# saugns/saugns

Hardware: AMD Instinct MI355X
Metric: mono samples/sec/GPU @ N voices (depth-3 FM) (higher is better)
Workload: dtype f32 (f64 table interpolation, u32 phase)

## Files before the change

### saugns_amd/build.py

```python
import os
import subprocess
import sys

HERE = os.path.dirname(os.path.abspath(__file__))
CSRC = os.path.join(HERE, "csrc")
LIB = os.path.join(HERE, "libsaugns_amd.so")
SOURCES = ["capi.cpp", "engine.cpp", "plan.cpp", "tables.cpp", "program_io.cpp", "sndout.cpp", "bank_builder.cpp",
           "hip_backend.hip"]
HEADERS = ["engine.h", "hip_backend.h", "capi_internal.h", "sau_dev_math.h", "sau_dev_ops.h", "launch_plan.h",
           "k_common.h", "k_wave_scan.h", "k_block_loop.h", "k_fast_types.h", "k_analyze.h", "k_decode.h", "k_fast_voice.h", "k_fast_group.h", "k_fast_group_lm.h",
           "k_chain.h", "k_finish.h", "k_levels.h", "k_decimate.h",
           "sau_dev_types.h", "../../include/sau_abi.h", "../../include/saugns_amd.h"]
FLAGS = ["--offload-arch=gfx950", "-O3", "-ffp-contract=off", "-fPIC", "-std=c++17",
         "-Wall", "-fvisibility=hidden", "-fvisibility-inlines-hidden"]


def _stale():
    if not os.path.exists(LIB):
        return True
    t = os.path.getmtime(LIB)
    deps = [os.path.join(CSRC, f) for f in SOURCES + HEADERS] + [__file__]
    return any(os.path.getmtime(d) > t for d in deps)


def build_variant(name, defines):
    build()
    hipcc = os.environ.get("HIPCC", "/opt/rocm/bin/hipcc")
    vdir = os.path.join(HERE, "variants")
    os.makedirs(vdir, exist_ok=True)
    obj = os.path.join(vdir, "hip_backend_%s.o" % name)
    subprocess.check_call([hipcc] + FLAGS + ["-D" + d for d in defines] +
                          ["-c", os.path.join(CSRC, "hip_backend.hip"), "-o", obj])
    objs = [os.path.join(CSRC, s.rsplit(".", 1)[0] + ".o") for s in SOURCES if s != "hip_backend.hip"]
    out = os.path.join(vdir, "lib_%s.so" % name)
    subprocess.check_call([hipcc, "--offload-arch=gfx950", "-shared", "-fPIC", "-o", out] + objs + [obj, "-ldl"])
    return out


def build(force=False, verbose=False):
    if not force and not _stale():
        return LIB
    import fcntl
    with open(os.path.join(HERE, ".build.lock"), "w") as lock:
        fcntl.flock(lock, fcntl.LOCK_EX)
        try:
            if not force and not _stale():
                return LIB
            return _build(verbose, force)
        finally:
            fcntl.flock(lock, fcntl.LOCK_UN)


def _build(verbose, force=False):
    hipcc = os.environ.get("HIPCC", "/opt/rocm/bin/hipcc")
    objs = []
    for src in SOURCES:
        obj = os.path.join(CSRC, src.rsplit(".", 1)[0] + ".o")
        objs.append(obj)
        deps = [src] + [h for h in HEADERS if src.endswith(".hip") or not h.startswith("k_")]
        if not force and os.path.exists(obj) and all(
                os.path.getmtime(os.path.join(CSRC, d)) <= os.path.getmtime(obj) for d in deps) and \
                os.path.getmtime(__file__) <= os.path.getmtime(obj):
            continue
        cmd = [hipcc] + FLAGS + ["-c", os.path.join(CSRC, src), "-o", obj]
        if verbose:
            print(" ".join(cmd), file=sys.stderr)
        subprocess.check_call(cmd)
    cmd = [hipcc, "--offload-arch=gfx950", "-shared", "-fPIC", "-o", LIB] + objs + ["-ldl"]
    subprocess.check_call(cmd)
    return LIB


if __name__ == "__main__":
    if len(sys.argv) > 2 and sys.argv[1] == "--variant":
        print(build_variant(sys.argv[2], sys.argv[3:]))
    else:
        print(build(force="--force" in sys.argv, verbose=True))
```

### saugns_amd/csrc/hip_backend.hip

```cpp
#include <hip/hip_runtime.h>
#include "hip_backend.h"
#include "launch_plan.h"
#include "sau_dev_ops.h"
#include <stdio.h>
#include <stdlib.h>
#include <string.h>
#include <deque>
#include <map>
#include <mutex>
#include <string>
#include <type_traits>
#include <vector>

namespace sauhip {

using namespace saudev;
using sauengine::BackendConfig;
using sauengine::tune_env;
using sauengine::SegmentDesc;
using namespace sauplan;

#include "k_common.h"
#include "k_block_loop.h"
#include "k_fast_types.h"
#include "k_analyze.h"
#include "k_decode.h"
#include "k_fast_voice.h"
#include "k_chain.h"
#include "k_finish.h"
#include "k_levels.h"
#include "k_decimate.h"
static_assert(MISC_BYTES == sizeof(Misc), "launch_plan.h plans the block loop's LDS with this size");


#define HIP_OK(call) do { hipError_t e_ = (call); if (e_ != hipSuccess) { \
	err = std::string(#call) + ": " + hipGetErrorString(e_); return false; } } while (0)

class BufPool {
public:
	static BufPool &get() { static BufPool *g = new BufPool; return *g; }
	static size_t bucket(size_t bytes) {
		size_t b = 4096;
		while (b * 2 <= bytes) b <<= 1;
		const size_t q = b / 8;
		return (bytes + q - 1) / q * q;
	}
	void *take(bool pinned, size_t bytes) {
		int dev = 0;
		(void)hipGetDevice(&dev);
		std::lock_guard<std::mutex> lk(mu_);
		auto &m = pinned ? pin_ : dev_[dev & 15];
		auto it = m.find(bytes);
		if (it == m.end()) return nullptr;
		void *q = it->second;
		m.erase(it);
		(pinned ? held_pin_ : held_dev_) -= bytes;
		return q;
	}
	bool give(bool pinned, void *q, size_t bytes) {
		int dev = 0;
		(void)hipGetDevice(&dev);
		std::lock_guard<std::mutex> lk(mu_);
		size_t &held = pinned ? held_pin_ : held_dev_;
		static const size_t cap_dev = env_mb("SAU_AMD_POOL_MB", (size_t)64 << 10);
		static const size_t cap_pin = env_mb("SAU_AMD_PINNED_POOL_MB", (size_t)1 << 10);
		if (held + bytes > (pinned ? cap_pin : cap_dev)) return false;
		(pinned ? pin_ : dev_[dev & 15]).emplace(bytes, q);
		held += bytes;
		return true;
	}
	size_t trim(bool pinned) {
		int dev = 0;
		(void)hipGetDevice(&dev);
		std::multimap<size_t, void *> out;
		{
			std::lock_guard<std::mutex> lk(mu_);
			out.swap(pinned ? pin_ : dev_[dev & 15]);
			for (auto &b : out) (pinned ? held_pin_ : held_dev_) -= b.first;
		}
		size_t n = 0;
		for (auto &b : out) { if (pinned) (void)hipHostFree(b.second); else (void)hipFree(b.second); n += b.first; }
		return n;
	}
private:
	static size_t env_mb(const char *name, size_t def_mb) {
		const char *v = getenv(name);
		return (v ? (size_t)atoll(v) : def_mb) << 20;
	}
	std::mutex mu_;
	std::multimap<size_t, void *> dev_[16], pin_;
	size_t held_dev_ = 0, held_pin_ = 0;
};

class StreamPool {
public:
	static StreamPool &get() { static StreamPool *g = new StreamPool; return *g; }
	hipStream_t take(int dev, int kind = 0) {
		std::lock_guard<std::mutex> lk(mu_);
		auto &v = free_[kind & 1][dev & 15];
		if (v.empty()) return nullptr;
		hipStream_t s = v.back();
		v.pop_back();
		return s;
	}
	void give(int dev, hipStream_t s, int kind = 0) {
		std::lock_guard<std::mutex> lk(mu_);
		auto &v = free_[kind & 1][dev & 15];
		if (v.size() < 8) v.push_back(s); else (void)hipStreamDestroy(s);
	}
private:
	std::mutex mu_;
	std::vector<hipStream_t> free_[2][16];
};

class SpreadLaunchOrder {
public:
	static SpreadLaunchOrder &get() { static SpreadLaunchOrder *g = new SpreadLaunchOrder; return *g; }
	template <typename F> bool ordered(int dev, hipStream_t stream, F launch) {
		std::lock_guard<std::mutex> lk(mu_);
		Dev &d = dev_[dev & 15];
		if (d.last && hipStreamWaitEvent(stream, d.last, 0) != hipSuccess) return false;
		if (!launch()) return false;
		hipEvent_t &e = d.ring[d.next++ & 63];
		if (!e && hipEventCreateWithFlags(&e, hipEventDisableTiming) != hipSuccess) return false;
		if (hipEventRecord(e, stream) != hipSuccess) return false;
		d.last = e;
		return true;
	}
private:
	struct Dev { hipEvent_t ring[64] = {}; hipEvent_t last = nullptr; unsigned next = 0; };
	std::mutex mu_;
	Dev dev_[16];
};

static void *pool_alloc(bool pinned, size_t &bytes, std::string &err) {
	bytes = BufPool::bucket(bytes);
	void *q = BufPool::get().take(pinned, bytes);
	if (q) return q;
	hipError_t e = pinned ? hipHostMalloc(&q, bytes, hipHostMallocDefault) : hipMalloc(&q, bytes);
	if (e != hipSuccess) {
		(void)hipGetLastError();
		if (BufPool::get().trim(pinned)) {
			e = pinned ? hipHostMalloc(&q, bytes, hipHostMallocDefault) : hipMalloc(&q, bytes);
			if (e == hipSuccess) return q;
			(void)hipGetLastError();
		}
		err = std::string(pinned ? "hipHostMalloc: " : "hipMalloc: ") + hipGetErrorString(e);
		return nullptr;
	}
	return q;
}
static void pool_free(bool pinned, void *q, size_t bytes) {
	if (!q) return;
	if (!BufPool::get().give(pinned, q, bytes)) { if (pinned) (void)hipHostFree(q); else (void)hipFree(q); }
}

static std::mutex &attr_mutex() { static std::mutex *m = new std::mutex; return *m; }
static bool raise_lds_attr(const void *fn, size_t lds, int dev, std::string &err) {
	static std::map<std::pair<const void *, int>, size_t> *slots = new std::map<std::pair<const void *, int>, size_t>;
	std::lock_guard<std::mutex> lk(attr_mutex());
	size_t &configured = (*slots)[std::make_pair(fn, dev & 15)];
	if (lds > configured) {
		hipError_t e = hipFuncSetAttribute(fn, hipFuncAttributeMaxDynamicSharedMemorySize, (int)lds);
		if (e != hipSuccess) { err = std::string("hipFuncSetAttribute: ") + hipGetErrorString(e); return false; }
		configured = lds;
	}
	return true;
}

enum : unsigned { FK_WIDE = 1, FK_TAIL = 2, FK_CUB = 4, FK_INNER = 8, FK_LANEMAJOR = 16 };
static const void *fast_kernel_fn(int build, uint32_t rows, unsigned form) {
	struct Entry { int build; uint32_t rows; unsigned form; const void *fn; };
#define FK(build, form, ...) {build, FK_ROWS(__VA_ARGS__), form, (const void *)fast_kernel<__VA_ARGS__>}
#define FK_ROWS(rows, ...) rows
	static const Entry table[] = {
		FK(0, 0, 2, 0), FK(0, 0, 4, 0), FK(0, 0, 5, 0), FK(0, 0, 6, 0), FK(0, 0, 8, 0),
		FK(1, 0, 2, 1), FK(1, 0, 4, 1),
		FK(2, 0, 2, 2), FK(2, 0, 4, 2), FK(2, 0, 5, 2), FK(2, 0, 6, 2), FK(2, 0, 8, 2),
		FK(3, 0, 4, 3), FK(3, 0, 5, 3), FK(3, 0, 6, 3),
		FK(0, FK_WIDE, 6, 0, false, true), FK(0, FK_WIDE, 8, 0, false, true), FK(0, FK_WIDE, 10, 0, false, true), FK(0, FK_WIDE, 12, 0, false, true),
		FK(2, FK_WIDE | FK_TAIL, 8, 2, false, true, true), FK(2, FK_WIDE, 8, 2, false, true), FK(2, FK_TAIL, 8, 2, false, false, true),
		FK(2, FK_CUB, (int)FAST_CUB_ROWS, 2, true),
		FK(0, FK_WIDE | FK_INNER | FK_LANEMAJOR, 12, 0, false, true, false, true, true), FK(0, FK_WIDE | FK_INNER, 12, 0, false, true, false, true),
		FK(0, FK_CUB, (int)FAST_CUB_ROWS, 0, true)};
#undef FK
#undef FK_ROWS
	for (const Entry &e : table)
		if (e.build == build && e.rows == rows && e.form == form) return e.fn;
	return nullptr;
}
static const void *repair_kernel_fn(uint32_t rows, bool wide) {
	if (wide)
		return rows == 12 ? (const void *)repair_kernel<12, true> : rows == 10 ? (const void *)repair_kernel<10, true>
		     : rows == 8 ? (const void *)repair_kernel<8, true> : rows == 6 ? (const void *)repair_kernel<6, true> : nullptr;
	return rows == 8 ? (const void *)repair_kernel<8> : rows == 6 ? (const void *)repair_kernel<6> : rows == 5 ? (const void *)repair_kernel<5>
	     : rows == 4 ? (const void *)repair_kernel<4> : rows == 2 ? (const void *)repair_kernel<2> : nullptr;
}
static const void *render_kernel_fn(uint32_t W, uint32_t T, uint32_t V, bool HB) {
	struct Entry { uint32_t W, T, V; bool HB; const void *fn; };
#define RK(W, T, V, HB) {W, T, V, HB, (const void *)render_kernel<W, T, V, HB>}
	static const Entry table[] = {
		RK(1, 4, 8, false), RK(1, 3, 8, false), RK(1, 2, 8, false), RK(1, 1, 8, false),
		RK(1, 4, 16, false), RK(1, 3, 16, false), RK(1, 2, 16, false), RK(1, 1, 16, false),
		RK(1, 1, 1, true), RK(1, 1, 1, false), RK(4, 4, 1, false), RK(8, 2, 1, false)};
#undef RK
	for (const Entry &e : table)
		if (e.W == W && e.T == T && e.V == V && e.HB == HB) return e.fn;
	return nullptr;
}

template <typename T, bool PINNED> struct PoolBuf {
	T *p = nullptr;
	size_t cap = 0, bytes = 0;
	PoolBuf() = default;
	PoolBuf(const PoolBuf &) = delete;
	PoolBuf &operator=(const PoolBuf &) = delete;
	~PoolBuf() { release(); }
	bool ensure(size_t n, std::string &err, bool keep = false) {
		if (n <= cap) return true;
		size_t nbytes = (n + n / 4 + 16) * sizeof(T);
		T *q = (T *)pool_alloc(PINNED, nbytes, err);
		if (!q) return false;
		if (keep && p && cap) {
			hipError_t e = PINNED ? (memcpy(q, p, cap * sizeof(T)), hipSuccess)
			                      : hipMemcpy(q, p, cap * sizeof(T), hipMemcpyDeviceToDevice);
			if (e != hipSuccess) { err = hipGetErrorString(e); return false; }
		}
		if (p) { (void)hipDeviceSynchronize(); pool_free(PINNED, p, bytes); }
		p = q; bytes = nbytes; cap = nbytes / sizeof(T);
		return true;
	}
	void release() { pool_free(PINNED, p, bytes); p = nullptr; cap = 0; bytes = 0; }
};
template <typename T> using DevBuf = PoolBuf<T, false>;
template <typename T> using PinBuf = PoolBuf<T, true>;

struct TableSet {
	int dev;
	std::vector<float> piluts;
	WaveConst wconst[12];
	HerpC23 *c23;
	HerpC01 *c01;
	WaveConst *wc;
};
static const TableSet *shared_tables(const float *piluts, const WaveConst *wconst, std::string &err) {
	static std::mutex mu;
	static std::vector<TableSet *> sets;
	int dev = 0;
	(void)hipGetDevice(&dev);
	std::lock_guard<std::mutex> lk(mu);
	for (const TableSet *t : sets)
		if (t->dev == dev && !memcmp(t->piluts.data(), piluts, (size_t)12 * WAVE_LEN * sizeof(float)) &&
		    !memcmp(t->wconst, wconst, sizeof t->wconst))
			return t;
	std::vector<HerpC23> h23((size_t)12 * WAVE_LEN);
	std::vector<HerpC01> h01((size_t)12 * WAVE_LEN);
	for (uint32_t wv = 0; wv < 12; ++wv)
		for (uint32_t i = 0; i < WAVE_LEN; ++i) {
			if (!herp_c1_scalable(piluts + (size_t)wv * WAVE_LEN, i)) {
				err = "wave table has slopes below 2^-100: unsupported";
				return nullptr;
			}
			herp_coeffs(piluts + (size_t)wv * WAVE_LEN, i,
					h23[(size_t)wv * WAVE_LEN + i], h01[(size_t)wv * WAVE_LEN + i]);
		}
	TableSet *t = new TableSet;
	t->dev = dev;
	t->piluts.assign(piluts, piluts + (size_t)12 * WAVE_LEN);
	memcpy(t->wconst, wconst, sizeof t->wconst);
	t->c23 = nullptr; t->c01 = nullptr; t->wc = nullptr;
	hipError_t e = hipMalloc((void **)&t->c23, h23.size() * sizeof(HerpC23));
	if (e == hipSuccess) e = hipMalloc((void **)&t->c01, h01.size() * sizeof(HerpC01));
	if (e == hipSuccess) e = hipMalloc((void **)&t->wc, 12 * sizeof(WaveConst));
	if (e == hipSuccess) e = hipMemcpy(t->c23, h23.data(), h23.size() * sizeof(HerpC23), hipMemcpyHostToDevice);
	if (e == hipSuccess) e = hipMemcpy(t->c01, h01.data(), h01.size() * sizeof(HerpC01), hipMemcpyHostToDevice);
	if (e == hipSuccess) e = hipMemcpy(t->wc, wconst, 12 * sizeof(WaveConst), hipMemcpyHostToDevice);
	if (e != hipSuccess) {
		err = std::string("wave tables: ") + hipGetErrorString(e);
		(void)hipFree(t->c23); (void)hipFree(t->c01); (void)hipFree(t->wc);
		delete t;
		return nullptr;
	}
	sets.push_back(t);
	return t;
}

int device_count() {
	int n = 0;
	if (hipGetDeviceCount(&n) != hipSuccess) return 0;
	return n;
}

bool device_pci_bus_id(int dev, char *buf, int len) {
	if (!buf || len < 16) return false;
	buf[0] = 0;
	return hipDeviceGetPCIBusId(buf, len, dev) == hipSuccess;
}

class HipBackendImpl : public HipBackend {
public:
	explicit HipBackendImpl(int device = -1) : want_dev_(device) {}
	void use_device() { (void)hipSetDevice(dev_); }

	~HipBackendImpl() override {
		use_device();
		if (stream_) (void)hipStreamSynchronize(stream_);
		if (chain_stream_) { (void)hipStreamSynchronize(chain_stream_); StreamPool::get().give(dev_, chain_stream_, 1); }
		for (hipEvent_t e : chain_ev_) (void)hipEventDestroy(e);
		for (int i = 0; i < 4; ++i) if (fetch_ev_[i]) (void)hipEventDestroy(fetch_ev_[i]);
		if (after_ev_) (void)hipEventDestroy(after_ev_);
		for (auto &e : events_) { (void)hipEventDestroy(e.a); (void)hipEventDestroy(e.b); }
		if (stream_) StreamPool::get().give(dev_, stream_);
	}

	bool init(const BackendConfig &cfg, std::string &err) override {
		cfg_ = cfg;
		int dev = 0;
		const char *env = getenv("SAU_AMD_DEVICE");
		if (want_dev_ >= 0) dev = want_dev_;
		else if (env) dev = atoi(env);
		if (dev < 0 || dev >= device_count()) { err = "no HIP device " + std::to_string(dev) + " (" + std::to_string(device_count()) + " visible)"; return false; }
		HIP_OK(hipSetDevice(dev));
		dev_ = dev;
		stream_ = StreamPool::get().take(dev);
		if (!stream_) HIP_OK(hipStreamCreateWithFlags(&stream_, hipStreamNonBlocking));
		static std::mutex prop_mu;
		static size_t dev_lds[16];
		static uint32_t dev_cus[16];
		static size_t dev_free[16];
		{
			std::lock_guard<std::mutex> lk(prop_mu);
			if (!dev_lds[dev & 15]) {
				hipDeviceProp_t prop;
				HIP_OK(hipGetDeviceProperties(&prop, dev));
				dev_lds[dev & 15] = prop.maxSharedMemoryPerMultiProcessor ? prop.maxSharedMemoryPerMultiProcessor
				                                                          : prop.sharedMemPerBlock;
				dev_cus[dev & 15] = prop.multiProcessorCount > 0 ? (uint32_t)prop.multiProcessorCount : FK_GRID;
				size_t mfree = 0, mtotal = 0;
				if (hipMemGetInfo(&mfree, &mtotal) == hipSuccess) dev_free[dev & 15] = mfree;
			}
			free_hint_ = dev_free[dev & 15];
			tun_ = tuning_from_env(tune_env);
			lim_ = device_limits(dev_lds[dev & 15], dev_cus[dev & 15], tun_);
		}
		debug_ = getenv("SAU_AMD_DEBUG") != nullptr;
		inmix_report_ = tune_env("SAU_AMD_INMIX_REPORT") != nullptr;
		inner_report_ = tune_env("SAU_AMD_INNER_REPORT") != nullptr;
		if (!ops_.ensure(cfg.op_count ? cfg.op_count : 1, err)) return false;
		HIP_OK(hipMemsetAsync(ops_.p, 0, ops_.cap * sizeof(DevOp), stream_));
		tables_ = shared_tables(cfg.piluts, cfg.wconst, err);
		if (!tables_) return false;
		memcpy(wconst_, cfg.wconst, sizeof wconst_);
		return true;
	}

	bool reserve_frames(uint32_t max_frames, bool , std::string &err) override {
		use_device();
		HIP_OK(hipStreamSynchronize(stream_));
		row_stride_ = (max_frames + 63) & ~63u;
		pcm_row_ = (size_t)row_stride_ * 2;
		if (!pcm_.ensure(pcm_row_ * cfg_.n_streams * pcm_units(), err)) return false;
		set_.vout_rows = 0;
		return true;
	}

	size_t pcm_units() const { return pcm_f32_ ? 2 : 1; }
	size_t pcm_pitch() const { return pcm_row_ * pcm_units() * sizeof(int16_t); }
	char *pcm_at(uint32_t stream) const { return (char *)pcm_.p + pcm_pitch() * stream; }
	bool set_format(sauengine::SampleFormat fmt, std::string &err) override {
		use_device();
		const bool f32 = fmt == sauengine::SF_F32;
		if (f32 == pcm_f32_) return true;
		pcm_f32_ = f32;
		if (pcm_row_ && !pcm_.ensure(pcm_row_ * cfg_.n_streams * pcm_units(), err)) { pcm_f32_ = !f32; return false; }
		return true;
	}

	void *stage(const void *src, size_t bytes, std::string &err) {
		const size_t need = (bytes + 63) & ~(size_t)63;
		if (arena_used_ + need > arena_.cap) {
			hipError_t e = hipStreamSynchronize(stream_);
			if (e != hipSuccess) { err = std::string("hipStreamSynchronize: ") + hipGetErrorString(e); return nullptr; }
			arena_used_ = 0;
			const size_t want = need > ((size_t)4 << 20) ? need : ((size_t)4 << 20);
			if (want > arena_.cap && !arena_.ensure(want, err)) return nullptr;
		}
		void *p = arena_.p + arena_used_;
		arena_used_ += need;
		memcpy(p, src, bytes);
		return p;
	}
	bool send(void *dst, const void *src, size_t bytes, std::string &err) {
		if (!bytes) return true;
		void *h = stage(src, bytes, err);
		if (!h) return false;
		HIP_OK(hipMemcpyAsync(dst, h, bytes, hipMemcpyHostToDevice, stream_));
		return true;
	}

	bool upload_plans(const Step *steps, const FastIds *fast_ids, size_t n_steps, const uint32_t *op_ids,
			size_t n_ids, std::string &err) override {
		use_device();
		if (!steps_.ensure(n_steps ? n_steps : 1, err) || !op_ids_.ensure(n_ids ? n_ids : 1, err) ||
		    !fast_ids_.ensure(n_steps ? 2 * n_steps : 1, err))
			return false;
		n_steps_total_ = (uint32_t)n_steps;
		return send(steps_.p, steps, n_steps * sizeof(Step), err) &&
			send(fast_ids_.p, fast_ids, 2 * n_steps * sizeof(FastIds), err) &&
			send(op_ids_.p, op_ids, n_ids * sizeof(uint32_t), err);
	}

	bool apply_updates(const OpUpdate *recs, size_t n, std::string &err) override {
		use_device();
		if (!n) return true;
		if (!recs_.ensure(n, err) || !send(recs_.p, recs, n * sizeof(OpUpdate), err)) return false;
		hipLaunchKernelGGL(event_kernel, dim3((unsigned)((n + 63) / 64)), dim3(64), 0, stream_,
				ops_.p, recs_.p, (uint32_t)n, tables_->wc);
		HIP_OK(hipGetLastError());
		return true;
	}

	bool poison_run(uint32_t frames, bool stereo, std::string &err) override {
		(void)frames; (void)stereo;
		use_device();
		if (pcm_.p) HIP_OK(hipMemsetD16Async((hipDeviceptr_t)pcm_.p, 0x5a5a, pcm_row_ * cfg_.n_streams * pcm_units(), stream_));
		return true;
	}

	bool zero_pcm(uint32_t first_stream, uint32_t n_streams, uint32_t first_frame, uint32_t n_frames, bool stereo,
			std::string &err) override {
		use_device();
		if (!pcm_.p || !n_streams || !n_frames) return true;
		const size_t fb = (stereo ? 2 : 1) * pcm_units() * sizeof(int16_t);
		char *at = pcm_at(first_stream) + (size_t)first_frame * fb;
		if (n_streams == 1) HIP_OK(hipMemsetAsync(at, 0, (size_t)n_frames * fb, stream_));
		else HIP_OK(hipMemset2DAsync(at, pcm_pitch(), 0, (size_t)n_frames * fb, n_streams, stream_));
		return true;
	}

	struct TimedPair { hipEvent_t a, b; int kind; bool used; };

	struct Job {
		const SegmentDesc &seg;
		PlanInputs in;
		BlockLoopPlan bl;
		FastPlan fk;
		RenderParams rp;
		FastParams fp;
		FastParams cfp;
		bool launched = true;
		bool tail_live = false;
		bool inmix_live = false;
		uint32_t early_mixed_blocks = 0;
		uint32_t block_grid = 1;
		TimedPair *tf = nullptr;
		explicit Job(const SegmentDesc &s) : seg(s) { memset(&rp, 0, sizeof rp); memset(&fp, 0, sizeof fp); }
	};

	bool render(const SegmentDesc &seg, std::string &err) override {
		use_device();
		if (!seg.n_voices) return true;
		++acc_launches_;
		Job j(seg);
		j.in.f32 = seg.format == sauengine::SF_F32;
		if (j.in.f32 != pcm_f32_) { err = "a segment of another sample format than the run announced"; return false; }
		if (j.in.f32 && seg.swap_bytes) { err = "float32 samples are not byte-swapped"; return false; }
		j.in.row_stride = row_stride_; j.in.pcm_row = pcm_row_; j.in.chain_budget = chain_rows_budget();
		j.bl = plan_block_loop(seg, tun_, lim_);
		if (!j.bl.ok) { err = "voice too large for one workgroup's LDS (block buffers + operator states)"; return false; }
		if (!ensure_rows(j, err) || !upload_descriptors(j, err)) return false;
		j.fk = plan_fast(seg, tun_, lim_, j.in);
		if (!prepare_fast(j, err) || !prepare_chains(j, err)) return false;
		fill_tables(j);
		if (!launch_analyze(j, err)) return false;
		if (j.fk.use_fast) {
			if (!launch_decode(j, err)) return false;
			if (j.fk.main_build == 2 && !launch_split(j, err)) return false;
			if (j.fp.scan ? !launch_sums_and_chains(j, err) : !launch_closed_form(j, err)) return false;
			if (!launch_cub(j, err)) return false;
			if (!j.launched) return false;
			if (!launch_repair(j, err)) return false;
			if (j.tf) (void)hipEventRecord(j.tf->b, stream_);
		}
		if (!launch_finalize(j, err)) return false;
		if (!launch_block_loop(j, err)) return false;
		return launch_mixer(j, err);
	}

	bool ensure_rows(Job &j, std::string &err) {
		const SegmentDesc &seg = j.seg;
		MixSet &S = set_;
		if (!voices_.ensure(seg.n_voices, err) || !S.vinfo.ensure(seg.n_voices, err)) return false;
		if (seg.n_voices > S.vout_rows || !S.vout.p) {
			HIP_OK(hipStreamSynchronize(stream_));
			if (!S.vout.ensure((size_t)seg.n_voices * row_stride_, err)) return false;
			S.vout_rows = seg.n_voices;
		}
		if (seg.n_pan_rows && !S.pan.ensure((size_t)seg.n_pan_rows * row_stride_, err)) return false;
		if (tun_.poison) {
			HIP_OK(hipMemsetD32Async((hipDeviceptr_t)S.vout.p, 0x3ea5a5a5, (size_t)seg.n_voices * row_stride_, stream_));
			if (seg.n_pan_rows) HIP_OK(hipMemsetD32Async((hipDeviceptr_t)S.pan.p, 0x3ea5a5a5, (size_t)seg.n_pan_rows * row_stride_, stream_));
		}
		return S.mstreams.ensure(seg.n_streams, err);
	}

	bool upload_descriptors(Job &j, std::string &err) {
		const SegmentDesc &seg = j.seg;
		MixSet &S = set_;
		ms_host_.resize(seg.n_streams);
		for (uint32_t s = 0; s < seg.n_streams; ++s) {
			MixStream &m = ms_host_[s];
			memset(&m, 0, sizeof m);
			m.first_row = seg.streams[s].first_voice;
			m.n_rows = seg.streams[s].n_voices;
			m.amp_scale = seg.streams[s].amp_scale;
			m.write_len = seg.streams[s].write_len;
			m.pcm = (int16_t *)pcm_at(s);
			if (m.write_len > j.in.max_write) j.in.max_write = m.write_len;
			if (m.n_rows > j.in.max_rows) j.in.max_rows = m.n_rows;
		}
		const bool same_voices = voices_sent_.size() == seg.n_voices && voices_dev_ == voices_.p &&
			memcmp(voices_sent_.data(), seg.voices, seg.n_voices * sizeof(VoiceDesc)) == 0;
		const bool same_ms = S.ms_sent.size() == seg.n_streams && S.ms_dev == S.mstreams.p &&
			memcmp(S.ms_sent.data(), ms_host_.data(), seg.n_streams * sizeof(MixStream)) == 0;
		if (!same_voices) {
			if (!send(voices_.p, seg.voices, seg.n_voices * sizeof(VoiceDesc), err)) return false;
			voices_sent_.assign(seg.voices, seg.voices + seg.n_voices);
			voices_dev_ = voices_.p;
		}
		if (!same_ms) {
			if (!send(S.mstreams.p, ms_host_.data(), seg.n_streams * sizeof(MixStream), err)) return false;
			S.ms_sent = ms_host_;
			S.ms_dev = S.mstreams.p;
		}
		return true;
	}

	bool prepare_fast(Job &j, std::string &err) {
		const SegmentDesc &seg = j.seg;
		const FastPlan &k = j.fk;
		FastParams &fp = j.fp;
		MixSet &S = set_;
		const size_t n_lists = (size_t)FAST_LISTS * seg.n_voices * k.fmax_steps;
		if (!finfo_.ensure(seg.n_voices, err) || !fdone_.ensure(seg.n_voices, err) ||
		    !worklist_.ensure(seg.n_voices, err) || !work_count_.ensure(4, err) ||
		    !fsteps_.ensure(n_lists * sizeof(FastStep), err) || !flines_.ensure(n_lists * sizeof(FastLine), err) ||
		    !faux_.ensure(n_lists * sizeof(FastAux), err)) return false;
		fp.voices = voices_.p; fp.steps = steps_.p; fp.fast_ids = fast_ids_.p; fp.op_ids = op_ids_.p; fp.ops = ops_.p;
		fp.vout = S.vout.p; fp.pan = S.pan.p; fp.info = finfo_.p; fp.fast_done = fdone_.p;
		fp.worklist = worklist_.p; fp.work_count = work_count_.p; fp.vinfo = S.vinfo.p;
		fp.g_c23 = tables_->c23; fp.g_c01 = tables_->c01; fp.fsteps = (FastStep *)fsteps_.p; fp.flines = (FastLine *)flines_.p; fp.faux = (FastAux *)faux_.p;
		fp.row_stride = row_stride_; fp.n_voices = seg.n_voices; fp.n_fast = k.n_fast;
		fp.seq_enable = k.seq_ok ? 1u : 0u; fp.ids_full_ofs = n_steps_total_;
		fp.scan = nullptr; fp.scan_groups = k.scan_groups; fp.mode = 0;
		if (tun_.xcd_queues && lim_.eight_xcds) {
			if (!inmix_ctl_.ensure(INMIX_WORDS, err)) return false;
			fp.inmix = inmix_ctl_.p;
		}
		if (k.scan) {
			if (!scan_.ensure((size_t)seg.n_voices * FAST_MAX_SCAN * k.scan_groups, err)) return false;
			fp.scan = scan_.p;
		}
		if (k.look) {
			if (k.look_words_real || !k.look_inside) {
				const unsigned long long *before = look_.p;
				if (!look_.ensure(k.look_words, err)) return false;
				if (look_.p != before || look_epoch_ >= (1u << 30) - 1) {
					HIP_OK(hipMemsetAsync(look_.p, 0, look_.cap * sizeof(unsigned long long), stream_));
					look_epoch_ = 0;
				}
				fp.look_epoch = ++look_epoch_;
			} else if (!look_.p && !look_.ensure(64, err)) {
				return false;
			}
			fp.look = look_.p;
		}
		if (!pass_flags_.p) {
			if (!pass_flags_.ensure(FAST_FLAGS, err)) return false;
			HIP_OK(hipMemsetAsync(pass_flags_.p, 0, pass_flags_.cap * sizeof(uint32_t), stream_));
		}
		fp.pass_flags = pass_flags_.p;
		fp.sum_levels = k.sum_levels;
		if (!repair_.ensure((size_t)seg.n_voices * FAST_REPAIR_WORDS, err)) return false;
		fp.repair = repair_.p;
		fp.repair_on = tun_.repair ? 1u : 0u;
		fp.max_ops = seg.max_ops; fp.max_steps = k.fmax_steps; fp.np = 64; fp.rows = k.rows; fp.rows_multi = k.rows_multi;
		fp.enable = k.use_fast ? 1u : 0u;
		if (k.inc_rows) {
			if (!inc_rows_.ensure((size_t)seg.n_inc_rows * 2 * k.inc_stride + 64, err)) return false;
			fp.inc_rows = inc_rows_.p; fp.inc_stride = k.inc_stride; fp.n_inc_rows = seg.n_inc_rows;
		}
		if (k.split_cf) {
			if (!vlists_.ensure((size_t)2 * seg.n_voices, err)) return false;
			fp.vlists = vlists_.p; fp.split_cf = 1; fp.rows_cf = k.rows_cf;
			fp.look_words_real = k.look_words_real && fp.look ? 1u : 0u;
		}
		fp.cub_ok = k.cub_ok ? 1u : 0u;
		memcpy(fp.wc, wconst_, sizeof wconst_);
		return true;
	}

	bool prepare_chains(Job &j, std::string &err) {
		const SegmentDesc &seg = j.seg;
		FastPlan &k = j.fk;
		FastParams &fp = j.fp;
		if (k.chains) {
			std::string rows_err;
			const size_t rows_need = (size_t)seg.n_chain_rows * 2 * k.chain_stride + 64;
			const char *rft = chain_rows_failed_once_ ? nullptr : tune_env("SAU_AMD_CHAIN_ROWS_FAIL");
			const bool rows_fail_test = rft && strcmp(rft, "real") != 0;
			if (rows_fail_test || !chain_rows_.ensure((rft && !rows_fail_test) ? (size_t)1 << 44 : rows_need, rows_err)) {
				chain_rows_failed_once_ = true;
				++chain_rows_failures_;
				if (debug_) fprintf(stderr, "saugns_amd: %zu bytes of chain rows not available (%s): block loop for this segment\n",
						rows_need * sizeof(float), rows_err.c_str());
				k.drop_chains();
			}
		}
		if (k.chains) {
			if (!chain_desc_.ensure(seg.n_chain_slots, err) ||
			    !fplines_.ensure((size_t)FAST_LISTS * seg.n_voices * k.fmax_steps * sizeof(FastLine), err)) return false;
			if (seg.chain_rows_padded) HIP_OK(hipMemsetAsync(chain_desc_.p, 0, (size_t)seg.n_chain_slots * sizeof(ChainDesc), stream_));
			fp.chain_rows = chain_rows_.p; fp.chain_stride = k.chain_stride; fp.n_chain_rows = seg.n_chain_rows; fp.n_chain_slots = seg.n_chain_slots;
			fp.chain_desc = chain_desc_.p; fp.fplines = (FastLine *)fplines_.p;
			fp.chain_inline = tun_.chain_inline ? 1u : 0u;
			fp.chain_early_ok = tun_.chain_early ? 1u : 0u;
			memcpy(fp.ctab_of_wave, k.ctabs.tab_of_wave, sizeof fp.ctab_of_wave);
			memcpy(fp.cwave_of_tab, k.ctabs.wave_of_tab, sizeof fp.cwave_of_tab);
			fp.n_ctabs = k.ctabs.n;
		}
		fp.lean_on = k.lean_on ? 1u : 0u;
		fp.rows_lean = k.rows_lean;
		return true;
	}

	void fill_tables(Job &j) {
		memcpy(j.fp.tab_of_wave, j.fk.tabs.tab_of_wave, sizeof j.fp.tab_of_wave);
		memcpy(j.fp.wave_of_tab, j.fk.tabs.wave_of_tab, sizeof j.fp.wave_of_tab);
		j.fp.n_tabs = j.fk.tabs.n;
	}

	bool launch_analyze(Job &j, std::string &err) {
		const SegmentDesc &seg = j.seg;
		(void)err;
		TimedPair *ta = timing_on_ ? new_pair(3) : nullptr;
		if (ta) (void)hipEventRecord(ta->a, stream_);
		uint32_t lo = seg.max_ops, ls = seg.max_steps;
		size_t albytes = (size_t)lo * sizeof(DevOp) + (size_t)ls * sizeof(Step) + (size_t)lo * sizeof(uint32_t);
		if (albytes > 48 * 1024 || !tun_.analyze_lds) { lo = 0; ls = 0; albytes = 0; }
		hipLaunchKernelGGL(analyze_kernel, dim3(seg.n_voices), dim3(64), albytes, stream_, j.fp, lo, ls);
		if (ta) (void)hipEventRecord(ta->b, stream_);
		return true;
	}
	bool launch_decode(Job &j, std::string &err) {
		hipLaunchKernelGGL(decode_kernel, dim3(j.seg.n_voices), dim3(64), 0, stream_, j.fp);
		if (!wait_for_predecessor(err)) return false;
		j.tf = timing_on_ ? new_pair(2) : nullptr;
		if (j.tf) (void)hipEventRecord(j.tf->a, stream_);
		return true;
	}

	bool launch_build(Job &j, std::string &err, int build, uint32_t rows, uint32_t grid, const FastParams *prm = nullptr, bool cf = false,
			bool wide = false) {
		if (build == 1 && rows > 4) rows = 4;
		if (build == 3) rows = rows < 5 ? 4 : rows > 6 ? 6 : rows;
		const void *fn = fast_kernel_fn(build, rows, (wide ? FK_WIDE : 0u) | (build == 2 && j.tail_live ? FK_TAIL : 0u));
		if (!fn) {
			err = "internal error: no fast_kernel build with " + std::to_string(rows) + " rows per pass in this form";
			return false;
		}
		const size_t lds = j.fk.launch_lds(build, rows, wide, cf);
		void *args[] = {(void *)(prm ? prm : &j.fp)};
		if (!raise_lds_attr(fn, lds, dev_, err)) return false;
		HIP_OK(hipLaunchKernel(fn, dim3(grid), dim3(1024), args, lds, stream_));
		return true;
	}
	void launch_fast(Job &j, std::string &err, uint32_t mode, uint32_t grid = 0) {
		FastParams &fp = j.fp;
		if (!grid) grid = j.fk.grid;
		fp.mode = mode;
		if (fp.lean_on && fp.chain_rows && (mode == fp.sum_levels + 1 || mode == fp.sum_levels + 2) &&
		    !launch_build(j, err, 3, fp.rows_lean, grid))
			j.launched = false;
		if (j.fk.main_build == 2) {
			fp.only_multi = 1;
			if (!launch_build(j, err, 1, j.fk.rows_multi, grid)) j.launched = false;
			fp.only_multi = 0;
		} else if (!launch_build(j, err, j.fk.main_build, j.fk.rows, grid, nullptr, false, j.fk.wide_cf)) {
			j.launched = false;
		}
	}

	bool launch_split(Job &j, std::string &err) {
		const SegmentDesc &seg = j.seg;
		const FastPlan &k = j.fk;
		FastParams &fp = j.fp, &cfp = j.cfp;
		if (k.tailmix) {
			if (!tail_ok_.ensure(seg.n_streams, err)) return false;
			fp.tail_ok = tail_ok_.p; fp.inmix_stream = set_.mstreams.p;
			fp.tail_flags = (seg.stereo ? 1u : 0u) | (seg.swap_bytes ? 2u : 0u);
			fp.tail_pcm_offset = seg.pcm_offset;
			hipLaunchKernelGGL(tailmix_kernel, dim3((seg.n_streams + 63) / 64), dim3(64), 0, stream_, fp, seg.n_streams);
			j.tail_live = true;
		}
		cfp = fp;
		cfp.n_fast = k.n_fast_cf; cfp.rows = k.rows_cf; cfp.mode = 0; cfp.only_multi = 0;
		if (getenv("SAU_AMD_DEBUG_DUO"))
			fprintf(stderr, "[sau-amd] duo %d: enabled %d look %d words_real %u FT %u rows_cf %u cub_ok %u tail %d may_scan %u of %u voices, lds %zu of %zu\n",
					(int)k.duo, (int)tun_.duo, fp.look != nullptr, fp.look_words_real, k.rows, k.rows_cf, fp.cub_ok, (int)j.tail_live, seg.n_may_scan, seg.n_voices,
					k.launch_lds(2, k.rows, false) + 1024, lim_.lds_limit);
		cfp.dyn_chunks = k.tasks_cf.dyn_chunks; cfp.dyn_static = k.tasks_cf.dyn_static;
		if (!k.duo && !launch_build(j, err, 0, k.rows_cf, k.grid_cf, &cfp, true, k.wide_cf)) j.launched = false;
		fp.mode = fp.sum_levels + 1; fp.only_multi = 0; fp.look_wpv = k.look_wpv; fp.look_groups = k.groups;
		fp.look_wpv_flags = k.look_wpv_flags;
		if (k.duo) {
			const size_t dlds = k.launch_lds(2, k.rows, false);
			if (!raise_lds_attr((const void *)duo_kernel, dlds, dev_, err)) return false;
			auto go = [&]() -> bool {
				void *da[] = {(void *)&fp, (void *)&cfp};
				return hipLaunchKernel((const void *)duo_kernel, dim3(lim_.fk_grid), dim3(1024), da, dlds, stream_) == hipSuccess;
			};
			if (!SpreadLaunchOrder::get().ordered(dev_, stream_, go)) j.launched = false;
		} else if (fp.look) {
			if (k.look_inside) {
				if (!launch_build(j, err, 2, k.rows, k.grid_look, nullptr, false, k.wide_look)) j.launched = false;
			} else if (!SpreadLaunchOrder::get().ordered(dev_, stream_, [&]() { return launch_build(j, err, 2, k.rows, k.grid_look, nullptr, false, k.wide_look); })) {
				j.launched = false;
			}
			if (fp.cub_ok) {
				const void *ck2 = fast_kernel_fn(2, FAST_CUB_ROWS, FK_CUB);
				const size_t lds2 = k.launch_lds(2, FAST_CUB_ROWS, false);
				if (!raise_lds_attr(ck2, lds2, dev_, err)) return false;
				auto go = [&]() -> bool {
					void *a2[] = {(void *)&fp};
					return hipLaunchKernel(ck2, dim3(k.grid_look), dim3(1024), a2, lds2, stream_) == hipSuccess;
				};
				if (k.look_inside ? !go() : !SpreadLaunchOrder::get().ordered(dev_, stream_, go)) j.launched = false;
			}
		}
		return true;
	}

	bool launch_sums_and_chains(Job &j, std::string &err) {
		const SegmentDesc &seg = j.seg;
		FastParams &fp = j.fp;
		if (fp.chain_rows && fp.chain_early_ok && !launch_early_chains(j, err)) return false;
		for (uint32_t pass = 1; pass <= fp.sum_levels && (!fp.look || seg.n_chain_rows); ++pass) {
			launch_fast(j, err, pass);
			hipLaunchKernelGGL(scan_kernel, dim3(seg.n_voices), dim3(64), 0, stream_, fp);
		}
		if (!fp.chain_rows) { launch_fast(j, err, fp.sum_levels + 1); return true; }
		return launch_chains(j, err);
	}

	bool launch_early_chains(Job &j, std::string &err) {
		FastParams &fp = j.fp;
		const uint32_t cgrid = j.fk.chain_grid;
		const size_t clds = chain_alone_lds((size_t)fp.n_ctabs * CHAIN_TAB_BYTES + CHAIN_IO_BYTES, cgrid);
		if (!raise_lds_attr((const void *)chain_kernel, clds, dev_, err)) return false;
		fp.chain_early = 1; fp.range_mode = 0;
		hipLaunchKernelGGL(chain_kernel, dim3(cgrid), dim3(192), clds, stream_, fp);
		const size_t rlds = chain_alone_lds(RCHAIN_LDS_BYTES, cgrid);
		if (!raise_lds_attr((const void *)rchain_kernel, rlds, dev_, err)) return false;
		hipLaunchKernelGGL(rchain_kernel, dim3(cgrid), dim3(RCHAIN_THREADS), rlds, stream_, fp);
		fp.chain_early = 0;
		return true;
	}

	bool launch_chains(Job &j, std::string &err) {
		const FastPlan &k = j.fk;
		FastParams &fp = j.fp;
		const uint32_t cgrid = k.chain_grid, n_chunks = k.chunks.n;
		const size_t clds = chain_alone_lds((size_t)fp.n_ctabs * CHAIN_TAB_BYTES + CHAIN_IO_BYTES, cgrid);
		if (!raise_lds_attr((const void *)chain_kernel, clds, dev_, err)) return false;
		TimedPair *tc = nullptr;
		if (n_chunks == 1) {
			tc = timing_on_ ? new_pair(0) : nullptr;
			fp.range_mode = 0;
			launch_fast(j, err, fp.sum_levels + 2);
			if (tc) (void)hipEventRecord(tc->a, stream_);
			hipLaunchKernelGGL(chain_kernel, dim3(cgrid), dim3(192), clds, stream_, fp);
			if (tc) (void)hipEventRecord(tc->b, stream_);
			launch_fast(j, err, fp.sum_levels + 1);
			return true;
		}
		if (!chain_stream_) {
			chain_stream_ = StreamPool::get().take(dev_, 1);
			if (!chain_stream_) {
				int lo = 0, hi = 0;
				(void)hipDeviceGetStreamPriorityRange(&lo, &hi);
				HIP_OK(hipStreamCreateWithPriority(&chain_stream_, hipStreamNonBlocking, hi));
			}
		}
		while (chain_ev_.size() < 2 * (size_t)n_chunks) {
			hipEvent_t e;
			HIP_OK(hipEventCreateWithFlags(&e, hipEventDisableTiming));
			chain_ev_.push_back(e);
		}
		tc = timing_on_ ? new_pair(0) : nullptr;
		const uint32_t *cb = k.chunks.cb;
		auto set_range = [&](FastParams &q, uint32_t mode, uint32_t c) {
			q.range_mode = mode; q.f_lo = cb[c]; q.f_hi = c + 1 == n_chunks ? 0xffffffffu : cb[c + 1];
		};
		for (uint32_t c = 0; c < n_chunks; ++c) {
			set_range(fp, 1, c);
			fp.range_last = c + 1 == n_chunks;
			launch_fast(j, err, fp.sum_levels + 2, k.pass_grid);
			HIP_OK(hipEventRecord(chain_ev_[2 * c], stream_));
			HIP_OK(hipStreamWaitEvent(chain_stream_, chain_ev_[2 * c], 0));
			FastParams cp = fp;
			set_range(cp, 1, c);
			if (tc && c == 0) (void)hipEventRecord(tc->a, chain_stream_);
			hipLaunchKernelGGL(chain_kernel, dim3(cgrid), dim3(192), clds, chain_stream_, cp);
			if (tc && c + 1 == n_chunks) (void)hipEventRecord(tc->b, chain_stream_);
			HIP_OK(hipEventRecord(chain_ev_[2 * c + 1], chain_stream_));
		}
		uint32_t mixed_blocks = 0;
		if (k.early_mix) hipLaunchKernelGGL(premix_kernel, dim3((j.seg.n_voices + 63) / 64), dim3(64), 0, stream_, fp);
		for (uint32_t c = 0; c < n_chunks; ++c) {
			HIP_OK(hipStreamWaitEvent(stream_, chain_ev_[2 * c + 1], 0));
			set_range(fp, 2, c);
			fp.range_last = c + 1 == n_chunks;
			launch_fast(j, err, fp.sum_levels + 1, c + 1 == n_chunks ? k.grid : k.pass_grid);
			if (k.early_mix && c + 1 < n_chunks && cb[c + 1] > 512) {
				const uint32_t hi = (cb[c + 1] - 512) / 256;
				if (hi > mixed_blocks) {
					MixParams mp = mix_params(j.seg, set_);
					mp.blk_lo = mixed_blocks; mp.blk_hi = hi;
					TimedPair *tm = timing_on_ ? new_pair(1) : nullptr;
					if (tm) (void)hipEventRecord(tm->a, stream_);
					hipLaunchKernelGGL((j.in.f32 ? mix_kernel_f32 : mix_kernel), dim3(hi - mixed_blocks, j.seg.n_streams), dim3(256), 0, stream_, mp);
					if (tm) (void)hipEventRecord(tm->b, stream_);
					mixed_blocks = hi;
				}
			}
		}
		j.early_mixed_blocks = mixed_blocks;
		fp.range_mode = 0; fp.f_lo = 0; fp.f_hi = 0; fp.range_last = 0;
		return true;
	}

	bool launch_closed_form(Job &j, std::string &err) {
		const SegmentDesc &seg = j.seg;
		const FastPlan &k = j.fk;
		FastParams &fp = j.fp;
		fp.dyn_chunks = k.tasks.dyn_chunks; fp.dyn_static = k.tasks.dyn_static; fp.dyn_small = k.tasks.dyn_small;
		if (k.queues) {
			fp.inmix_flags = k.inmix_flags;
			fp.inmix_div_s = k.div.s; fp.inmix_div_m = k.div.m;
			if (k.inmix) {
				fp.inmix_stream = set_.mstreams.p;
				fp.inmix_pcm_offset = seg.pcm_offset;
				hipLaunchKernelGGL(premix_kernel, dim3((seg.n_voices + 63) / 64), dim3(64), 0, stream_, fp);
				j.inmix_live = true;
			}
		}
		if (k.inner != INNER_NONE) {
			const bool lm = k.inner == INNER_LANE_MAJOR;
			const void *ik = fast_kernel_fn(0, 12, FK_WIDE | FK_INNER | (lm ? FK_LANEMAJOR : 0u));
			const size_t lds = k.inner_lds();
			FastParams ep = fp;
			ep.mode = 0; ep.edge_only = 1; ep.dyn_static = 1; ep.dyn_chunks = 2; ep.dyn_small = 0; ep.inmix_flags = 0;
			if (!launch_build(j, err, 0, k.rows, k.grid_edge, &ep, false, true)) j.launched = false;
			fp.mode = 0;
			void *iargs[] = {(void *)&fp};
			if (!raise_lds_attr(ik, lds, dev_, err)) return false;
			HIP_OK(hipLaunchKernel(ik, dim3(k.grid), dim3(1024), iargs, lds, stream_));
			if (inner_report_) fprintf(stderr, "[sau-amd] inner: %s, %u voices\n", lm ? "lane-major" : "row-major", seg.n_voices);
		} else {
			if (inner_report_) fprintf(stderr, "[sau-amd] inner: none (rows %u, wide %d, chunks %u), %u voices\n", k.rows, k.wide_cf ? 1 : 0, fp.dyn_chunks, seg.n_voices);
			launch_fast(j, err, 0);
		}
		fp.dyn_chunks = 0; fp.inmix_flags = 0; fp.dyn_small = 0;
		return true;
	}

	bool launch_cub(Job &j, std::string &err) {
		if (!j.fp.cub_ok) return true;
		const FastPlan &k = j.fk;
		FastParams q = k.main_build == 2 ? j.cfp : j.fp;
		q.n_fast = k.n_fast_cf; q.rows = FAST_CUB_ROWS; q.mode = 0; q.only_multi = 0;
		q.dyn_chunks = k.tasks_cub.dyn_chunks; q.dyn_static = k.tasks_cub.dyn_static;
		const size_t qlds = k.launch_lds(0, FAST_CUB_ROWS, false, true);
		const void *ck = fast_kernel_fn(0, FAST_CUB_ROWS, FK_CUB);
		if (!raise_lds_attr(ck, qlds, dev_, err)) return false;
		void *qargs[] = {(void *)&q};
		HIP_OK(hipLaunchKernel(ck, dim3(k.grid_cub), dim3(1024), qargs, qlds, stream_));
		return true;
	}

	bool launch_repair(Job &j, std::string &err) {
		const FastPlan &k = j.fk;
		const size_t rlds = k.launch_lds(0, k.rows_repair, k.wide_cf, k.main_build == 2);
		FastParams rpar = k.main_build == 2 ? j.cfp : j.fp;
		rpar.mode = 0;
		const void *rk = repair_kernel_fn(k.rows_repair, k.wide_cf);
		if (!rk) {
			err = "internal error: no repair_kernel build with " + std::to_string(k.rows_repair) + " rows per pass in this form";
			return false;
		}
		if (!raise_lds_attr(rk, rlds, dev_, err)) return false;
		j.fp.mode = 0;
		void *rargs[] = {(void *)&rpar};
		HIP_OK(hipLaunchKernel(rk, dim3(k.grid_repair), dim3(1024), rargs, rlds, stream_));
		return true;
	}

	bool launch_finalize(Job &j, std::string &err) {
		const SegmentDesc &seg = j.seg;
		TimedPair *tz = timing_on_ ? new_pair(3) : nullptr;
		if (tz) (void)hipEventRecord(tz->a, stream_);
		hipLaunchKernelGGL(finalize_kernel, dim3((unsigned)(((size_t)seg.n_voices * j.fp.max_ops * 8 + 63) / 64)), dim3(64), 0,
				stream_, j.fp);
		if (tz) (void)hipEventRecord(tz->b, stream_);
		HIP_OK(hipGetLastError());
		if (debug_ && j.fk.use_fast) {
			(void)hipStreamSynchronize(stream_);
			FastInfo fi0;
			(void)hipMemcpy(&fi0, finfo_.p, sizeof fi0, hipMemcpyDeviceToHost);
			fprintf(stderr, "[sau-amd] fast: voice 0 total %u H %u bail %u steps %u seq %u; n_fast %u rows %u\n",
					fi0.total, fi0.H, fi0.bail, fi0.n_fsteps, fi0.seq, j.fk.n_fast, j.fk.rows);
			std::vector<FastStep> fs(fi0.n_fsteps < 64 ? fi0.n_fsteps : 64);
			if (!fs.empty()) (void)hipMemcpy(fs.data(), fsteps_.p, fs.size() * sizeof(FastStep), hipMemcpyDeviceToHost);
			for (size_t i = 0; i < fs.size(); ++i)
				fprintf(stderr, "[sau-amd]   step %zu kind %u flags %#x which %u dep %u out %d pm %d fpm %d amp %d aux %d type %#x inc %u ac %g fc %g ramp %u\n",
						i, fs[i].kind & 0xff, (fs[i].kind >> 8) & 0xff, (fs[i].kind >> 16) & 0xff, fs[i].kind >> 24,
						(int)fs[i].out_off, (int)fs[i].pm_off, (int)fs[i].fpm_off, (int)fs[i].amp_off, (int)fs[i].aux_off,
						fs[i].type, fs[i].inc, fs[i].ac, fs[i].fc, fs[i].ramp);
		}
		return true;
	}

	bool launch_block_loop(Job &j, std::string &err) {
		const SegmentDesc &seg = j.seg;
		const BlockLoopPlan &b = j.bl;
		RenderParams &rp = j.rp;
		rp.team_bytes = (uint32_t)b.team_bytes;
		memcpy(rp.tab_of_wave, b.tabs.tab_of_wave, sizeof rp.tab_of_wave);
		memcpy(rp.wave_of_tab, b.tabs.wave_of_tab, sizeof rp.wave_of_tab);
		rp.voices = voices_.p; rp.steps = steps_.p; rp.op_ids = op_ids_.p; rp.ops = ops_.p;
		rp.vout = set_.vout.p; rp.pan = set_.pan.p; rp.vinfo = set_.vinfo.p;
		rp.g_c23 = tables_->c23; rp.g_c01 = tables_->c01;
		rp.row_stride = row_stride_; rp.seg_len = seg.len;
		rp.n_slots = seg.n_slots; rp.max_ops = seg.max_ops; rp.n_tabs = b.tabs.n;
		rp.max_steps = seg.max_steps; rp.n_main = seg.n_main;
		memcpy(rp.wc, wconst_, sizeof wconst_);
		rp.fast_done = fdone_.p; rp.worklist = worklist_.p; rp.work_count = work_count_.p;
		j.block_grid = b.grid(seg, j.fk.use_fast);
		if (b.HB) {
			const size_t stride = ((size_t)seg.n_slots * 64 * sizeof(float) + (size_t)seg.max_ops * sizeof(DevOp) +
				(size_t)seg.max_steps * sizeof(Step) + 255) / 256 * 256 / sizeof(float);
			if (stride > 0xffffffffu) { err = "voice too large (block buffers + operator records beyond 16 GiB)"; return false; }
			if (!big_slots_.ensure((size_t)j.block_grid * stride, err)) return false;
			rp.big_slots = big_slots_.p; rp.big_stride = (uint32_t)stride;
		}
		if (!wait_for_predecessor(err)) return false;
		TimedPair *tp = timing_on_ ? new_pair(0) : nullptr;
		if (tp) (void)hipEventRecord(tp->a, stream_);
		const void *fn = render_kernel_fn(b.W, b.T, b.V, b.HB);
		if (!fn) { err = "internal error: no render_kernel build of this geometry"; return false; }
		if (!raise_lds_attr(fn, b.lds, dev_, err)) return false;
		void *args[] = {(void *)&rp};
		HIP_OK(hipLaunchKernel(fn, dim3(j.block_grid), dim3(64 * b.W * b.V), args, b.lds, stream_));
		HIP_OK(hipGetLastError());
		if (tp) (void)hipEventRecord(tp->b, stream_);
		if (debug_) debug_dump("after render", seg, j.block_grid);
		return true;
	}

	bool launch_mixer(Job &j, std::string &err) {
		const SegmentDesc &seg = j.seg;
		const uint32_t max_write = j.in.max_write;
		const Mixer which = plan_mixer(seg, tun_, j.in, pcm_pitch(), j.inmix_live, j.early_mixed_blocks);
		if (which == MIX_NONE) return true;
		MixParams mp = mix_params(seg, set_);
		mp.early_blocks = j.early_mixed_blocks;
		mp.inmix = j.inmix_live ? inmix_ctl_.p : nullptr;
		mp.tail_ok = j.tail_live ? tail_ok_.p : nullptr;
		TimedPair *tm = timing_on_ ? new_pair(1) : nullptr;
		if (tm) (void)hipEventRecord(tm->a, stream_);
		switch (which) {
		case MIX_FEW_F32: hipLaunchKernelGGL(mix_few_kernel_f32, dim3((max_write + 1023) / 1024, seg.n_streams), dim3(256), 0, stream_, mp); break;
		case MIX_F32: hipLaunchKernelGGL(mix_kernel_f32, dim3((max_write + 255) / 256, seg.n_streams), dim3(256), 0, stream_, mp); break;
		case MIX_FEW: hipLaunchKernelGGL(mix_few_kernel, dim3((max_write + 1023) / 1024, seg.n_streams), dim3(256), 0, stream_, mp); break;
		case MIX_64: hipLaunchKernelGGL(mix_kernel64, dim3((max_write + 63) / 64, seg.n_streams), dim3(64), 0, stream_, mp); break;
		default: hipLaunchKernelGGL(mix_kernel, dim3((max_write + 255) / 256, seg.n_streams), dim3(256), 0, stream_, mp); break;
		}
		HIP_OK(hipGetLastError());
		if (tm) (void)hipEventRecord(tm->b, stream_);
		if (mp.inmix && inmix_report_) report_inmix(mp, seg.n_voices, max_write);
		return true;
	}

	void report_inmix(const MixParams &mp, uint32_t n_voices, uint32_t max_write) {
		std::vector<uint32_t> h(INMIX_WORDS);
		uint32_t g[2] = {0, 0};
		(void)hipStreamSynchronize(stream_);
		(void)hipMemcpy(h.data(), mp.inmix, INMIX_WORDS * sizeof(uint32_t), hipMemcpyDeviceToHost);
		(void)hipMemcpy(g, work_count_.p, sizeof g, hipMemcpyDeviceToHost);
		const uint32_t nch = h[INMIX_NCH] < INMIX_MAX_CHUNKS ? h[INMIX_NCH] : INMIX_MAX_CHUNKS, tpc = h[INMIX_TPC];
		uint32_t tiles = 0, whole = 0, all = 0;
		for (uint32_t k = 0; k < nch; ++k) {
			uint32_t lo_f = k * h[INMIX_CF], hi_f = lo_f + h[INMIX_CF];
			if (k >= h[INMIX_NCH1]) { lo_f = h[INMIX_BASE] + (k - h[INMIX_NCH1]) * h[INMIX_CFS]; hi_f = lo_f + h[INMIX_CFS]; }
			else if (hi_f > h[INMIX_BASE]) hi_f = h[INMIX_BASE];
			if (hi_f > max_write) hi_f = max_write;
			const uint32_t tk = hi_f > lo_f ? (hi_f - lo_f + INMIX_TILE - 1) / INMIX_TILE : 0u;
			uint32_t c = 0;
			for (uint32_t j = 0; j < tk && j < tpc && j < INMIX_MAX_TPC; ++j) c += (h[INMIX_CHUNK + INMIX_LINE * k + INMIX_BITS + (j >> 5)] >> (j & 31u)) & 1u;
			tiles += c; whole += c == tk ? 1u : 0u; all += tk;
		}
		fprintf(stderr, "[sau-amd] inmix: voices %u frames %u chunks %u x %u frames, tiles %u of %u, chunks mixed whole %u, guard %u %u\n",
				n_voices, max_write, nch, h[INMIX_CF], tiles, all, whole, g[0], g[1]);
	}

	template <typename SetT> MixParams mix_params(const SegmentDesc &seg, const SetT &S) {
		MixParams mp;
		mp.streams = S.mstreams.p; mp.vout = S.vout.p; mp.pan = S.pan.p; mp.vinfo = S.vinfo.p;
		mp.row_stride = row_stride_; mp.pcm_offset = seg.pcm_offset;
		mp.stereo = seg.stereo ? 1 : 0;
		mp.swap_bytes = seg.swap_bytes ? 1 : 0;
		mp.blk_lo = 0; mp.blk_hi = 0; mp.early_blocks = 0; mp.guard = work_count_.p; mp.inmix = nullptr; mp.tail_ok = nullptr;
		return mp;
	}

	bool fetch_pcm(uint32_t stream, int16_t *dst, uint32_t frames, bool stereo, std::string &err) override {
		if (pcm_f32_) { err = "the last run's samples are float32"; return false; }
		return fetch_units(stream, dst, (size_t)frames * (stereo ? 2 : 1), err);
	}
	bool fetch_pcm_f32(uint32_t stream, float *dst, uint32_t frames, bool stereo, std::string &err) override {
		if (!pcm_f32_) { err = "the last run's samples are int16"; return false; }
		return fetch_units(stream, (int16_t *)dst, (size_t)frames * (stereo ? 2 : 1) * 2, err);
	}
	bool fetch_units(uint32_t stream, int16_t *dst, const size_t n, std::string &err) {
		use_device();
		const bool pinned = host_blocks_.count(dst) != 0;
		if (!pinned && !h_pcm_.ensure(n, err)) return false;
		HIP_OK(hipMemcpyAsync(pinned ? dst : h_pcm_.p, pcm_at(stream), n * sizeof(int16_t),
				hipMemcpyDeviceToHost, stream_));
		HIP_OK(hipStreamSynchronize(stream_));
		if (!pinned) memcpy(dst, h_pcm_.p, n * sizeof(int16_t));
		return true;
	}

	bool fetch_pcm_async(uint32_t stream, int16_t *dst, uint32_t frames, bool stereo, int slot,
			std::string &err) override {
		if (pcm_f32_) { err = "the last run's samples are float32"; return false; }
		return fetch_bytes_async(stream, dst, (size_t)frames * (stereo ? 2 : 1) * sizeof(int16_t), slot, err);
	}
	bool fetch_pcm_f32_async(uint32_t stream, float *dst, uint32_t frames, bool stereo, int slot,
			std::string &err) override {
		if (!pcm_f32_) { err = "the last run's samples are int16"; return false; }
		return fetch_bytes_async(stream, dst, (size_t)frames * (stereo ? 2 : 1) * sizeof(float), slot, err);
	}
	bool fetch_bytes_async(uint32_t stream, void *dst, size_t bytes, int slot, std::string &err) {
		slot &= 3;
		use_device();
		if (!fetch_ev_[slot]) HIP_OK(hipEventCreateWithFlags(&fetch_ev_[slot], hipEventDisableTiming));
		hipStream_t cs = stream_;
		HIP_OK(hipMemcpyAsync(dst, pcm_at(stream), bytes, hipMemcpyDeviceToHost, cs));
		HIP_OK(hipEventRecord(fetch_ev_[slot], cs));
		return true;
	}
	bool wait_fetch(int slot, std::string &err) override {
		slot &= 3;
		if (fetch_ev_[slot]) HIP_OK(hipEventSynchronize(fetch_ev_[slot]));
		return true;
	}
	void *alloc_host(size_t bytes) override {
		use_device();
		std::string err;
		void *p = pool_alloc(true, bytes, err);
		if (p) host_blocks_[p] = bytes;
		return p;
	}
	void free_host(void *p) override {
		use_device();
		auto it = host_blocks_.find(p);
		if (it == host_blocks_.end()) return;
		(void)hipStreamSynchronize(stream_);
		pool_free(true, p, it->second);
		host_blocks_.erase(it);
	}

	bool begin_metering(std::string &err) override {
		use_device();
		if (lev_acc_.p) return true;
		if (!lev_acc_.ensure(cfg_.n_streams, err)) return false;
		HIP_OK(hipMemsetAsync(lev_acc_.p, 0, (size_t)cfg_.n_streams * sizeof(LevelsAcc), stream_));
		return true;
	}
	bool launch_levels(LevelsParams lp, const LevelsPlan &plan, std::string &err) {
		if (!plan.blocks) lp.parts = nullptr;
		else {
			if (!lev_parts_.ensure(plan.parts, err)) return false;
			lp.parts = lev_parts_.p;
			lp.blocks = plan.blocks;
			if (lp.f32) hipLaunchKernelGGL(levels_kernel<float>, dim3(plan.blocks, plan.rows), dim3(LEVELS_THREADS), 0, stream_, lp);
			else hipLaunchKernelGGL(levels_kernel<int16_t>, dim3(plan.blocks, plan.rows), dim3(LEVELS_THREADS), 0, stream_, lp);
			HIP_OK(hipGetLastError());
		}
		hipLaunchKernelGGL(levels_finish_kernel, dim3(plan.finish_grid), dim3(64), 0, stream_, lp);
		HIP_OK(hipGetLastError());
		return true;
	}
	bool measure_streams(const uint32_t *frames, bool stereo, sauengine::SampleFormat format, std::string &err) override {
		use_device();
		const bool f32 = format == sauengine::SF_F32;
		if (!lev_acc_.p) { err = "level metering has not begun"; return false; }
		if (f32 != pcm_f32_ || !pcm_.p) { err = "no rows of that sample format to measure"; return false; }
		uint32_t longest = 0;
		for (uint32_t s = 0; s < cfg_.n_streams; ++s) {
			if (frames[s] > row_stride_) { err = "frames beyond the streams' rows"; return false; }
			if (frames[s] > longest) longest = frames[s];
		}
		if (!longest) return true;
		const LevelsPlan plan = plan_levels(longest, stereo ? 2 : 1, cfg_.n_streams);
		if (!plan.ok) { err = "too many streams for one level measurement"; return false; }
		if (!lev_frames_.ensure(cfg_.n_streams, err) || !send(lev_frames_.p, frames, (size_t)cfg_.n_streams * sizeof(uint32_t), err)) return false;
		LevelsParams lp;
		memset((void *)&lp, 0, sizeof lp);
		lp.rows = pcm_.p; lp.pitch = pcm_pitch();
		lp.row_frames = lev_frames_.p;
		lp.channels = stereo ? 2 : 1;
		lp.acc = lev_acc_.p; lp.n_rows = cfg_.n_streams; lp.f32 = f32 ? 1 : 0; lp.accumulate = 1;
		return launch_levels(lp, plan, err);
	}
	static void levels_out(const LevelsAcc &a, sauengine::Levels &o) {
		o.frames = a.frames;
		for (int c = 0; c < 2; ++c) {
			const float ip = (float)a.ipeak[c] / 32767.0f;
			o.peak[c] = a.fpeak[c] > ip ? a.fpeak[c] : ip;
			o.sum_sq[c] = a.fsum[c] + (double)a.isum[c] / (32767.0 * 32767.0);
			o.over[c] = a.over[c]; o.full_scale[c] = a.full[c]; o.nonfinite[c] = a.nonf[c];
		}
	}
	bool read_records(const LevelsAcc *dev, size_t n, sauengine::Levels *out, std::string &err) {
		std::vector<LevelsAcc> h(n);
		HIP_OK(hipMemcpyAsync(h.data(), dev, n * sizeof(LevelsAcc), hipMemcpyDeviceToHost, stream_));
		HIP_OK(hipStreamSynchronize(stream_));
		for (size_t i = 0; i < n; ++i) levels_out(h[i], out[i]);
		return true;
	}
	bool read_levels(sauengine::Levels *out, bool reset, std::string &err) override {
		use_device();
		if (!lev_acc_.p) { memset((void *)out, 0, sizeof(sauengine::Levels) * cfg_.n_streams); return true; }
		if (!read_records(lev_acc_.p, cfg_.n_streams, out, err)) return false;
		if (reset) HIP_OK(hipMemsetAsync(lev_acc_.p, 0, (size_t)cfg_.n_streams * sizeof(LevelsAcc), stream_));
		return true;
	}
	bool measure_rows(const void *rows, size_t pitch, size_t n_rows, sauengine::SampleFormat format, size_t frames, bool stereo,
			sauengine::Levels *out, std::string &err) override {
		use_device();
		const bool f32 = format == sauengine::SF_F32;
		const size_t ch = stereo ? 2 : 1, size = f32 ? sizeof(float) : sizeof(int16_t);
		if (!n_rows) return true;
		if (!rows || ((uintptr_t)rows & 15u) || (pitch & 15u) || !out) { err = "bad argument: rows and pitch_bytes must be multiples of 16"; return false; }
		if (frames > SIZE_MAX / 8 || (n_rows > 1 && frames * ch * size > pitch)) { err = "bad argument: rows longer than their pitch"; return false; }
		if (frames) {
			hipPointerAttribute_t at;
			memset((void *)&at, 0, sizeof at);
			if (hipPointerGetAttributes(&at, rows) != hipSuccess) { (void)hipGetLastError(); err = "bad argument: rows is not device memory"; return false; }
			if (at.type != hipMemoryTypeDevice || at.device != dev_) { err = "bad argument: rows must be memory of the batch's device"; return false; }
			hipDeviceptr_t base = nullptr;
			size_t span = 0;
			if (hipMemGetAddressRange(&base, &span, (hipDeviceptr_t)rows) != hipSuccess) { (void)hipGetLastError(); err = "bad argument: rows is not device memory"; return false; }
			size_t need = 0;
			const bool wraps = __builtin_mul_overflow(pitch, n_rows - 1, &need) || __builtin_add_overflow(need, frames * ch * size, &need);
			const size_t ofs = (size_t)((const char *)rows - (const char *)base);
			if (wraps || ofs > span || need > span - ofs) { err = "bad argument: the rows reach beyond their allocation"; return false; }
		}
		const LevelsPlan plan = plan_levels(frames, (uint32_t)ch, n_rows);
		if (!plan.ok) { err = "bad argument: too many rows (65535 at most) or frames for one level measurement"; return false; }
		if (!lev_out_.ensure(n_rows, err)) return false;
		LevelsParams lp;
		memset((void *)&lp, 0, sizeof lp);
		lp.rows = rows; lp.pitch = pitch; lp.row_frames = nullptr; lp.frames = frames;
		lp.channels = (uint32_t)ch;
		lp.acc = lev_out_.p; lp.n_rows = (uint32_t)n_rows; lp.f32 = f32 ? 1 : 0; lp.accumulate = 0;
		return launch_levels(lp, plan, err) && read_records(lev_out_.p, n_rows, out, err);
	}
	bool requantize(uint32_t stream, uint32_t frames, bool stereo, float gain, sauengine::SampleFormat out, bool swap_bytes,
			std::string &err) override {
		use_device();
		if (!pcm_f32_ || !pcm_.p) { err = "the last run's samples are not float32"; return false; }
		if (stream >= cfg_.n_streams || frames > row_stride_) { err = "frames beyond the stream's row"; return false; }
		const bool f32 = out == sauengine::SF_F32;
		if (f32 && swap_bytes) { err = "float32 samples are not byte-swapped"; return false; }
		const size_t n = (size_t)frames * (stereo ? 2 : 1);
		if (!n) return true;
		if (!requant_.ensure(n * (f32 ? sizeof(float) : sizeof(int16_t)), err)) return false;
		RequantParams rq;
		rq.src = (const float *)pcm_at(stream); rq.dst = requant_.p; rq.n = n; rq.gain = gain; rq.swap_bytes = swap_bytes ? 1 : 0;
		const dim3 grid((unsigned)((n + 1023) / 1024));
		if (f32) hipLaunchKernelGGL(requant_kernel<float>, grid, dim3(256), 0, stream_, rq);
		else hipLaunchKernelGGL(requant_kernel<int16_t>, grid, dim3(256), 0, stream_, rq);
		HIP_OK(hipGetLastError());
		return true;
	}
	bool fetch_requant_async(void *dst, size_t bytes, int slot, std::string &err) override {
		slot &= 3;
		use_device();
		if (bytes > requant_.bytes) { err = "more bytes than were requantised"; return false; }
		if (!fetch_ev_[slot]) HIP_OK(hipEventCreateWithFlags(&fetch_ev_[slot], hipEventDisableTiming));
		HIP_OK(hipMemcpyAsync(dst, requant_.p, bytes, hipMemcpyDeviceToHost, stream_));
		HIP_OK(hipEventRecord(fetch_ev_[slot], stream_));
		return true;
	}

	bool begin_decimation(int factor, bool stereo, std::string &err) override {
		use_device();
		const DecimPlan plan = plan_decimate(0, factor, stereo ? 2 : 1, cfg_.n_streams, sizeof(float));
		if (!plan.ok) { err = "bad argument"; return false; }
		const size_t hist = (size_t)cfg_.n_streams * plan.hist_floats;
		if (!decim_hist_.ensure(hist, err) || !decim_taps_.ensure(plan.taps, err) || !decim_frames_.ensure(cfg_.n_streams, err)) return false;
		HIP_OK(hipMemsetAsync(decim_hist_.p, 0, hist * sizeof(float), stream_));
		std::vector<double> h(plan.taps);
		if (sauengine::decimator_taps(factor, h.data(), h.size()) != plan.taps) { err = "bad argument"; return false; }
		if (!send(decim_taps_.p, h.data(), h.size() * sizeof(double), err)) return false;
		decim_factor_ = factor; decim_stereo_ = stereo;
		return true;
	}
	template <int K, typename OutT> void launch_decimate(const DecimPlan &plan, const DecimParams &dp, bool stereo) {
		const dim3 grid(plan.tiles, plan.streams), block(DECIM_THREADS);
		if (stereo) hipLaunchKernelGGL((decimate_kernel<K, OutT, 2>), grid, block, 0, stream_, dp, (const double *)decim_taps_.p);
		else hipLaunchKernelGGL((decimate_kernel<K, OutT, 1>), grid, block, 0, stream_, dp, (const double *)decim_taps_.p);
	}
	bool decimate(const uint32_t *frames_hi, uint32_t buf_len, int factor, bool stereo, sauengine::SampleFormat out_fmt, bool swap_bytes,
			std::string &err) override {
		use_device();
		if (!decim_hist_.p || factor != decim_factor_ || stereo != decim_stereo_) { err = "decimation has not begun"; return false; }
		const bool f32 = out_fmt == sauengine::SF_F32;
		if (f32 && swap_bytes) { err = "float32 samples are not byte-swapped"; return false; }
		const uint32_t ch = stereo ? 2 : 1;
		const DecimPlan plan = plan_decimate(buf_len, factor, ch, cfg_.n_streams, f32 ? sizeof(float) : sizeof(int16_t));
		if (!plan.ok) { err = "bad argument"; return false; }
		const unsigned long long n_hi = (unsigned long long)buf_len * (unsigned)factor;
		bool any = false;
		for (uint32_t s = 0; s < cfg_.n_streams; ++s) {
			if (frames_hi[s] > n_hi || frames_hi[s] > row_stride_) { err = "frames beyond the streams' rows"; return false; }
			any = any || frames_hi[s] != 0;
		}
		if (any && (!pcm_f32_ || !pcm_.p)) { err = "the last run's samples are not float32"; return false; }
		decim_out_f32_ = f32; decim_out_pitch_ = plan.out_pitch; decim_out_bytes_ = (size_t)buf_len * ch * (f32 ? sizeof(float) : sizeof(int16_t));
		if (!plan.tiles) return true;
		if (!decim_out_.ensure(plan.out_pitch * cfg_.n_streams, err)) return false;
		if (!send(decim_frames_.p, frames_hi, (size_t)cfg_.n_streams * sizeof(uint32_t), err)) return false;
		DecimParams dp;
		memset((void *)&dp, 0, sizeof dp);
		dp.rows = (const float *)pcm_.p; dp.row_pitch = pcm_f32_ ? pcm_pitch() : 0;
		dp.frames = decim_frames_.p; dp.hist = decim_hist_.p;
		dp.out = decim_out_.p; dp.out_pitch = plan.out_pitch;
		dp.buf_len = buf_len; dp.swap_bytes = swap_bytes ? 1 : 0;
		switch (factor * 2 + (f32 ? 1 : 0)) {
		case 5: launch_decimate<2, float>(plan, dp, stereo); break;
		case 4: launch_decimate<2, int16_t>(plan, dp, stereo); break;
		case 9: launch_decimate<4, float>(plan, dp, stereo); break;
		case 8: launch_decimate<4, int16_t>(plan, dp, stereo); break;
		case 17: launch_decimate<8, float>(plan, dp, stereo); break;
		default: launch_decimate<8, int16_t>(plan, dp, stereo); break;
		}
		HIP_OK(hipGetLastError());
		hipLaunchKernelGGL(decimate_carry_kernel, dim3(plan.streams), dim3(DECIM_CARRY_THREADS), 0, stream_, dp, plan.hist_floats, ch, n_hi);
		HIP_OK(hipGetLastError());
		return true;
	}
	bool fetch_decimated_async(uint32_t stream, void *dst, size_t bytes, int slot, std::string &err) override {
		slot &= 3;
		use_device();
		if (stream >= cfg_.n_streams || bytes > decim_out_bytes_ || (bytes && !decim_out_.p)) { err = "more bytes than were decimated"; return false; }
		if (!fetch_ev_[slot]) HIP_OK(hipEventCreateWithFlags(&fetch_ev_[slot], hipEventDisableTiming));
		if (bytes) {
			const char *src = (const char *)decim_out_.p + decim_out_pitch_ * stream;
			if (host_blocks_.count(dst)) HIP_OK(hipMemcpyAsync(dst, src, bytes, hipMemcpyDeviceToHost, stream_));
			else {
				if (!h_pcm_.ensure((bytes + 1) / 2, err)) return false;
				HIP_OK(hipMemcpyAsync(h_pcm_.p, src, bytes, hipMemcpyDeviceToHost, stream_));
				HIP_OK(hipStreamSynchronize(stream_));
				memcpy(dst, h_pcm_.p, bytes);
			}
		}
		HIP_OK(hipEventRecord(fetch_ev_[slot], stream_));
		return true;
	}
	const float *device_decimated_f32(uint32_t stream) override {
		return decim_out_.p && decim_out_f32_ && decim_out_bytes_ && stream < cfg_.n_streams ? (const float *)((const char *)decim_out_.p + decim_out_pitch_ * stream) : nullptr;
	}
	size_t device_decimated_pitch() override { return decim_out_.p && decim_out_bytes_ ? decim_out_pitch_ : 0; }

	const int16_t *device_pcm(uint32_t stream) override { return pcm_.p && !pcm_f32_ ? (const int16_t *)pcm_at(stream) : nullptr; }
	const float *device_pcm_f32(uint32_t stream) override { return pcm_.p && pcm_f32_ ? (const float *)pcm_at(stream) : nullptr; }
	size_t device_pcm_pitch() override { return pcm_.p ? pcm_pitch() : 0; }

	bool sync(std::string &err) override {
		use_device();
		HIP_OK(hipStreamSynchronize(stream_));
		arena_used_ = 0;
		return true;
	}
	bool save_state(int slot, std::string &err) override {
		slot &= 3;
		use_device();
		if (!ops_snap_[slot].ensure(ops_.cap, err)) return false;
		HIP_OK(hipMemcpyAsync(ops_snap_[slot].p, ops_.p, ops_.cap * sizeof(DevOp), hipMemcpyDeviceToDevice, stream_));
		return true;
	}
	bool load_state(int slot, std::string &err) override {
		slot &= 3;
		use_device();
		if (!ops_snap_[slot].p || ops_snap_[slot].cap < ops_.cap) { err = "no operator state was saved under this slot"; return false; }
		HIP_OK(hipMemcpyAsync(ops_.p, ops_snap_[slot].p, ops_.cap * sizeof(DevOp), hipMemcpyDeviceToDevice, stream_));
		return true;
	}

	void timing(double *render_ms, double *mix_ms, uint64_t *launches, bool reset) override {
		if (!timing_on_) { timing_on_ = true; }
		(void)hipStreamSynchronize(stream_);
		drain_pairs();
		if (render_ms) *render_ms = acc_ms_[0] + acc_ms_[2];
		if (mix_ms) *mix_ms = acc_ms_[1];
		if (launches) *launches = acc_launches_;
		if (reset) { acc_ms_[0] = acc_ms_[1] = acc_ms_[2] = acc_ms_[3] = 0; acc_launches_ = 0; }
	}

	size_t chain_rows_budget() override { return sauengine::chain_rows_budget(free_hint_, chain_rows_failures_); }
	void *stream_handle() override { return (void *)stream_; }
	bool order_after(HipBackend *before, std::string &err) override {
		HipBackendImpl *o = static_cast<HipBackendImpl *>(before);
		if (o == this) return true;
		if (o->dev_ != dev_) { err = "sauAmd_Batch_order_after: the two batches are on different devices"; return false; }
		use_device();
		if (!after_ev_) HIP_OK(hipEventCreateWithFlags(&after_ev_, hipEventDisableTiming));
		HIP_OK(hipEventRecord(after_ev_, o->stream_));
		after_pending_ = true;
		return true;
	}
	bool wait_for_predecessor(std::string &err) {
		if (!after_pending_) return true;
		after_pending_ = false;
		HIP_OK(hipStreamWaitEvent(stream_, after_ev_, 0));
		return true;
	}
	void set_timing(int level) override { timing_on_ = level > 0; timing_level_ = level; }

	void timing_ex(double *out4, uint64_t *segments, bool reset) override {
		if (!timing_on_) timing_on_ = true;
		(void)hipStreamSynchronize(stream_);
		drain_pairs();
		out4[0] = acc_ms_[2]; out4[1] = acc_ms_[0]; out4[2] = acc_ms_[1]; out4[3] = acc_ms_[3];
		if (segments) *segments = acc_launches_;
		if (reset) { acc_ms_[0] = acc_ms_[1] = acc_ms_[2] = acc_ms_[3] = 0; acc_launches_ = 0; }
	}

	void debug_dump(const char *what, const SegmentDesc &seg, uint32_t block_grid) {
		(void)hipStreamSynchronize(stream_);
		uint32_t n = cfg_.op_count < 8 ? cfg_.op_count : 8;
		std::vector<DevOp> h(n);
		(void)hipMemcpy(h.data(), ops_.p, n * sizeof(DevOp), hipMemcpyDeviceToHost);
		fprintf(stderr, "[sau-amd] %s: seg len %u off %u voices %u slots %u\n", what, seg.len,
				seg.pcm_offset, seg.n_voices, seg.n_slots);
		for (uint32_t v = 0; v < seg.n_voices && v < 4; ++v)
			fprintf(stderr, "  voice %u: run_len %u plan %u+%u ops %u+%u\n", v, seg.voices[v].run_len,
					seg.voices[v].plan_ofs, seg.voices[v].plan_len, seg.voices[v].ops_ofs, seg.voices[v].nops);
		{
			uint32_t wc = 0;
			(void)hipMemcpy(&wc, work_count_.p, 4, hipMemcpyDeviceToHost);
			{
				std::vector<FastInfo> all(seg.n_voices);
				(void)hipMemcpy(all.data(), finfo_.p, all.size() * sizeof(FastInfo), hipMemcpyDeviceToHost);
				uint32_t shown = 0;
				for (size_t v = 0; v < all.size() && shown < 16; ++v)
					if (all[v].bail || all[v].total < seg.voices[v].run_len) {
						uint32_t dbg = 0;
						(void)hipMemcpy(&dbg, repair_.p + v * FAST_REPAIR_WORDS + 1, 4, hipMemcpyDeviceToHost);
						fprintf(stderr, "  voice %zu: fast total %u of %u, bail %u, H %u, seq %u; last unresolved hold: lane p_min+%u row %u step %u group %u (mod 4096)\n", v, all[v].total,
								seg.voices[v].run_len, all[v].bail, all[v].H, all[v].seq, dbg >> 24, (dbg >> 20) & 15, (dbg >> 12) & 255, dbg & 0xfff);
						++shown;
					}
			}
			std::vector<VoiceOut> vi(seg.n_voices < 4 ? seg.n_voices : 4);
			std::vector<uint32_t> fd(vi.size());
			std::vector<FastInfo> fi(vi.size());
			(void)hipMemcpy(vi.data(), set_.vinfo.p, vi.size() * sizeof(VoiceOut), hipMemcpyDeviceToHost);
			(void)hipMemcpy(fd.data(), fdone_.p, fd.size() * 4, hipMemcpyDeviceToHost);
			(void)hipMemcpy(fi.data(), finfo_.p, fi.size() * sizeof(FastInfo), hipMemcpyDeviceToHost);
			float v8[8] = {0};
			(void)hipMemcpy(v8, set_.vout.p, sizeof v8, hipMemcpyDeviceToHost);
			fprintf(stderr, "  work_count %u block_grid %u; row0: %g %g %g %g %g %g\n", wc, block_grid, v8[0], v8[1],
					v8[2], v8[3], v8[4], v8[5]);
			for (size_t v = 0; v < vi.size(); ++v)
				fprintf(stderr, "  vinfo %zu: pan %g has_pan %u valid %u prow %u | fast total %u H %u bail %u done %u\n", v,
						vi[v].pan_const, vi[v].has_pan, vi[v].valid_len, vi[v].pan_row, fi[v].total, fi[v].H,
						fi[v].bail, fd[v]);
		}
		for (uint32_t i = 0; i < n; ++i) {
			const DevOp &o = h[i];
			fprintf(stderr, "  op %u: time %u flags %#x type %u wave %u phase %u prev_s %g fb %g\n", i, o.time,
					o.flags, o.type, o.wave, o.phase, o.prev_s, o.fb_s);
			for (int l = 0; l < 6; ++l)
				if (o.line[l].flags || o.line[l].v0 != 0.f)
					fprintf(stderr, "     line %d: v0 %g vt %g pos %u end %u type %u flags %#x\n", l,
							o.line[l].v0, o.line[l].vt, o.line[l].pos, o.line[l].end, o.line[l].type,
							o.line[l].flags);
		}
	}

private:
	TimedPair *new_pair(int kind) {
		if (timing_level_ == 1 && kind != 2) return nullptr;
		if (n_used_ == events_.size()) {
			if (events_.size() >= 4096) { (void)hipStreamSynchronize(stream_); drain_pairs(); }
			else {
				TimedPair p; p.kind = 0; p.used = false;
				if (hipEventCreate(&p.a) != hipSuccess || hipEventCreate(&p.b) != hipSuccess) return nullptr;
				events_.push_back(p);
			}
		}
		TimedPair *p = &events_[n_used_++];
		p->kind = kind; p->used = true;
		return p;
	}
	void drain_pairs() {
		for (size_t i = 0; i < n_used_; ++i) {
			float ms = 0;
			if (hipEventElapsedTime(&ms, events_[i].a, events_[i].b) == hipSuccess) {
				acc_ms_[events_[i].kind & 3] += ms;
			}
		}
		n_used_ = 0;
	}

	BackendConfig cfg_;
	hipStream_t stream_ = nullptr;
	Tuning tun_;
	DeviceLimits lim_;
	bool debug_ = false;
	bool inner_report_ = false;
	bool inmix_report_ = false;
	uint32_t row_stride_ = 0;
	size_t pcm_row_ = 0;
	bool pcm_f32_ = false;
	WaveConst wconst_[12];
	DevBuf<DevOp> ops_;
	DevBuf<DevOp> ops_snap_[4];
	DevBuf<Step> steps_;
	DevBuf<FastIds> fast_ids_;
	uint32_t n_steps_total_ = 0;
	DevBuf<uint32_t> op_ids_;
	DevBuf<VoiceDesc> voices_;
	struct MixSet {
		DevBuf<float> vout, pan;
		DevBuf<VoiceOut> vinfo;
		DevBuf<MixStream> mstreams;
		uint32_t vout_rows = 0;
		std::vector<MixStream> ms_sent;
		const void *ms_dev = nullptr;
	};
	MixSet set_;
	DevBuf<int16_t> pcm_;
	DevBuf<OpUpdate> recs_;
	const TableSet *tables_ = nullptr;
	PinBuf<int16_t> h_pcm_;
	PinBuf<unsigned char> arena_;
	size_t arena_used_ = 0;
	std::vector<VoiceDesc> voices_sent_;
	std::vector<MixStream> ms_host_;
	const void *voices_dev_ = nullptr;
	std::deque<TimedPair> events_;
	size_t n_used_ = 0;
	bool timing_on_ = false;
	double acc_ms_[4] = {0, 0, 0, 0};
	uint64_t acc_launches_ = 0;
	int timing_level_ = 2;
	DevBuf<FastInfo> finfo_;
	DevBuf<uint32_t> fdone_, worklist_, work_count_;
	DevBuf<float> big_slots_;
	DevBuf<unsigned char> fsteps_, flines_, faux_;
	DevBuf<unsigned long long> scan_;
	DevBuf<uint32_t> pass_flags_, repair_;
	hipEvent_t fetch_ev_[4] = {nullptr, nullptr, nullptr, nullptr};
	int dev_ = 0;
	int want_dev_ = -1;
	std::map<void *, size_t> host_blocks_;
	DevBuf<unsigned long long> look_;
	uint32_t look_epoch_ = 0;
	DevBuf<uint32_t> inc_rows_;
	hipStream_t chain_stream_ = nullptr;
	std::vector<hipEvent_t> chain_ev_;
	DevBuf<float> chain_rows_;
	bool chain_rows_failed_once_ = false;
	unsigned chain_rows_failures_ = 0;
	size_t free_hint_ = 0;
	DevBuf<ChainDesc> chain_desc_;
	DevBuf<unsigned char> fplines_;
	hipEvent_t after_ev_ = nullptr;
	bool after_pending_ = false;
	DevBuf<uint32_t> inmix_ctl_;
	DevBuf<uint32_t> tail_ok_;
	DevBuf<LevelsAcc> lev_acc_, lev_out_;
	DevBuf<LevelsPart> lev_parts_;
	DevBuf<uint32_t> lev_frames_;
	DevBuf<unsigned char> requant_;
	DevBuf<float> decim_hist_;
	DevBuf<double> decim_taps_;
	DevBuf<uint32_t> decim_frames_;
	DevBuf<unsigned char> decim_out_;
	int decim_factor_ = 0;
	bool decim_stereo_ = false, decim_out_f32_ = false;
	size_t decim_out_pitch_ = 0, decim_out_bytes_ = 0;
	DevBuf<uint32_t> vlists_;
	size_t chain_alone_lds(size_t need, uint32_t grid) const {
		if (!tun_.chain_alone || grid > lim_.cus || need * 2 > lim_.lds_limit) return need;
		const size_t half = lim_.lds_limit / 2 + 1024;
		return need > half ? need : half;
	}
};

HipBackend *create_hip_backend(std::string &err, int device) {
	if (device_count() <= 0) {
		err = "no HIP device available (this backend has no CPU fallback)";
		return nullptr;
	}
	return new HipBackendImpl(device);
}

}
```

### saugns_amd/csrc/k_analyze.h

```cpp

__device__ __forceinline__ bool step_is_chain(const Step &st, const DevOp &o) {
	return !o.rt_frozen && step_may_chain(st) && (o.type == OT_WAVE || o.type == OT_RASEG) &&
		(st.sm != NO_SLOT || o.line[L_PMA].v0 != 0.f || (o.line[L_PMA].flags & LP_GOAL));
}
__device__ __forceinline__ bool step_is_chain_acc(const Step &st, const DevOp &o) {
	return step_is_chain(st, o) && !o.rt_fconst_valid && st.pm == NO_SLOT && st.fpm == NO_SLOT;
}

__device__ __forceinline__ bool step_is_chain_inline(bool enabled, const Step *plan, uint32_t si, const uint32_t *ids, const DevOp *ops,
		uint32_t *line_step) {
	if (!enabled) { *line_step = ~0u; return false; }
	const Step st = plan[si];
	const DevOp &o = ops[ids[st.op]];
	*line_step = ~0u;
	if (!step_is_chain(st, o) || st.pm != NO_SLOT || st.fpm != NO_SLOT || st.sm != NO_SLOT) return false;
	if (o.rt_fconst_valid) return true;
	uint32_t fmul = st.fmul, prov = st.prov;
	if (st.freq != NO_SLOT) {
		uint32_t q = si;
		bool found = false;
		while (q-- > 0) {
			const Step sq = plan[q];
			if (sq.kind == ST_LINE && sq.which == L_FREQ && sq.op == st.op && sq.out == st.freq) { found = true; break; }
			if ((sq.kind == ST_OSC || sq.kind == ST_LERP || sq.kind == ST_LINE || sq.kind == ST_SMLINE) && sq.out == st.freq) return false;
		}
		if (!found) return false;
		*line_step = q;
		fmul = plan[q].fmul; prov = plan[q].prov;
	}
	if (fmul != NO_SLOT) {
		const LineState &fl = o.line[L_FREQ];
		const bool ratio = (fl.flags & LP_STATE_RATIO) || ((fl.flags & LP_GOAL) && (fl.flags & LP_GOAL_RATIO));
		if (ratio && !(prov != NO_SLOT && ops[ids[prov]].rt_fconst_valid)) return false;
	}
	return true;
}

__device__ __forceinline__ uint32_t block_owner(const Step *plan, uint32_t si, uint32_t slot) {
	for (uint32_t q = si; q-- > 0;) {
		const Step sq = plan[q];
		if (sq.kind == ST_LINE && sq.which == L_FREQ && sq.out == slot) return sq.op;
	}
	return 0xff;
}

__device__ __forceinline__ bool op_has_fpm(const Step *plan, uint32_t n, uint32_t op) {
	for (uint32_t q = 0; q < n; ++q) {
		const Step sq = plan[q];
		if (sq.kind == ST_OSC && sq.op == op) return sq.fpm != NO_SLOT;
	}
	return false;
}

__global__ void __launch_bounds__(64) analyze_kernel(FastParams P, uint32_t lds_ops, uint32_t lds_steps) {
	extern __shared__ __align__(16) unsigned char a_lds[];
	const uint32_t v = blockIdx.x;
	const int lane = threadIdx.x;
	if (v == 0 && lane == 0 && P.inmix)
		for (uint32_t x = 0; x < 8; ++x) P.inmix[INMIX_QUEUE + INMIX_LINE * x] = 0;
	if (v == 0 && lane == 0) { P.work_count[0] = 0; P.work_count[1] = 0; }
	if (v >= P.n_voices) return;
	const VoiceDesc vd = P.voices[v];
	const uint32_t *gids = P.op_ids + vd.ops_ofs;
	const bool use_lds = lds_ops != 0 && vd.nops <= lds_ops && vd.plan_len <= lds_steps;
	DevOp *lops = (DevOp *)a_lds;
	Step *lplan = (Step *)(a_lds + (size_t)lds_ops * sizeof(DevOp));
	uint32_t *lids = (uint32_t *)(a_lds + (size_t)lds_ops * sizeof(DevOp) + (size_t)lds_steps * sizeof(Step));
	__shared__ uint8_t a_extra[256], a_dep[256], a_level[256];
	for (uint32_t i = (uint32_t)lane; i < 64; i += 64) { ((uint32_t *)a_extra)[i] = 0; ((uint32_t *)a_dep)[i] = 0; ((uint32_t *)a_level)[i] = 0; }
	if (use_lds) {
		static_assert(sizeof(DevOp) % 16 == 0 && sizeof(Step) == 16, "copied 16 bytes at a time");
		constexpr uint32_t Q = sizeof(DevOp) / 16;
		for (uint32_t i = (uint32_t)lane; i < vd.nops * Q; i += 64)
			((uint4 *)lops)[i] = ((const uint4 *)&P.ops[gids[i / Q]])[i % Q];
		for (uint32_t i = (uint32_t)lane; i < vd.plan_len; i += 64) ((uint4 *)lplan)[i] = ((const uint4 *)(P.steps + vd.plan_ofs))[i];
		for (uint32_t i = (uint32_t)lane; i < vd.nops; i += 64) lids[i] = i;
	}
	__syncthreads();
	if (lane == 0) {
	const uint32_t *ids = use_lds ? lids : gids;
	DevOp *const OPS = use_lds ? lops : P.ops;
	bool bad = (vd.flags & VD_NO_FAST) != 0 || !P.enable;
	bool seq = false, has_red = false, has_rcub = false, has_rchain = false;
	uint32_t min_time = 0xFFFFFFFFu;
	const Step *plan = use_lds ? lplan : P.steps + vd.plan_ofs;
	for (uint32_t i = 0; i < vd.nops; ++i) OPS[ids[i]].rt_frozen = 0;
	if (P.chain_desc)
		for (uint32_t k = 0; k < vd.n_chain; ++k)
			((uint32_t *)P.chain_desc)[(size_t)(vd.chain_slot + k) * CHAIN_DESC_WORDS] = 0;
	const bool chain_ok = P.chain_rows != nullptr && P.scan != nullptr;
	bool has_chain = false;
	{
		uint32_t dep = 0, frozen_at = 0;
		for (uint32_t si = 0; si < vd.plan_len; ++si) {
			const Step st = plan[si];
			DevOp &o = OPS[ids[st.op]];
			if (st.flags & SF_BEGIN) {
				++dep;
				if (!frozen_at && !(o.flags & OPF_TIME_INF) && o.time == 0) frozen_at = dep;
			}
			if (frozen_at) o.rt_frozen = 1;
			if (st.flags & SF_END) {
				if (dep == frozen_at) frozen_at = 0;
				--dep;
			}
		}
	}
	if (OPS[ids[vd.carr_local]].rt_frozen) bad = true;
	for (uint32_t i = 0; i < vd.nops; ++i) {
		DevOp &o = OPS[ids[i]];
		if (o.rt_frozen) continue;
		if ((vd.flags & VD_TAILS) && o.type == OT_RASEG && o.wave == LN_cub) has_rcub = true;
		for (uint32_t ln = 0; ln < L_COUNT; ++ln) {
			if (!(o.line[ln].flags & LP_GOAL)) continue;
			if ((vd.flags & VD_TAILS) && o.line[ln].type == LN_cub) bad = true;
			if (ln == L_FREQ || ln == L_FREQ2) seq = true;
			else if (ln == L_PAN) {
				if (!(vd.plan_len && plan[vd.plan_len - 1].kind == ST_VOICE)) bad = true;
			} else if (ln == L_PMA) { if (!(chain_ok && (o.type == OT_WAVE || (o.type == OT_RASEG && P.chain_early_ok)))) bad = true; }
			else if (ln != L_AMP && ln != L_AMP2) bad = true;
		}
		if (o.type == OT_NOISE && o.wave == NZ_re) { seq = true; has_red = true; }
		if (o.line[L_PMA].v0 != 0.f && !(chain_ok && (o.type == OT_WAVE || (o.type == OT_RASEG && P.chain_early_ok)))) bad = true;
		if (o.type == OT_WAVE) o.ras_level = 0;
		o.rt_fconst_valid = 0;
		o.rt_fblk_valid = 0;
		o.st_phase = 0;
		o.st_prev_phase = 0;
		if (!(o.flags & OPF_TIME_INF) && o.time < min_time) min_time = o.time;
	}
	uint32_t depth = 0, maxd = 0;
	auto extra_of = [&](uint32_t sl) -> uint32_t { return sl == NO_SLOT ? 0u : (uint32_t)a_extra[sl & 255u]; };
	auto set_extra = [&](uint32_t sl, uint32_t x, bool keep_max) {
		if (sl == NO_SLOT) return;
		if (keep_max) { const uint32_t old = extra_of(sl); if (old > x) x = old; }
		a_extra[sl & 255u] = (uint8_t)(x & 7u);
	};
	uint32_t x_carrier = 0;
	for (uint32_t si = 0; si < vd.plan_len && !bad; ++si) {
		const Step st = plan[si];
		DevOp &o = OPS[ids[st.op]];
		if (o.rt_frozen) {
			if (st.flags & SF_BEGIN) ++depth;
			if (st.flags & SF_END) --depth;
			continue;
		}
		if (st.flags & SF_BEGIN) { ++depth; if (depth > maxd) maxd = depth; }
		const bool is_osc = o.type == OT_WAVE || o.type == OT_RASEG;
		const bool freq_here = (st.kind == ST_LINE && st.which == L_FREQ) ||
			(st.kind == ST_OSC && st.freq == NO_SLOT && is_osc);
		if (st.kind == ST_ZERO) bad = true;
		if (st.kind == ST_SMLINE && !(chain_ok && o.type == OT_WAVE)) bad = true;
		if (st.kind == ST_OSC && st.sm != NO_SLOT && !(chain_ok && o.type == OT_WAVE)) bad = true;
		if (step_may_chain(st) && o.type == OT_WAVE &&
		    (st.sm != NO_SLOT || o.line[L_PMA].v0 != 0.f || (o.line[L_PMA].flags & LP_GOAL)))
			has_chain = true;
		if (step_may_chain(st) && o.type == OT_RASEG && !o.rt_frozen &&
		    (st.sm != NO_SLOT || o.line[L_PMA].v0 != 0.f || (o.line[L_PMA].flags & LP_GOAL))) {
			has_chain = true;
			has_rchain = true;
		}
		bool pconst = false; float pf = 0.f;
		if (st.fmul != NO_SLOT && st.fmul >= FSLOT_BASE) {
			const uint32_t ow = block_owner(plan, si, st.fmul);
			if (ow != 0xff) {
				const DevOp &po = OPS[ids[ow]];
				pconst = po.rt_fblk_valid != 0; pf = po.rt_fconst;
			} else if (st.prov != NO_SLOT) {
				const DevOp &po = OPS[ids[st.prov]];
				pconst = po.rt_fconst_valid != 0; pf = po.rt_fconst;
			}
		}
		uint32_t x_step = 0;
		if (st.kind == ST_LERP) x_step = extra_of(st.freq) > extra_of(st.pm) ? extra_of(st.freq) : extra_of(st.pm);
		if ((st.kind == ST_OSC || st.kind == ST_LERP) && st.out != NO_SLOT && st.out >= FSLOT_BASE) {
			const uint32_t ow = block_owner(plan, si, st.out);
			if (ow != 0xff) {
				DevOp &oo = OPS[ids[ow]];
				oo.rt_fblk_valid = 0;
				const uint32_t wd = st.kind == ST_OSC ? depth : depth + 1;
				if (oo.st_phase == 0 || wd < oo.st_phase) oo.st_phase = wd;
			}
		}
		if (st.kind == ST_LINE || freq_here) {
			const LineState &ls = o.line[st.kind == ST_LINE ? st.which : L_FREQ];
			const bool g_ratio = (ls.flags & LP_GOAL_RATIO) != 0, s_ratio = (ls.flags & LP_STATE_RATIO) != 0;
			if (st.fmul != NO_SLOT) {
				if ((ls.flags & LP_GOAL) && g_ratio != s_ratio) {
					const bool parent_const = st.prov != NO_SLOT && OPS[ids[st.prov]].rt_fconst_valid != 0;
					if (!parent_const) bad = true;
				}
				if ((s_ratio || ((ls.flags & LP_GOAL) && g_ratio)) && !pconst) {
					seq = true;
					if (st.fmul >= FSLOT_BASE) {
						const uint32_t ow = block_owner(plan, si, st.fmul);
						const uint32_t wd = ow != 0xff ? OPS[ids[ow]].st_phase : 0u;
						if (wd) {
							const uint32_t need = depth + (op_has_fpm(plan, vd.plan_len, st.op) ? 1u : 0u);
							x_step = (need > wd ? need - wd : 0u) + extra_of(st.fmul);
							if (st.kind == ST_LINE && (st.which == L_FREQ || st.which == L_FREQ2) && (o.st_phase == 0 || wd < o.st_phase))
								o.st_phase = wd;
						}
					}
				}
			}
		}
		if (freq_here && !bad) {
			const LineState &fl = o.line[L_FREQ];
			bool isconst = !(fl.flags & LP_GOAL) && !(st.kind == ST_LINE && (st.flags & SF_FORCE));
			float fc = fl.v0;
			if (st.fmul != NO_SLOT && (fl.flags & LP_STATE_RATIO)) {
				if (pconst) fc = fl.v0 * pf;
				else isconst = false;
			}
			o.rt_fconst = fc;
			o.rt_fconst_valid = isconst ? 1u : 0u;
			o.rt_fblk_valid = (isconst || (st.kind == ST_LINE && (st.flags & SF_FORCE) && !(fl.flags & LP_GOAL) &&
					!((fl.flags & LP_STATE_RATIO) && st.fmul != NO_SLOT && !pconst))) ? 1u : 0u;
			if (!isconst) seq = true;
		}
		if (st.kind == ST_OSC && is_osc && st.freq != NO_SLOT && !o.rt_fconst_valid) seq = true;
		if (st.kind == ST_LINE) {
			if (x_step > 7) bad = true;
			set_extra(st.out, extra_of(st.fmul), false);
			if ((st.which == L_FREQ || st.which == L_FREQ2) && x_step > o.st_prev_phase) o.st_prev_phase = x_step;
		} else if (st.kind == ST_LERP) {
			if (x_step > 7) bad = true;
			set_extra(st.out, x_step, true);
		} else if (st.kind == ST_OSC) {
			uint32_t x = x_step > o.st_prev_phase ? x_step : o.st_prev_phase;
			const uint32_t in[5] = {extra_of(st.freq), extra_of(st.pm), extra_of(st.fpm), extra_of(st.amp), extra_of(st.sm)};
#pragma unroll
			for (int k = 0; k < 5; ++k) if (in[k] > x) x = in[k];
			if (x > 7) bad = true;
			o.st_prev_phase = x;
			if (st.op == vd.carr_local) x_carrier = x;
			if (!(st.which & OX_VOICE)) set_extra(st.out, x, (st.flags & SF_LAYER) != 0 || st.out >= FSLOT_BASE);
		} else if (st.kind == ST_VOICE) {
			const uint32_t x = extra_of(st.out) > extra_of(st.pm) ? extra_of(st.out) : extra_of(st.pm);
			if (x > x_carrier) x_carrier = x;
		}
		if (st.flags & SF_END) --depth;
	}
	bool early = false;
	if (has_chain && !bad) {
		constexpr uint32_t c0 = 1u, c1 = 2u;
		auto dep = [&](uint32_t c, uint32_t sl) -> bool { return sl != NO_SLOT && (a_dep[sl & 255u] & c) != 0; };
		auto set_dep = [&](uint32_t c, uint32_t sl, bool v, bool keep) {
			if (sl == NO_SLOT) return;
			const uint8_t old = a_dep[sl & 255u];
			a_dep[sl & 255u] = v ? (uint8_t)(old | c) : (keep ? old : (uint8_t)(old & ~c));
		};
		for (uint32_t si = 0; si < vd.plan_len && !bad; ++si) {
			const Step st = plan[si];
			const DevOp &o = OPS[ids[st.op]];
			if (o.rt_frozen) continue;
			if (st.kind == ST_LINE) { set_dep(c0, st.out, dep(c0, st.fmul), false); set_dep(c1, st.out, dep(c1, st.fmul), false); }
			else if (st.kind == ST_SMLINE) { set_dep(c0, st.out, false, false); set_dep(c1, st.out, false, false); }
			else if (st.kind == ST_LERP) {
				set_dep(c0, st.out, dep(c0, st.freq) || dep(c0, st.pm), true);
				set_dep(c1, st.out, dep(c1, st.freq) || dep(c1, st.pm), true);
			} else if (st.kind == ST_OSC) {
				const bool in_dep = dep(c0, st.pm) || dep(c0, st.fpm) || dep(c0, st.freq) || dep(c0, st.fmul) || dep(c0, st.sm);
				const bool in_late = dep(c1, st.pm) || dep(c1, st.fpm) || dep(c1, st.freq) || dep(c1, st.fmul) || dep(c1, st.sm);
				const bool chain = step_may_chain(st) && (o.type == OT_WAVE || o.type == OT_RASEG) &&
					(st.sm != NO_SLOT || o.line[L_PMA].v0 != 0.f || (o.line[L_PMA].flags & LP_GOAL));
				uint32_t ls_ = ~0u;
				const bool inl = chain && step_is_chain_inline(P.chain_early_ok != 0, plan, si, ids, OPS, &ls_);
				const bool fvar = (o.type == OT_WAVE || o.type == OT_RASEG) && !o.rt_fconst_valid && !(chain && inl);
				if (chain && o.type == OT_RASEG) {
					if (inl) early = true; else bad = true;
				}
				if (chain && in_late) bad = true;
				else if (chain && in_dep) early = true;
				if (fvar && (dep(c1, st.freq) || dep(c1, st.fmul))) bad = true;
				else if (fvar && (dep(c0, st.freq) || dep(c0, st.fmul))) early = true;
				if (!(st.which & OX_VOICE)) {
					set_dep(c0, st.out, chain || in_dep || dep(c0, st.amp), (st.flags & SF_LAYER) != 0);
					set_dep(c1, st.out, (chain && !inl) || in_late || dep(c1, st.amp), (st.flags & SF_LAYER) != 0);
				}
			}
		}
	}
	uint32_t seq_kind = seq ? 1u : 0u, n_scan_out = 0, levels_out = 0, lvl_bits_out = 0;
	if (seq && !bad) {
		auto level_of = [&](uint32_t sl) -> uint32_t { return sl == NO_SLOT ? 0u : (uint32_t)a_level[sl & 255u]; };
		auto set_level = [&](uint32_t sl, uint32_t lv, bool keep_max) {
			if (sl == NO_SLOT) return;
			if (keep_max) { const uint32_t old = level_of(sl); if (old > lv) lv = old; }
			a_level[sl & 255u] = (uint8_t)(lv & 3u);
		};
		auto max2 = [](uint32_t a, uint32_t b) { return a > b ? a : b; };
		bool multi = true;
		uint32_t n_scan = 0;
		for (uint32_t si = 0; si < vd.plan_len; ++si) {
			const Step st = plan[si];
			DevOp &o = OPS[ids[st.op]];
			if (o.rt_frozen) continue;
			if (st.kind == ST_LINE) {
				set_level(st.out, level_of(st.fmul), false);
			} else if (st.kind == ST_LERP) {
				set_level(st.out, max2(level_of(st.freq), level_of(st.pm)), true);
			} else if (st.kind == ST_OSC) {
				const bool fvar = ((o.type == OT_WAVE || o.type == OT_RASEG) && !o.rt_fconst_valid &&
					!(chain_ok && step_is_chain_acc(st, o))) || (o.type == OT_NOISE && o.wave == NZ_re);
				uint32_t lv = max2(max2(level_of(st.pm), level_of(st.fpm)), max2(level_of(st.amp),
						max2(level_of(st.freq), level_of(st.fmul))));
				if (fvar) {
					const uint32_t mine = 1 + max2(level_of(st.freq), level_of(st.fmul));
					if (mine > P.sum_levels || n_scan >= FAST_MAX_SCAN) multi = false;
					else {
						lvl_bits_out |= mine << (2 * n_scan);
						if (mine > levels_out) levels_out = mine;
						o.rt_fblk_valid = mine;
					}
					++n_scan;
					lv = max2(lv, mine > 3 ? 3u : mine);
				}
				if (!(st.which & OX_VOICE)) set_level(st.out, lv, (st.flags & SF_LAYER) != 0);
			}
		}
		if (P.look && !has_chain && n_scan <= FAST_MAX_SCAN && n_scan <= vd.n_look) {
			seq_kind = 3;
		} else if (multi && P.scan) {
			seq_kind = 2;
			for (uint32_t p = 0; p < levels_out && p < P.sum_levels; ++p) atomicOr(&P.pass_flags[p], 1u);
		}
		n_scan_out = n_scan;
	}
	if (has_red && seq_kind != 3) bad = true;
	(void)has_rchain;
	if (has_rcub && (!P.cub_ok || (seq_kind != 0 && seq_kind != 3) || has_chain)) bad = true;
	if (has_chain && !bad) {
		if (seq_kind == 1) bad = true;
		else {
			seq_kind = 2;
			atomicOr(&P.pass_flags[FAST_MAX_LEVELS + 1], 1u);
		}
	}
	FastInfo fi;
	if (seq || has_chain) ++x_carrier;
	fi.n_chain = has_chain && !bad ? 1u : 0u;
	fi.H = maxd + x_carrier; fi.xlead = x_carrier; fi.bail = 0; fi.n_fsteps = 0; fi.n_pass[0] = fi.n_pass[1] = fi.n_pass[2] = fi.n_pass[3] = 0; fi.seq = seq_kind; fi.cub = has_rcub ? 1u : 0u; fi.early = (early && has_chain && !bad) ? 1u : 0u; fi.n_scan = n_scan_out; fi.levels = levels_out; fi.lvl_bits = lvl_bits_out; fi.tail = 0; fi.tail_stream = 0;
	fi.total = 0;
	if ((seq || has_chain) && !P.seq_enable) bad = true;
	if (!bad && vd.nops <= P.max_ops && vd.plan_len <= P.max_steps && maxd >= 1 && maxd + x_carrier <= P.np / 2)
		fi.total = min(min_time, vd.run_len);
	P.info[v] = fi;
	if (fi.total && seq_kind == 2 && n_scan_out == 0 && P.lean_on) atomicOr(&P.pass_flags[FAST_LEAN_FLAG], 1u);
	else if (fi.total && (seq_kind == 1 || seq_kind == 2)) atomicOr(&P.pass_flags[FAST_MAX_LEVELS + 2], 1u);
	P.fast_done[v] = 0;
	P.repair[(size_t)v * FAST_REPAIR_WORDS] = 0;
	if (fi.total && fi.cub) atomicOr(&P.pass_flags[FAST_CUB_FLAG], 1u);
	if (fi.total && fi.early) atomicOr(&P.pass_flags[FAST_EARLY_FLAG], 1u);
	if (P.split_cf && fi.total) {
		if (seq_kind == 0) P.vlists[atomicAdd(&P.pass_flags[FAST_CF_COUNT], 1u)] = v;
		else if (seq_kind == 3) P.vlists[P.n_voices + atomicAdd(&P.pass_flags[FAST_LK_COUNT], 1u)] = v;
	}
	}
	if (use_lds) {
		__syncthreads();
		constexpr uint32_t Q = sizeof(DevOp) / 16;
		for (uint32_t i = (uint32_t)lane; i < vd.nops * Q; i += 64)
			((uint4 *)&P.ops[gids[i / Q]])[i % Q] = ((const uint4 *)lops)[i];
	}
}
```

### saugns_amd/csrc/k_decode.h

```cpp
struct FastStep {
	uint32_t kind;
	uint32_t out_off, pm_off, fpm_off, amp_off, aux_off;
	uint32_t type;
	uint32_t inc, phase0, prev_phase;
	float fc, ac, diff_scale, diff_offset;
	int32_t tab;
	uint32_t gop;
	double prev_Is;
	float pan;
	uint32_t ramp;
};
static_assert(sizeof(FastStep) == 80, "FastStep is 20 dwords");

struct FastLine {
	Sweep sw;
	uint32_t goal_len;
	float hold;
	uint32_t pad;
};
static_assert(sizeof(FastLine) == 48, "FastLine is 12 dwords");

enum : uint32_t {
	CM_BASE = 0,
	CM_INC = 1,
	CM_INLINE = 2,
};
enum : uint32_t { CL_FCONST = 1, CL_MUL_GOAL = 2, CL_MUL_HOLD = 4, CL_EARLY = 8 ,
	CL_RASEG = 16  };
struct ChainDesc {
	uint32_t n;
	uint32_t gop;
	uint32_t wave_mode;
	uint32_t row;
	float coeff;
	uint32_t inc_const;
	uint32_t lflags;
	float mulc;
	FastLine fl;
	FastLine pl;
};
static_assert(sizeof(ChainDesc) == 4 * CHAIN_DESC_WORDS && offsetof(ChainDesc, n) == 0, "ChainDesc is 32 dwords, n first");
__device__ __forceinline__ uint32_t chain_wave_id(const ChainDesc &c) { return c.wave_mode & 0xffu; }
__device__ __forceinline__ uint32_t chain_mode(const ChainDesc &c) { return c.wave_mode >> 8; }

enum : uint32_t {
	FA_FVAR_SLOT = 1u << 0,
	FA_FVAR_LINE = 1u << 1,
	FA_MUL_GOAL = 1u << 2,
	FA_MUL_HOLD = 1u << 3,
};
struct FastAux {
	uint32_t freq_off, fmul_off;
	float coeff;
	uint32_t flags;
	float mulc;
	uint32_t pad[3];
	FastLine fl;
};
static_assert(sizeof(FastAux) == 80, "FastAux is 20 dwords");


typedef const uint32_t __attribute__((address_space(4))) *const_u32_ptr;
#ifndef FK_COMMON
#define FK_COMMON 1
#endif
#ifndef FK_CONSTD
#define FK_CONSTD 1
#endif
#ifndef FK_PREFETCH
#define FK_PREFETCH 0
#endif
__device__ __forceinline__ FastLine load_line_uniform(const FastLine *p) {
	const_u32_ptr q = (const_u32_ptr)(uintptr_t)p;
	union { FastLine s; uint32_t u[12]; } c;
#pragma unroll
	for (int i = 0; i < 12; ++i) c.u[i] = q[i];
	return c.s;
}
__device__ __forceinline__ FastAux load_aux_uniform(const FastAux *p) {
	const_u32_ptr q = (const_u32_ptr)(uintptr_t)p;
	union { FastAux s; uint32_t u[20]; } c;
#pragma unroll
	for (int i = 0; i < 20; ++i) c.u[i] = q[i];
	return c.s;
}
__device__ __forceinline__ float fast_line_value(const FastLine &fl, int t) {
	const uint32_t i = (uint32_t)t;
	return i < fl.goal_len ? sweep_value_inl<true>(fl.sw, i) : fl.hold;
}

__global__ void __launch_bounds__(64) scan_kernel(FastParams P) {
	const uint32_t v = blockIdx.x;
	const int l = threadIdx.x;
	if (P.pass_flags[P.mode - 1] == 0) return;
	const FastInfo fi = P.info[v];
	if (fi.seq != 2 || fi.total == 0) return;
	const uint32_t C = 64u - fi.H;
	const uint32_t nrows = (fi.total + C - 1) / C;
	const uint32_t ngroups = (nrows + P.rows_multi - 1) / P.rows_multi;
	for (uint32_t x = 0; x < fi.n_scan && x < FAST_MAX_SCAN; ++x) {
		if (((fi.lvl_bits >> (2 * x)) & 3u) != P.mode) continue;
		unsigned long long *a = P.scan + ((size_t)v * FAST_MAX_SCAN + x) * P.scan_groups;
		unsigned long long carry = 0;
		for (uint32_t base = 0; base < ngroups; base += 64) {
			const bool in = base + (uint32_t)l < ngroups;
			const unsigned long long val = in ? a[base + l] : 0ull;
			const unsigned long long incl = wave_incl_scan64_dpp(val);
			if (in) a[base + l] = carry + (incl - val);
			carry += readlane64(incl, 63);
		}
	}
}

__global__ void __launch_bounds__(64) decode_kernel(FastParams P) {
	const uint32_t v = blockIdx.x;
	const int l = threadIdx.x;
	if (P.info[v].total == 0) return;
	const bool lean = P.lean_on && P.info[v].seq == 2 && P.info[v].n_scan == 0;
	const uint32_t NP = 64 * (P.info[v].cub ? FAST_CUB_ROWS : lean ? P.rows_lean : (P.info[v].seq == 1 || P.info[v].seq == 2) ? P.rows_multi :
		(P.split_cf && P.info[v].seq == 0) ? P.rows_cf : P.rows);
	const VoiceDesc vd = P.voices[v];
	const uint32_t *ids = P.op_ids + vd.ops_ofs;
	bool keep = false;
	FastStep f;
	FastLine fl, pl;
	FastAux fa;
	memset(&f, 0, sizeof f); memset(&fl, 0, sizeof fl); memset(&fa, 0, sizeof fa); memset(&pl, 0, sizeof pl);
	bool is_chain = false, chain_line = false, chain_inline = false;
	uint32_t dep = 0;
	const uint32_t seq = P.info[v].seq;
	if ((uint32_t)l < vd.plan_len) {
		const Step *plan = P.steps + vd.plan_ofs;
		for (uint32_t q = 0; q <= (uint32_t)l; ++q) {
			const Step sq = plan[q];
			if (sq.flags & SF_BEGIN) ++dep;
			if (q < (uint32_t)l && (sq.flags & SF_END)) --dep;
		}
		const Step st = plan[l];
		const DevOp &o = P.ops[ids[st.op]];
		keep = !(st.kind == ST_LINE && st.which == L_FREQ && o.rt_fconst_valid);
		is_chain = step_is_chain(st, o);
		const uint32_t st_which = st.kind == ST_SMLINE ? (uint32_t)L_PMA : (uint32_t)st.which;
		bool zero_fill = false;
		if (o.rt_frozen) {
			bool root_end = false;
			if (st.kind == ST_OSC && (st.flags & SF_END)) {
				uint32_t d2 = 0, frozen_at = 0;
				for (uint32_t q = 0; q <= (uint32_t)l; ++q) {
					const Step sq = plan[q];
					const DevOp &oq = P.ops[ids[sq.op]];
					if (sq.flags & SF_BEGIN) {
						++d2;
						if (!frozen_at && !(oq.flags & OPF_TIME_INF) && oq.time == 0) frozen_at = d2;
					}
					if (q == (uint32_t)l) root_end = (d2 == frozen_at);
					if (sq.flags & SF_END) { if (d2 == frozen_at) frozen_at = 0; --d2; }
				}
			}
			zero_fill = root_end && !(st.flags & SF_LAYER) && !(st.which & OX_VOICE);
			keep = zero_fill;
		}
		const uint32_t eff_dep = dep + P.info[v].xlead - min(P.ops[ids[st.op]].st_prev_phase, P.info[v].xlead);
		f.kind = (uint32_t)(st.kind == ST_SMLINE ? (uint8_t)ST_LINE : st.kind) | ((uint32_t)st.flags << 8) | (st_which << 16) | (eff_dep << 24);
		const FastIds cs = P.fast_ids[(seq ? P.ids_full_ofs : 0u) + vd.plan_ofs + l];
		f.out_off = cs.out != NO_SLOT ? (uint32_t)cs.out * NP : ~0u;
		f.pm_off = cs.pm != NO_SLOT ? (uint32_t)cs.pm * NP : ~0u;
		f.fpm_off = cs.fpm != NO_SLOT ? (uint32_t)cs.fpm * NP : ~0u;
		f.amp_off = cs.amp != NO_SLOT ? (uint32_t)cs.amp * NP : ~0u;
		f.aux_off = cs.aux != NO_SLOT ? (uint32_t)cs.aux * NP : ~0u;
		if (st.kind == ST_OSC) f.aux_off = cs.sm != NO_SLOT ? (uint32_t)cs.sm * NP : ~0u;
		const uint32_t wv = o.type == OT_WAVE ? (o.wave < 12 ? o.wave : 0) : o.wave;
		f.type = o.type | (wv << 8) | ((o.flags & OPF_OSC_RESET) ? 1u << 16 : 0u);
		f.fc = o.rt_fconst;
		f.inc = rint32w(o.coeff * o.rt_fconst);
		f.phase0 = o.type == OT_NOISE ? o.noise_n : o.phase;
		f.prev_phase = o.type == OT_NOISE ? o.noise_prev : o.prev_phase;
		f.ac = (st.kind == ST_LINE || st.kind == ST_SMLINE) ? o.line[st_which].v0 : o.line[L_AMP].v0;
		f.diff_scale = o.type == OT_WAVE ? P.wc[wv].diff_scale : 0.f;
		f.diff_offset = o.type == OT_WAVE ? P.wc[wv].diff_offset : 0.f;
		f.tab = o.type == OT_WAVE ? P.tab_of_wave[wv] : -1;
		f.gop = ids[st.op];
		f.prev_Is = o.prev_Is;
		if (o.type == OT_RASEG) {
			const bool rate2x = (o.flags & OPF_RATE2X) != 0;
			const unsigned long long inc64 = (unsigned long long)rint64((rate2x ? o.coeff * 2 : o.coeff) * o.rt_fconst);
			f.inc = (uint32_t)inc64;
			f.prev_phase = (uint32_t)(inc64 >> 32);
			f.prev_Is = __longlong_as_double((long long)o.cycle_phase);
			f.tab = (int32_t)((o.ras_func & 0xff) | ((o.ras_flags & 0xffff) << 8) | ((o.wave & 0x7f) << 24));
			f.diff_scale = bits_f(o.ras_level);
			f.diff_offset = bits_f(o.ras_alpha);
			f.type |= rate2x ? 1u << 17 : 0u;
			if (P.info[v].cub && (vd.flags & VD_TAILS) && o.wave == LN_cub && !o.rt_frozen) {
				uint32_t rem = (vd.flags & VD_MORE) ? TAIL_FAR : min(vd.run_len, TAIL_FAR);
				uint32_t closed = 0;
				for (uint32_t q = (uint32_t)l + 1; q-- > 0;) {
					const Step sq = plan[q];
					if (q != (uint32_t)l && (sq.flags & SF_END)) ++closed;
					if (sq.flags & SF_BEGIN) {
						if (closed) --closed;
						else {
							const DevOp &oa = P.ops[ids[sq.op]];
							if (!(oa.flags & OPF_TIME_INF) && oa.time < rem) rem = oa.time;
						}
					}
				}
				f.type |= FT_CUBTAIL;
				f.phase0 = rem;
			}
		}
		f.pan = o.line[L_PAN].v0;
		f.ramp = 0;
		if (o.type == OT_AMP) f.fc = 1.f;
		if (is_chain && !zero_fill) {
			uint32_t k = 0;
			for (uint32_t q = 0; q < (uint32_t)l; ++q) if (step_may_chain(plan[q])) ++k;
			const uint32_t row = vd.chain_base + k;
			f.type |= FT_CHAIN;
			f.pan = bits_f(row);
			ChainDesc cd;
			memset(&cd, 0, sizeof cd);
			cd.n = P.info[v].total; cd.gop = ids[st.op]; cd.row = row;
			uint32_t cmode = step_is_chain_acc(st, o) ? CM_INC : CM_BASE;
			if (st.sm == NO_SLOT) {
				LineState pls = o.line[L_PMA];
				const LineBlock lb = line_begin(pls, P.info[v].total, false, 0.f, lattice_none(), 0);
				pl.sw = lb.sw; pl.goal_len = lb.goal_len; pl.hold = lb.hold; pl.pad = 0;
				chain_line = true;
			}
			uint32_t lstep = ~0u;
			if (step_is_chain_inline(P.chain_inline != 0 || P.info[v].early != 0, plan, (uint32_t)l, ids, P.ops, &lstep)) {
				chain_inline = true;
				cmode = CM_INLINE;
				if (P.info[v].early) { cd.lflags |= CL_EARLY; f.type |= FT_CHAIN_EARLY; }
				if (o.type == OT_RASEG) cd.lflags |= CL_RASEG;
				cd.coeff = o.coeff;
				cd.pl = pl;
				cd.mulc = 1.f;
				if (o.rt_fconst_valid) {
					cd.lflags |= CL_FCONST;
					cd.inc_const = rint32w(o.coeff * o.rt_fconst);
				} else {
					const Step ls = lstep != ~0u ? plan[lstep] : st;
					const bool have_mul = ls.fmul != NO_SLOT;
					float pf = 1.f;
					if (have_mul && ls.prov != NO_SLOT) pf = P.ops[ids[ls.prov]].rt_fconst;
					LineState fls = o.line[L_FREQ];
					const LineBlock lb = line_begin(fls, P.info[v].total, have_mul, pf, lattice_none(), 0);
					cd.fl.sw = lb.sw; cd.fl.goal_len = lb.goal_len; cd.fl.hold = lb.hold; cd.fl.pad = 0;
					if (lb.mul_goal) cd.lflags |= CL_MUL_GOAL;
					if (lb.mul_hold) cd.lflags |= CL_MUL_HOLD;
					cd.mulc = pf;
				}
			}
			cd.wave_mode = (wv & 0xffu) | (cmode << 8);
			P.chain_desc[vd.chain_slot + k] = cd;
		}
		if (st.kind == ST_OSC && o.type == OT_WAVE && !zero_fill && !is_chain && st.pm == NO_SLOT && st.fpm == NO_SLOT &&
		    o.rt_fconst_valid && f.inc == 0 && ((o.flags & OPF_OSC_RESET) || o.prev_phase == o.phase)) {
			float held = o.prev_s;
			double Is0 = o.prev_Is;
			uint32_t pprev = o.prev_phase;
			if (o.flags & OPF_OSC_RESET) {
				const HerpC23 *g23 = P.g_c23 + (size_t)wv * WAVE_LEN;
				const HerpC01 *g01 = P.g_c01 + (size_t)wv * WAVE_LEN;
				const uint32_t pa = o.phase, pb = o.phase - SLEN;
				Is0 = herp_poly(g23[pa >> SLEN_BITS], g01[pa >> SLEN_BITS], pa);
				held = wosc_reset_s(Is0, herp_poly_rise(g23[pb >> SLEN_BITS], g01[pb >> SLEN_BITS], pb), g01[pb >> SLEN_BITS].c0,
						P.wc[wv].diff_scale, P.wc[wv].diff_offset);
				pprev = pa;
			}
			DevOp &ow = P.ops[ids[st.op]];
			ow.st_phase = o.phase; ow.st_prev_phase = pprev; ow.st_prev_Is = Is0; ow.st_prev_s = held;
			f.type = OT_AMP;
			f.fc = held;
		}
		if (zero_fill) {
			f.kind = (uint32_t)ST_LINE | ((uint32_t)L_AMP << 16) | (dep << 24);
			f.ac = 0.f;
			f.ramp = ((4u << FAST_MAX_LEVELS) - 4u) | FR_CHAIN_IN;
		} else {
			const bool line_step = st.kind == ST_LINE || st.kind == ST_SMLINE;
			const bool amp_inline = st.kind == ST_OSC && st.amp == NO_SLOT;
			const bool have_mul = st.fmul != NO_SLOT;
			bool pconst = false; float pf = 1.f;
			if (have_mul && st.prov != NO_SLOT) {
				const DevOp &po = P.ops[ids[st.prov]];
				pconst = po.rt_fconst_valid != 0; pf = po.rt_fconst;
			}
			fa.freq_off = ~0u; fa.fmul_off = ~0u; fa.coeff = o.coeff; fa.flags = 0; fa.mulc = 1.f;
			fa.pad[0] = fa.pad[1] = fa.pad[2] = 0;
			fa.fl.goal_len = 0; fa.fl.hold = 0.f; fa.fl.pad = 0;
			fa.fl.sw = sweep_setup(LN_sah, 0.f, 0.f, 0, 1);
			LineState ls = o.line[line_step ? st_which : L_AMP];
			if (line_step || amp_inline) {
				if (ls.flags & LP_GOAL) {
					const LineBlock lb = line_begin(ls, P.info[v].total, line_step && have_mul, pconst ? pf : 1.f, lattice_none(), 0);
					fl.sw = lb.sw; fl.goal_len = lb.goal_len; fl.hold = lb.hold; fl.pad = 0;
					f.ramp = 1;
					if (lb.mul_goal) fa.flags |= FA_MUL_GOAL;
					if (lb.mul_hold) fa.flags |= FA_MUL_HOLD;
				} else if (line_step && have_mul && (ls.flags & LP_STATE_RATIO)) {
					fa.flags |= FA_MUL_HOLD;
				}
				if (fa.flags & (FA_MUL_GOAL | FA_MUL_HOLD)) {
					if (pconst) fa.mulc = pf; else fa.fmul_off = cs.fmul != NO_SLOT ? (uint32_t)cs.fmul * NP : ~0u;
					f.ramp |= 2;
				}
			}
			const bool is_osc = o.type == OT_WAVE || o.type == OT_RASEG;
			if (seq == 2) {
				unsigned long long want[FAST_MAX_LEVELS];
				bool mine[FAST_MAX_LEVELS];
				for (uint32_t p = 0; p < FAST_MAX_LEVELS; ++p) { want[p] = 0; mine[p] = false; }
				unsigned long long want_c = 0;
				bool mine_c = false;
				bool ran_full = false;
				unsigned long long want_f = 0;
				bool mine_f = false;
				uint32_t xi = 0;
				for (uint32_t q = vd.plan_len; q-- > 0;) {
					const Step sq = plan[q];
					const DevOp &oq = P.ops[ids[sq.op]];
					if (oq.rt_frozen) continue;
					if (sq.kind == ST_LINE && sq.which == L_FREQ && oq.rt_fconst_valid) continue;
					const FastIds cq = P.fast_ids[P.ids_full_ofs + vd.plan_ofs + q];
					auto bit = [](uint8_t id) -> unsigned long long { return id != NO_SLOT ? 1ull << id : 0ull; };
					const bool q_fvar = sq.kind == ST_OSC && (oq.type == OT_WAVE || oq.type == OT_RASEG) && !oq.rt_fconst_valid &&
						!step_is_chain_acc(sq, oq);
					const uint32_t q_level = q_fvar ? oq.rt_fblk_valid : 0u;
					if (q_fvar && q < (uint32_t)l) ++xi;
					const bool writes = sq.kind == ST_LINE || sq.kind == ST_LERP || sq.kind == ST_SMLINE ||
						(sq.kind == ST_OSC && !(sq.which & OX_VOICE));
					const bool rmw = sq.kind == ST_LERP || (sq.kind == ST_OSC && (sq.flags & SF_LAYER));
					const bool v_early = P.info[v].early != 0;
					const bool q_chain = step_is_chain(sq, oq);
					uint32_t q_ls = ~0u;
					const bool q_inline = q_chain && step_is_chain_inline(P.chain_inline != 0 || v_early, plan, q, ids, P.ops, &q_ls);
					const bool q_early = q_inline && v_early;
					{
						bool needed = false;
						if (q_inline) {
							if (v_early && writes && (want_c & bit(cq.out))) {
								needed = true;
								if (!rmw) want_c &= ~bit(cq.out);
								want_c |= bit(cq.amp);
							}
						} else if (q_chain) {
							needed = true;
							want_c |= bit(cq.freq) | bit(cq.fmul) | bit(cq.pm) | bit(cq.fpm) | bit(cq.sm);
						} else if (writes && (want_c & bit(cq.out))) {
							needed = true;
							if (!rmw) want_c &= ~bit(cq.out);
							want_c |= bit(cq.pm) | bit(cq.fpm) | bit(cq.amp) | bit(cq.aux) | bit(cq.freq) | bit(cq.fmul) | bit(cq.sm);
						}
						if (q == (uint32_t)l) mine_c = needed;
						bool needed_f = sq.kind == ST_VOICE || (sq.kind == ST_OSC && (sq.which & OX_VOICE));
						if (!needed_f && writes && (want_f & bit(cq.out))) {
							needed_f = true;
							if (!rmw) want_f &= ~bit(cq.out);
						}
						const bool q_saved = q_fvar && seq == 2 && P.inc_rows && vd.n_inc && sq.fpm == NO_SLOT && !q_chain;
						if (needed_f) {
							if (sq.kind == ST_VOICE) want_f |= bit(cq.out) | bit(cq.pm);
							else if (q_chain) want_f |= bit(cq.amp);
							else if (q_saved) want_f |= bit(cq.pm) | bit(cq.amp) | bit(cq.aux) | bit(cq.sm);
							else want_f |= bit(cq.pm) | bit(cq.fpm) | bit(cq.amp) | bit(cq.aux) | bit(cq.freq) | bit(cq.fmul) | bit(cq.sm);
						}
						if (q == (uint32_t)l) mine_f = needed_f;
					}
					for (uint32_t p = 0; p < FAST_MAX_LEVELS; ++p) {
						bool needed = false;
						if (q_early) {
							if (writes && (want[p] & bit(cq.out))) {
								needed = true;
								if (!rmw) want[p] &= ~bit(cq.out);
								want[p] |= bit(cq.amp);
							}
						} else if (q_fvar && q_level == p + 1) {
							needed = true;
							want[p] |= bit(cq.freq) | bit(cq.fmul);
						} else if (!(q_fvar && q_level > p + 1)) {
							if (writes && (want[p] & bit(cq.out))) {
								needed = true;
								if (!rmw) want[p] &= ~bit(cq.out);
								want[p] |= bit(cq.pm) | bit(cq.fpm) | bit(cq.amp) | bit(cq.aux) | bit(cq.freq) | bit(cq.fmul);
							}
						}
						if (q == (uint32_t)l) {
							mine[p] = needed;
							if (needed && !(q_fvar && q_level == p + 1) && p < P.sum_levels) ran_full = true;
						}
					}
				}
				for (uint32_t p = 0; p < FAST_MAX_LEVELS; ++p) if (mine[p]) f.ramp |= 4u << p;
				if (mine_c) f.ramp |= FR_CHAIN_IN;
				if (!mine_f && (mine_c || ran_full || st.kind == ST_LINE || st.kind == ST_SMLINE || st.kind == ST_LERP))
					f.ramp |= FR_FINAL_SKIP;
				fa.pad[1] = (o.type == OT_WAVE || o.type == OT_RASEG) && !o.rt_fconst_valid && !step_is_chain_acc(st, o) ? o.rt_fblk_valid : 0u;
				fa.pad[0] = xi;
			}
			const bool is_red = o.type == OT_NOISE && o.wave == NZ_re;
			if (seq == 3 && st.kind == ST_OSC && ((is_osc && !o.rt_fconst_valid) || is_red)) {
				uint32_t xi = 0;
				for (uint32_t q = 0; q < (uint32_t)l; ++q) {
					const Step sq = plan[q];
					const DevOp &oq = P.ops[ids[sq.op]];
					if (oq.rt_frozen) continue;
					if (sq.kind == ST_OSC && (((oq.type == OT_WAVE || oq.type == OT_RASEG) && !oq.rt_fconst_valid) ||
					                          (oq.type == OT_NOISE && oq.wave == NZ_re))) ++xi;
				}
				fa.pad[0] = xi; fa.pad[1] = 0;
				if (is_red) f.ramp |= 2;
			}
			if (st.kind == ST_OSC && is_osc && !o.rt_fconst_valid) {
				if (st.freq != NO_SLOT) {
					fa.flags |= FA_FVAR_SLOT;
					fa.freq_off = cs.freq != NO_SLOT ? (uint32_t)cs.freq * NP : ~0u;
				} else {
					LineState fls = o.line[L_FREQ];
					const LineBlock lb = line_begin(fls, P.info[v].total, have_mul, pconst ? pf : 1.f, lattice_none(), 0);
					fa.fl.sw = lb.sw; fa.fl.goal_len = lb.goal_len; fa.fl.hold = lb.hold;
					fa.flags |= FA_FVAR_LINE;
					if (lb.mul_goal) fa.flags |= FA_MUL_GOAL;
					if (lb.mul_hold) fa.flags |= FA_MUL_HOLD;
					if (fa.flags & (FA_MUL_GOAL | FA_MUL_HOLD)) {
						if (pconst) fa.mulc = pf; else fa.fmul_off = cs.fmul != NO_SLOT ? (uint32_t)cs.fmul * NP : ~0u;
					}
				}
				f.ramp |= 2;
				if (step_is_chain_acc(st, o)) fa.pad[2] = 1;
				else if (seq == 2 && P.inc_rows && vd.n_inc && st.fpm == NO_SLOT && !is_chain) {
					uint32_t k = 0;
					for (uint32_t q = 0; q < (uint32_t)l; ++q) {
						const Step sq = plan[q];
						const uint32_t tq = P.ops[ids[sq.op]].type;
						if (sq.kind == ST_OSC && (tq == OT_WAVE || tq == OT_RASEG)) ++k;
					}
					if (k < vd.n_inc) fa.pad[2] = 2u | ((vd.inc_base + k) << 8);
				}
			}
		}
	}
	{
		bool lost = false;
		if ((uint32_t)l < vd.plan_len && seq) {
			const Step st = P.steps[vd.plan_ofs + l];
			const FastIds cs = P.fast_ids[P.ids_full_ofs + vd.plan_ofs + l];
			const DevOp &o = P.ops[ids[st.op]];
			if (keep && st.kind == ST_LINE && st.which == L_FREQ && cs.out == NO_SLOT) lost = true;
			if (keep && st.kind == ST_LINE && (st.which == L_FREQ2 || st.which == L_AMP2) && cs.out == NO_SLOT)
				keep = false;
			if (keep && st.kind == ST_LERP && st.freq != NO_SLOT && cs.aux == NO_SLOT) {
				bool found = false;
				for (uint32_t q = (uint32_t)l; q-- > 0;) {
					const Step sq = P.steps[vd.plan_ofs + q];
					if (sq.out != st.freq) continue;
					if (sq.kind == ST_LINE && (sq.which == L_FREQ2 || sq.which == L_AMP2)) {
						const DevOp &oq = P.ops[ids[sq.op]];
						const LineState &ls = oq.line[sq.which];
						float c = ls.v0;
						bool pc = true;
						if (sq.fmul != NO_SLOT && (ls.flags & LP_STATE_RATIO)) {
							pc = sq.prov != NO_SLOT && P.ops[ids[sq.prov]].rt_fconst_valid != 0;
							if (pc) c *= P.ops[ids[sq.prov]].rt_fconst;
							else {
								for (uint32_t r = q; r-- > 0;) {
									const Step sr = P.steps[vd.plan_ofs + r];
									if (sr.out != sq.fmul) continue;
									if (sr.kind == ST_LINE && sr.which == L_FREQ) {
										const DevOp &po = P.ops[ids[sr.op]];
										const LineState &pls = po.line[L_FREQ];
										pc = !(pls.flags & LP_GOAL) && (sr.fmul == NO_SLOT || !(pls.flags & LP_STATE_RATIO) ||
										                                (sr.prov != NO_SLOT && P.ops[ids[sr.prov]].rt_fconst_valid != 0));
										if (pc) c *= po.rt_fconst;
									}
									break;
								}
							}
						}
						found = pc && !(ls.flags & LP_GOAL);
						f.fc = c;
					}
					break;
				}
				if (!found) lost = true;
			}
			if (keep && st.kind == ST_OSC && (o.type == OT_WAVE || o.type == OT_RASEG) && !o.rt_fconst_valid && st.freq != NO_SLOT && cs.freq == NO_SLOT) lost = true;
			if (keep && (f.ramp & 2) && fa.fmul_off == ~0u && (fa.flags & (FA_MUL_GOAL | FA_MUL_HOLD)) && fa.mulc == 1.f && st.fmul != NO_SLOT && cs.fmul == NO_SLOT) {
				bool pc = false;
				if (st.prov != NO_SLOT) pc = P.ops[ids[st.prov]].rt_fconst_valid != 0;
				if (!pc) lost = true;
			}
		}
		if (__any(lost)) {
			if (l == 0) { P.info[v].total = 0; P.info[v].bail = 1; }
			keep = false;
		}
	}
#pragma unroll
	for (uint32_t li = 0; li < FAST_LISTS; ++li) {
		bool in;
		if (li == 0) in = keep && !(f.ramp & FR_FINAL_SKIP);
		else if (li == 4) in = keep && seq == 2 && (f.ramp & FR_CHAIN_IN);
		else in = keep && seq == 2 && (f.ramp & (2u << li));
		const unsigned long long m = __ballot(in);
		if (in) {
			const uint32_t pos = (uint32_t)__popcll(m & ((1ull << l) - 1ull));
			const size_t at = ((size_t)li * P.n_voices + v) * P.max_steps + pos;
			P.fsteps[at] = f;
			if (f.ramp & 1) P.flines[at] = fl;
			if (f.ramp & 2) P.faux[at] = fa;
			if (chain_line && P.fplines) P.fplines[at] = pl;
		}
		if (l == 0) { if (li == 0) P.info[v].n_fsteps = (uint32_t)__popcll(m); else P.info[v].n_pass[li - 1] = (uint32_t)__popcll(m); }
	}
	const unsigned long long mc = __ballot(is_chain && keep && !chain_inline);
	if (l == 0) P.info[v].n_chain = (uint32_t)__popcll(mc);
}
```

### saugns_amd/csrc/launch_plan.h

```cpp
#ifndef SAU_LAUNCH_PLAN_H
#define SAU_LAUNCH_PLAN_H

#include "engine.h"
#include "sau_dev_math.h"
#include <string.h>

namespace sauplan {

using namespace saudev;
using sauengine::SegmentDesc;

#ifndef FK_GRID
#define FK_GRID 256
#endif
constexpr uint32_t FAST_TAB_BYTES = (uint32_t)(WAVE_LEN * (sizeof(HerpC23) + sizeof(HerpC01))), FAST_TAB_BYTES_WIDE = 65536u;
constexpr uint32_t FAST_MAX_SCAN = 8;
constexpr uint32_t LOOK_LDS_BYTES = FAST_MAX_SCAN * 2 * 64 * sizeof(unsigned long long);
constexpr uint32_t FAST_MAX_LEVELS = 3;
constexpr uint32_t FAST_CUB_ROWS = 4;
constexpr uint32_t FAST_LISTS = 5;
constexpr uint32_t INMIX_NSMALL = 8;
#ifndef SAU_CHAIN_BATCH_FRAMES
#define SAU_CHAIN_BATCH_FRAMES 32
#endif
constexpr uint32_t CHAIN_BATCH = SAU_CHAIN_BATCH_FRAMES;
constexpr uint32_t CHAIN_IO_WORDS = CHAIN_BATCH * 64;
constexpr uint32_t CHAIN_TAB_BYTES = 65536, CHAIN_TAB_C01 = 32768;
constexpr size_t CHAIN_IO_BYTES = (size_t)(2 * 2 + 2) * CHAIN_IO_WORDS * 4;
constexpr size_t MISC_BYTES = 1488;
constexpr size_t BLOCK_TAB_BYTES = (size_t)WAVE_LEN * (sizeof(HerpC23) + sizeof(HerpC01));

struct Tuning {
	int geo = 1;
	uint32_t multi_min = 256;
	uint32_t multi_teams = 16;
	uint32_t fk_grid = 0;
	bool lds_limit_set = false;
	size_t lds_limit = 0;
	bool fast = true;
	bool seq = true;
	bool two_pass = true;
	bool lookback = true;
	bool inc_rows = true;
	uint32_t fast_rows = 8;
	uint32_t look_rows = 8;
	uint32_t look_min_voices = 1;
	bool look_no_lds = false, look_withhold = false, look_spread = false;
	bool wide_tabs = true;
	bool wide_look = true;
	uint32_t more_rows = 12;
	bool repair = true;
	bool analyze_lds = true;
	bool chain = true;
	bool chain_inline = true;
	bool chain_early = true;
	uint32_t chain_chunks = 0;
	uint32_t chain_chunk_frames = 16384;
	bool short_last_chunk = true;
	bool chain_alone = false;
	bool lean = true;
	uint32_t lean_rows = 6;
	bool dyn = true;
	uint32_t dyn_groups = 12;
	uint32_t dyn_floor = 24;
	uint32_t dyn_min_tasks = 2;
	bool xcd_queues = true;
	bool inmix = true;
	uint32_t inmix_min_voices = 64;
	uint32_t inmix_min_steps = 2;
	bool inmix_taper = false;
	uint32_t inmix_at = 13;
	bool inmix_dry = false;
	bool inner = true;
	bool lanemajor = true;
	bool duo = true;
	uint32_t duo_lw = 0, duo_prio = 0;
	bool tailmix = false;
	bool mix_few = true;
	bool early_mix = true;
	bool mix64 = true;
	bool poison = false;
};

inline Tuning tuning_from_env(const char *(*env)(const char *)) {
	Tuning t;
	auto off = [&](const char *name) { return env(name) == nullptr; };
	auto num = [&](const char *name, uint32_t &v) { if (const char *s = env(name)) v = (uint32_t)atoi(s); };
	auto at_least_1 = [&](const char *name, uint32_t &v) { if (const char *s = env(name)) { const int n = atoi(s); v = n >= 1 ? (uint32_t)n : 1u; } };
	const char *wt = env("SAU_AMD_GEOMETRY");
	t.geo = (wt && !strcmp(wt, "8x2")) ? 0 : 1;
	if (const char *mm = env("SAU_AMD_MULTI_MIN")) t.multi_min = (uint32_t)atol(mm);
	if (const char *mt = env("SAU_AMD_MULTI_TEAMS")) t.multi_teams = atoi(mt) == 8 ? 8u : 16u;
	if (const char *fg = env("SAU_AMD_FK_GRID")) { const int n = atoi(fg); if (n >= 1 && n <= (int)FK_GRID) t.fk_grid = (uint32_t)n; }
	if (const char *ll = env("SAU_AMD_LDS_LIMIT")) { t.lds_limit_set = true; t.lds_limit = (size_t)atol(ll); }
	t.fast = off("SAU_AMD_NO_FAST");
	t.seq = off("SAU_AMD_NO_SEQ");
	t.two_pass = off("SAU_AMD_NO_TWO_PASS");
	t.lookback = off("SAU_AMD_NO_LOOKBACK");
	t.inc_rows = off("SAU_AMD_NO_INC_ROWS");
	if (const char *fr = env("SAU_AMD_FAST_ROWS")) {
		const int r = atoi(fr);
		t.fast_rows = r >= 8 ? 8 : r >= 6 ? 6 : r >= 5 ? 5 : r >= 4 ? 4 : 2;
	}
	num("SAU_AMD_LOOK_ROWS", t.look_rows);
	num("SAU_AMD_LOOK_MIN_VOICES", t.look_min_voices);
	t.look_no_lds = !off("SAU_AMD_LOOK_NO_LDS");
	t.look_withhold = !off("SAU_AMD_LOOK_WITHHOLD");
	t.look_spread = !off("SAU_AMD_LOOK_SPREAD");
	t.wide_tabs = off("SAU_AMD_NO_WIDE_TABS");
	t.wide_look = off("SAU_AMD_NO_WIDE_LOOK");
	num("SAU_AMD_MORE_ROWS", t.more_rows);
	t.repair = off("SAU_AMD_NO_REPAIR");
	t.analyze_lds = off("SAU_AMD_ANALYZE_NO_LDS");
	t.chain = off("SAU_AMD_NO_CHAIN");
	t.chain_inline = off("SAU_AMD_NO_CHAIN_INLINE");
	t.chain_early = off("SAU_AMD_NO_EARLY_CHAINS");
	if (const char *cc = env("SAU_AMD_CHAIN_CHUNKS")) {
		const int n = atoi(cc);
		t.chain_chunks = n >= 32 ? 32 : n >= 1 ? (uint32_t)n : 1;
	}
	if (const char *cf = env("SAU_AMD_CHAIN_CHUNK_FRAMES")) { const int n = atoi(cf); if (n >= 4096) t.chain_chunk_frames = (uint32_t)n; }
	t.short_last_chunk = off("SAU_AMD_NO_SHORT_LAST_CHUNK");
	if (const char *ca = env("SAU_AMD_CHAIN_ALONE")) t.chain_alone = atoi(ca) != 0;
	t.lean = off("SAU_AMD_NO_LEAN");
	num("SAU_AMD_LEAN_ROWS", t.lean_rows);
	t.dyn = off("SAU_AMD_NO_DYN");
	at_least_1("SAU_AMD_DYN_GROUPS", t.dyn_groups);
	at_least_1("SAU_AMD_DYN_FLOOR", t.dyn_floor);
	at_least_1("SAU_AMD_DYN_MIN_TASKS", t.dyn_min_tasks);
	t.xcd_queues = off("SAU_AMD_NO_XCD_QUEUES");
	t.inmix = off("SAU_AMD_NO_INMIX");
	num("SAU_AMD_INMIX_MIN_VOICES", t.inmix_min_voices);
	num("SAU_AMD_INMIX_MIN_STEPS", t.inmix_min_steps);
	t.inmix_taper = !off("SAU_AMD_INMIX_TAPER");
	if (const char *ia = env("SAU_AMD_INMIX_AT")) t.inmix_at = (uint32_t)atoi(ia) & 15u;
	t.inmix_dry = !off("SAU_AMD_INMIX_DRY");
	t.inner = off("SAU_AMD_NO_INNER");
	t.lanemajor = off("SAU_AMD_NO_LANEMAJOR");
	t.duo = off("SAU_AMD_NO_DUO");
	if (const char *lw = env("SAU_AMD_DUO_LW")) t.duo_lw = (uint32_t)atoi(lw) & 15u;
	if (const char *pr = env("SAU_AMD_DUO_PRIO")) t.duo_prio = (uint32_t)atoi(pr) & 7u;
	t.tailmix = !off("SAU_AMD_TAILMIX");
	t.mix_few = off("SAU_AMD_NO_MIX_FEW");
	t.early_mix = off("SAU_AMD_NO_EARLY_MIX");
	t.mix64 = off("SAU_AMD_NO_MIX64");
	t.poison = !off("SAU_AMD_POISON");
	return t;
}

struct DeviceLimits {
	size_t lds_limit = 160 * 1024;
	uint32_t fk_grid = FK_GRID;
	uint32_t cus = 256;
	bool eight_xcds = true;
};
inline DeviceLimits device_limits(size_t lds_per_cu, uint32_t cus, const Tuning &t) {
	DeviceLimits d;
	d.cus = cus;
	d.eight_xcds = cus == 256;
	d.fk_grid = t.fk_grid ? t.fk_grid : cus < FK_GRID ? cus : FK_GRID;
	d.lds_limit = t.lds_limit_set ? t.lds_limit : lds_per_cu > 160 * 1024 ? (size_t)160 * 1024 : lds_per_cu;
	return d;
}

struct PlanInputs {
	uint32_t row_stride = 0;
	size_t pcm_row = 0;
	size_t chain_budget = 0;
	bool f32 = false;
	uint32_t max_write = 0;
	uint32_t max_rows = 0;
};

struct TableMap {
	uint32_t n = 0;
	int8_t tab_of_wave[12];
	uint8_t wave_of_tab[12];
};
inline TableMap map_tables(uint64_t wave_mask, size_t max_tabs) {
	TableMap m;
	memset(m.wave_of_tab, 0, sizeof m.wave_of_tab);
	for (int wv = 0; wv < 12; ++wv) {
		m.tab_of_wave[wv] = -1;
		if (((wave_mask >> wv) & 1) && m.n < max_tabs) {
			m.tab_of_wave[wv] = (int8_t)m.n;
			m.wave_of_tab[m.n] = (uint8_t)wv;
			++m.n;
		}
	}
	return m;
}
inline size_t tabs_that_fit(size_t limit, size_t fixed, size_t tab_bytes) { return fixed > limit ? 0 : (limit - fixed) / tab_bytes; }
inline uint32_t n_waves_used(uint64_t wave_mask) { return (uint32_t)__builtin_popcountll(wave_mask & 0xffffffffull); }

inline size_t buf_area(uint32_t n_bufs, uint32_t rows, uint32_t fmax_steps) {
	return (size_t)n_bufs * 64 * rows * sizeof(float) + (size_t)fmax_steps * sizeof(unsigned long long);
}
inline bool fits_lds(const DeviceLimits &d, size_t n_tabs, size_t tab_bytes, size_t area, size_t extra = 0) {
	return n_tabs * tab_bytes + 16 * area + extra + 1024 <= d.lds_limit;
}
inline uint32_t row_groups(uint32_t len, uint32_t rows) { return (len + (60 * rows) - 1) / (60 * rows); }
inline uint32_t wave_grid(unsigned long long waves, uint32_t max_grid) {
	const unsigned long long g = (waves + 15) / 16;
	return g > max_grid ? max_grid : g < 1 ? 1u : (uint32_t)g;
}
inline uint32_t group_grid(uint32_t n_voices, uint32_t groups, uint32_t max_grid) {
	return wave_grid((unsigned long long)n_voices * (groups < 64 ? groups : 64), max_grid);
}
inline uint32_t fewer_rows(uint32_t t) { return t > 6 ? 6u : t > 5 ? 5u : t > 4 ? 4u : 2u; }
inline uint32_t rows_at_most(uint32_t r) { return r >= 8 ? 8u : r >= 6 ? 6u : r >= 5 ? 5u : r >= 4 ? 4u : 2u; }

struct BlockLoopPlan {
	bool ok = true;
	uint32_t W = 4, T = 4, V = 1;
	bool HB = false;
	size_t team_bytes = 0, lds = 0;
	TableMap tabs;
	uint32_t grid(const SegmentDesc &seg, bool use_fast) const {
		const bool all = seg.maybe_block || !use_fast;
		if (V > 1) {
			const uint32_t full = (seg.n_voices + V - 1) / V;
			return all ? (full < 512 ? full : 512) : 2;
		}
		return all ? (seg.n_voices < 1024 ? seg.n_voices : 1024) : 16;
	}
};
inline BlockLoopPlan plan_block_loop(const SegmentDesc &seg, const Tuning &tun, const DeviceLimits &dev) {
	BlockLoopPlan p;
	p.W = tun.geo ? 4 : 8; p.T = tun.geo ? 4 : 2;
	auto team_size = [&](uint32_t w, uint32_t t) {
		size_t b = p.HB ? MISC_BYTES + 64
			: (size_t)w * 64 * t * sizeof(float) * seg.n_slots + (size_t)seg.max_ops * sizeof(DevOp) +
			MISC_BYTES + (size_t)seg.max_steps * sizeof(Step) + 64;
		return (b + 15) & ~(size_t)15;
	};
	if (tun.multi_min && seg.n_voices >= tun.multi_min && (seg.serial || tun.multi_min == 1)) {
		const size_t need_tab = seg.wave_mask ? BLOCK_TAB_BYTES : 0;
		const uint32_t mt = tun.multi_teams;
		for (uint32_t t : {4u, 3u, 2u, 1u})
			if (mt * team_size(1, t) + need_tab <= dev.lds_limit) { p.W = 1; p.T = t; p.V = mt; break; }
	}
	if (p.V == 1 && team_size(p.W, p.T) > dev.lds_limit) { p.W = 1; p.T = 1; }
	if (p.V == 1 && p.W == 1 && team_size(1, 1) > dev.lds_limit) p.HB = true;
	p.team_bytes = team_size(p.W, p.T);
	const size_t fixed = p.team_bytes * p.V;
	if (fixed > dev.lds_limit) { p.ok = false; return p; }
	size_t budget = dev.lds_limit / 2 > fixed ? dev.lds_limit / 2 - fixed : 0;
	if (p.V > 1) budget = dev.lds_limit - fixed;
	if (budget < BLOCK_TAB_BYTES && dev.lds_limit - fixed >= BLOCK_TAB_BYTES) budget = BLOCK_TAB_BYTES;
	p.tabs = map_tables(seg.wave_mask, budget / BLOCK_TAB_BYTES);
	p.lds = p.tabs.n * BLOCK_TAB_BYTES + fixed;
	return p;
}

struct ChainChunks {
	uint32_t n = 1;
	uint32_t cb[34];
	bool short_last = false;
};
inline ChainChunks chain_chunk_bounds(uint32_t len, const Tuning &tun) {
	ChainChunks k;
	uint32_t n = tun.chain_chunks ? tun.chain_chunks : (len + tun.chain_chunk_frames - 1) / tun.chain_chunk_frames;
	if (n > 32) n = 32;
	while (n > 1 && len / n < 4096) --n;
	if (n < 1) n = 1;
	k.short_last = !tun.chain_chunks && tun.short_last_chunk && n >= 4 && n < 32 && len > 8 * 4096u;
	const uint32_t tail = k.short_last ? 4096u : 0u;
	const uint32_t body = tail ? (len - tail) & ~255u : len;
	const uint32_t clen0 = ((body + n - 1) / n + 255) & ~255u;
	for (uint32_t c = 0; c <= n; ++c) k.cb[c] = (unsigned long long)c * clen0 < body ? c * clen0 : body;
	if (tail) { ++n; k.cb[n] = len; }
	uint32_t m = 0;
	for (uint32_t c = 0; c < n; ++c)
		if (k.cb[c + 1] > k.cb[c]) { k.cb[m] = k.cb[c]; ++m; k.cb[m] = k.cb[c + 1]; }
	if (m) n = m;
	k.n = n;
	return k;
}

struct Tasks { uint32_t dyn_chunks = 0, dyn_static = 0, dyn_small = 0; };
inline uint32_t task_groups(const SegmentDesc &seg, const Tuning &tun) {
	const uint32_t S = seg.max_steps ? seg.max_steps : 1;
	uint32_t G = tun.dyn_groups;
	if (G * S < tun.dyn_floor) G = (tun.dyn_floor + S - 1) / S;
	return G;
}
inline Tasks plan_tasks(const SegmentDesc &seg, const Tuning &tun, uint32_t n_groups, uint32_t grid) {
	Tasks q;
	const uint32_t waves = grid * 16;
	const uint32_t G = task_groups(seg, tun);
	const uint32_t k_dyn = (n_groups + G - 1) / G;
	if (tun.dyn && (unsigned long long)seg.n_voices * k_dyn >= (unsigned long long)tun.dyn_min_tasks * waves) {
		q.dyn_chunks = k_dyn ? k_dyn : 1;
		q.dyn_static = 0;
	} else {
		uint32_t k = waves / seg.n_voices;
		if (k > n_groups) k = n_groups;
		q.dyn_chunks = k ? k : 1;
		q.dyn_static = 1;
	}
	return q;
}
inline Tasks static_tasks(const SegmentDesc &seg, uint32_t n_groups, uint32_t grid) {
	Tasks q;
	uint32_t k = grid * 16 / seg.n_voices;
	if (k > n_groups) k = n_groups;
	q.dyn_chunks = k ? k : 1; q.dyn_static = 1;
	return q;
}
struct MagicDiv { uint32_t m = 0, s = 0; };
inline MagicDiv magic_div(uint32_t d) {
	MagicDiv q;
	while ((1ull << q.s) < d) ++q.s;
	q.m = (uint32_t)(((1ull << (32 + q.s)) / d) + 1ull - (1ull << 32));
	return q;
}
inline uint32_t magic_quotient(uint32_t q, MagicDiv d) {
	if (d.s == 0) return q;
	const uint32_t t = (uint32_t)(((unsigned long long)q * d.m) >> 32);
	return (t + ((q - t) >> 1)) >> (d.s - 1);
}

enum Inner : uint32_t { INNER_NONE = 0, INNER_ROW_MAJOR = 1, INNER_LANE_MAJOR = 2 };
enum Mixer : uint32_t { MIX_NONE = 0, MIX_FEW_F32, MIX_F32, MIX_FEW, MIX_64, MIX_256 };

struct FastPlan {
	bool use_fast = false;
	bool seq_ok = false;
	bool look_split = false;
	int main_build = 0;
	uint32_t fmax_steps = 0, n_fast = 0, n_fast_cf = 0;
	uint32_t rows = 2;
	uint32_t rows_multi = 2;
	uint32_t rows_cf = 2;
	uint32_t rows_lean = 4;
	bool lean_on = false;
	TableMap tabs;
	uint32_t n_want = 0;
	bool wide_cf = false;
	bool wide_look = false;
	bool cub_ok = false;
	uint32_t sum_levels = 2;
	uint32_t scan_groups = 0;
	bool scan = false;
	bool look = false;
	size_t look_words = 0;
	bool look_words_real = false;
	uint32_t look_wpv = 1;
	bool look_inside = true;
	uint32_t look_wpv_flags = 0;
	bool inc_rows = false;
	uint32_t inc_stride = 0;
	bool chains = false;
	uint32_t chain_stride = 0, chain_grid = 0;
	TableMap ctabs;
	ChainChunks chunks;
	uint32_t pass_grid = 0;
	bool early_mix = false;
	bool split_cf = false, duo = false, tailmix = false;
	bool queues = false;
	bool inmix = false;
	uint32_t inmix_flags = 0;
	MagicDiv div;
	Inner inner = INNER_NONE;
	Tasks tasks, tasks_cf, tasks_cub;
	uint32_t groups = 0, groups_cf = 0;
	uint32_t grid = 1, grid_cf = 1, grid_look = 1, grid_edge = 1, grid_cub = 1, grid_repair = 1;
	uint32_t rows_repair = 2;

	void drop_chains() { chains = false; lean_on = false; }
	size_t launch_lds(int build, uint32_t r, bool wide, bool cf = false) const {
		return tabs.n * (size_t)(wide ? FAST_TAB_BYTES_WIDE : FAST_TAB_BYTES) + 16 * buf_area(cf ? n_fast_cf : n_fast, r, fmax_steps) +
			(build == 2 ? LOOK_LDS_BYTES : 0);
	}
	size_t inner_lds() const {
		return inner == INNER_LANE_MAJOR ? tabs.n * (size_t)FAST_TAB_BYTES_WIDE : launch_lds(0, rows, true);
	}
};

inline void plan_rows(FastPlan &p, const SegmentDesc &seg, const Tuning &tun, const DeviceLimits &dev) {
	p.fmax_steps = seg.max_steps < 64 ? seg.max_steps : 64;
	uint32_t FT = tun.fast_rows;
	p.look_split = tun.seq && seg.may_scan && tun.two_pass && tun.lookback && tun.look_rows != 0 && seg.n_voices >= tun.look_min_voices;
	if (tun.seq && seg.may_scan && FT > 4 && !p.look_split) FT = 4;
	if (p.look_split && FT > tun.look_rows) FT = rows_at_most(tun.look_rows);
	p.seq_ok = tun.seq && seg.may_scan;
	p.n_fast = p.seq_ok && seg.n_fast_full > seg.n_fast ? seg.n_fast_full : seg.n_fast;
	p.n_fast_cf = seg.n_fast;
	p.n_want = n_waves_used(seg.wave_mask);
	auto area_of = [&](uint32_t t) { return buf_area(p.n_fast, t, p.fmax_steps); };
	const size_t look_lds = p.look_split ? LOOK_LDS_BYTES : 0;
	while (FT > 2 && !fits_lds(dev, seg.wave_mask ? 1 : 0, FAST_TAB_BYTES, area_of(FT), look_lds)) FT = fewer_rows(FT);
	{
		uint32_t t = FT;
		while (t > 4 && !fits_lds(dev, p.n_want, FAST_TAB_BYTES, area_of(t), look_lds)) t = fewer_rows(t);
		if (fits_lds(dev, p.n_want, FAST_TAB_BYTES, area_of(t), look_lds)) FT = t;
	}
	p.use_fast = tun.fast && fits_lds(dev, 0, 0, area_of(FT), look_lds);
	p.rows = FT;
	p.rows_multi = FT > 4 && p.seq_ok ? 4 : FT;
	p.tabs = map_tables(seg.wave_mask, p.use_fast ? tabs_that_fit(dev.lds_limit, 16 * area_of(FT) + look_lds + 1024, FAST_TAB_BYTES) : 0);
	const uint32_t ft = p.tabs.n;
	const bool all_wide_ok = tun.wide_tabs && tun.more_rows && ft > 0 && ft == p.n_want && seg.max_steps >= 2;
	if (p.use_fast && !p.seq_ok && all_wide_ok && FT == 8)
		for (uint32_t t : {12u, 10u})
			if (t <= tun.more_rows && fits_lds(dev, ft, FAST_TAB_BYTES_WIDE, area_of(t))) { p.rows = p.rows_multi = t; break; }
	p.split_cf = p.use_fast && p.seq_ok && p.look_split;
	auto area_cf = [&](uint32_t t) { return buf_area(p.n_fast_cf, t, p.fmax_steps); };
	p.rows_cf = 2;
	if (p.split_cf) {
		for (uint32_t t : {8u, 6u, 5u, 4u})
			if (t <= tun.fast_rows && fits_lds(dev, ft, FAST_TAB_BYTES, area_cf(t))) { p.rows_cf = t; break; }
		if (p.rows_cf == 8 && all_wide_ok)
			for (uint32_t t : {12u, 10u})
				if (t <= tun.more_rows && fits_lds(dev, ft, FAST_TAB_BYTES_WIDE, area_cf(t))) { p.rows_cf = t; break; }
	}
	p.cub_ok = p.use_fast && seg.maybe_cub && fits_lds(dev, ft, FAST_TAB_BYTES, area_cf(FAST_CUB_ROWS)) &&
		(!p.look_split || fits_lds(dev, ft, FAST_TAB_BYTES, area_of(FAST_CUB_ROWS), LOOK_LDS_BYTES));
	p.rows_lean = 4;
	for (uint32_t t : {6u, 5u})
		if (t <= tun.fast_rows && t <= tun.lean_rows && fits_lds(dev, ft, FAST_TAB_BYTES, area_of(t))) { p.rows_lean = t; break; }
	p.main_build = !p.seq_ok ? 0 : p.look_split ? 2 : 1;
	auto wide_fits = [&](uint32_t rows, size_t area) {
		return tun.wide_tabs && (rows == 8 || rows == 6 || rows == 10 || rows == 12) && ft > 0 && ft == p.n_want && seg.max_steps >= 2 &&
			fits_lds(dev, ft, FAST_TAB_BYTES_WIDE, area);
	};
	p.wide_cf = p.main_build == 2 ? wide_fits(p.rows_cf, area_cf(p.rows_cf)) : p.main_build == 0 && wide_fits(p.rows, area_of(p.rows));
	p.wide_look = tun.wide_tabs && tun.wide_look && p.rows == 8 && ft > 0 && ft == p.n_want &&
		fits_lds(dev, ft, FAST_TAB_BYTES_WIDE, area_of(p.rows), LOOK_LDS_BYTES);
	p.sum_levels = seg.sum_levels >= FAST_MAX_LEVELS ? FAST_MAX_LEVELS : 2u;
}

inline void plan_sums(FastPlan &p, const SegmentDesc &seg, const Tuning &tun, const DeviceLimits &dev) {
	if (p.seq_ok && tun.two_pass) {
		p.scan_groups = seg.len / (32 * p.rows_multi) + 2;
		p.scan = !p.look_split || seg.n_chain_rows;
		p.look = p.look_split && seg.n_look_rows;
	}
	if (p.look) {
		const uint32_t groups = row_groups(seg.len, p.rows);
		unsigned long long wpv = ((unsigned long long)dev.fk_grid * 16) / seg.n_voices;
		if (wpv > 64) wpv = 64;
		if (wpv > groups) wpv = groups;
		if (wpv < 1) wpv = 1;
		auto is_inside = [&](unsigned long long w) { return w <= 16 && (16 % w) == 0 && !tun.look_no_lds; };
		p.look_words = (size_t)seg.n_look_rows * 2 * p.scan_groups;
		p.look_words_real = p.look_words * sizeof(unsigned long long) <= ((size_t)1 << 30);
		if (!p.look_words_real && !is_inside(wpv) && !tun.look_no_lds)
			wpv = wpv > 16 ? 16 : wpv > 8 ? 8 : wpv > 4 ? 4 : 2;
		p.look_wpv = (uint32_t)wpv;
		p.look_inside = !p.look_words_real && is_inside(wpv);
	}
	p.inc_stride = (seg.len + 63) & ~63u;
	p.inc_rows = tun.inc_rows && p.use_fast && p.scan && seg.n_inc_rows && seg.len <= sauengine::CHAIN_SEG &&
		(size_t)seg.n_inc_rows * 2 * p.inc_stride * sizeof(uint32_t) <= ((size_t)1 << 30);
}

inline void plan_chains(FastPlan &p, const SegmentDesc &seg, const Tuning &tun, const DeviceLimits &dev, const PlanInputs &in) {
	p.chains = tun.chain && p.use_fast && p.scan && seg.serial && seg.n_chain_rows &&
		seg.len <= sauengine::chain_seg_frames(seg.n_chain_rows, in.chain_budget);
	p.chain_stride = (seg.len + 63) & ~63u;
	p.ctabs = map_tables(seg.wave_mask, tabs_that_fit(dev.lds_limit, CHAIN_IO_BYTES + 1024, CHAIN_TAB_BYTES));
	p.lean_on = p.chains && tun.lean &&
		fits_lds(dev, p.tabs.n, FAST_TAB_BYTES, buf_area(p.n_fast, p.rows_lean, p.fmax_steps));
	p.chain_grid = (seg.n_chain_slots + 63) / 64;
	if (p.chains) p.chunks = chain_chunk_bounds(seg.len, tun);
	p.pass_grid = p.chunks.n > 1 && p.grid + p.chain_grid > dev.fk_grid ? (dev.fk_grid > p.chain_grid + 32 ? dev.fk_grid - p.chain_grid : 32) : p.grid;
	p.early_mix = tun.early_mix && in.max_write && !p.cub_ok && !(tun.mix_few && in.max_rows <= 8 && seg.n_streams >= 8);
}

inline void plan_split(FastPlan &p, const SegmentDesc &seg, const Tuning &tun, const DeviceLimits &dev, const PlanInputs &in) {
	const uint32_t ft = p.tabs.n;
	p.tailmix = p.look && p.rows == 8 && tun.tailmix && !in.f32 && in.max_write && !p.cub_ok && seg.len < (1u << 30) &&
		tun.mix_few && in.max_rows <= 8 && seg.n_streams >= 8 && (seg.pcm_offset & 3u) == 0 && (in.pcm_row & 3u) == 0;
	p.groups_cf = row_groups(seg.len, p.rows_cf);
	p.grid_cf = group_grid(seg.n_voices, p.groups_cf, dev.fk_grid);
	p.duo = tun.duo && p.look && p.look_words_real && p.rows == 8 && p.rows_cf == 8 && !p.cub_ok && !p.tailmix &&
		!p.wide_look && !p.wide_cf && fits_lds(dev, ft, FAST_TAB_BYTES, buf_area(p.n_fast, p.rows, p.fmax_steps), LOOK_LDS_BYTES);
	p.tasks_cf = plan_tasks(seg, tun, p.groups_cf, p.duo ? (dev.fk_grid + 1) / 2 : p.grid_cf);
	p.look_wpv_flags = (tun.look_no_lds ? 1u : 0u) | (tun.look_withhold ? 2u : 0u) | (tun.look_spread ? 4u : 0u);
	if (p.duo) p.look_wpv_flags |= (tun.duo_lw << 8) | (tun.duo_prio << 12);
	p.grid_look = wave_grid((unsigned long long)seg.n_voices * (p.look_words_real ? (p.groups < 64 ? p.groups : 64) : p.look_wpv), dev.fk_grid);
}

inline void plan_closed_form(FastPlan &p, const SegmentDesc &seg, const Tuning &tun, const DeviceLimits &dev, const PlanInputs &in) {
	if (p.main_build == 0) p.tasks = plan_tasks(seg, tun, p.groups, p.grid);
	p.queues = tun.xcd_queues && dev.eight_xcds && p.main_build == 0 && !p.tasks.dyn_static && p.tasks.dyn_chunks >= 16 && !p.cub_ok;
	if (p.queues) {
		p.inmix_flags = 64u;
		if (tun.inmix_taper) {
			const uint32_t G = task_groups(seg, tun);
			const uint32_t small = G / 4 ? G / 4 : 1;
			if (p.groups >= 32 * G + INMIX_NSMALL * small) {
				p.tasks.dyn_small = small;
				p.tasks.dyn_chunks = (p.groups - INMIX_NSMALL * small + G - 1) / G + INMIX_NSMALL;
			}
		}
		p.div = magic_div(seg.n_voices);
		p.inmix = tun.inmix && !in.f32 && seg.n_streams == 1 && in.max_write && seg.n_voices >= tun.inmix_min_voices &&
			seg.max_steps >= tun.inmix_min_steps && in.row_stride < (1u << 24);
		if (p.inmix)
			p.inmix_flags = 64u | 32u | (seg.stereo ? 1u : 0u) | (seg.swap_bytes ? 2u : 0u) | (tun.inmix_dry ? 4u : 0u) | ((tun.inmix_at & 15u) << 8);
	}
	if (tun.inner && p.main_build == 0 && p.wide_cf && p.rows == 12 && p.tasks.dyn_chunks >= 3)
		p.inner = tun.lanemajor && p.n_fast == 1 ? INNER_LANE_MAJOR : INNER_ROW_MAJOR;
	p.grid_edge = wave_grid(2ull * seg.n_voices, dev.fk_grid);
}

inline FastPlan plan_fast(const SegmentDesc &seg, const Tuning &tun, const DeviceLimits &dev, const PlanInputs &in) {
	FastPlan p;
	plan_rows(p, seg, tun, dev);
	plan_sums(p, seg, tun, dev);
	p.groups = row_groups(seg.len, p.rows);
	p.grid = group_grid(seg.n_voices, p.groups, dev.fk_grid);
	plan_chains(p, seg, tun, dev, in);
	if (p.use_fast && p.main_build == 2) plan_split(p, seg, tun, dev, in);
	if (p.use_fast && !p.scan) plan_closed_form(p, seg, tun, dev, in);
	const uint32_t g4 = row_groups(seg.len, FAST_CUB_ROWS);
	p.grid_cub = group_grid(seg.n_voices, g4, dev.fk_grid);
	p.tasks_cub = static_tasks(seg, g4, p.grid_cub);
	p.rows_repair = p.main_build == 2 ? p.rows_cf : p.rows;
	p.grid_repair = wave_grid(seg.n_voices, 64);
	return p;
}

inline Mixer plan_mixer(const SegmentDesc &seg, const Tuning &tun, const PlanInputs &in, size_t pcm_pitch, bool inmix_live,
		uint32_t early_blocks) {
	if (!in.max_write) return MIX_NONE;
	const bool few = tun.mix_few && in.max_rows <= 8 && seg.n_streams >= 8;
	const bool few_f32_aligned = (pcm_pitch & 15u) == 0 && (seg.pcm_offset & (seg.stereo ? 1u : 3u)) == 0;
	if (in.f32) return few && few_f32_aligned ? MIX_FEW_F32 : MIX_F32;
	if (few && (seg.pcm_offset & 3u) == 0 && (in.pcm_row & 3u) == 0) return MIX_FEW;
	if (inmix_live && !early_blocks && tun.mix64) return MIX_64;
	return MIX_256;
}

constexpr uint32_t LEVELS_THREADS = 256;
constexpr uint32_t LEVELS_SWEEP_F32 = LEVELS_THREADS * 4, LEVELS_SWEEP_S16 = LEVELS_THREADS * 8;
constexpr uint32_t LEVELS_WG_SAMPLES = 16384;
static_assert(LEVELS_WG_SAMPLES % LEVELS_SWEEP_S16 == 0 && LEVELS_WG_SAMPLES % LEVELS_SWEEP_F32 == 0, "a block is whole sweeps (and begins on an even sample, on 16 bytes)");
constexpr uint32_t LEVELS_MAX_ROWS = 65535;
struct LevelsPlan {
	bool ok = false;
	uint32_t blocks = 0;
	uint32_t rows = 0;
	uint32_t finish_grid = 0;
	size_t parts = 0;
};
inline LevelsPlan plan_levels(uint64_t max_frames, uint32_t channels, size_t n_rows) {
	LevelsPlan p;
	const uint64_t samples = max_frames * channels;
	const uint64_t blocks = (samples + LEVELS_WG_SAMPLES - 1) / LEVELS_WG_SAMPLES;
	if (n_rows > LEVELS_MAX_ROWS || blocks > 0x7fffffffull || max_frames > (~(uint64_t)0 >> 2)) return p;
	p.ok = true;
	p.blocks = (uint32_t)blocks;
	p.rows = (uint32_t)n_rows;
	p.finish_grid = (uint32_t)((n_rows + 63) / 64);
	p.parts = (size_t)n_rows * (size_t)blocks;
	return p;
}

constexpr uint32_t DECIM_THREADS = 64, DECIM_PER_LANE = 4;
constexpr uint32_t DECIM_TILE = 256;
static_assert(DECIM_TILE == DECIM_THREADS * DECIM_PER_LANE, "a lane's frames are DECIM_THREADS apart");
constexpr uint32_t DECIM_HALF = (uint32_t)sauengine::DECIM_HALF;
constexpr uint32_t DECIM_SPAN_Q = DECIM_TILE + 2 * DECIM_HALF;
constexpr uint32_t DECIM_CARRY_THREADS = 256;
constexpr uint32_t DECIM_MAX_STREAMS = 65535;
struct DecimPlan {
	bool ok = false;
	uint32_t tiles = 0;
	uint32_t streams = 0;
	uint32_t taps = 0;
	uint32_t hist_floats = 0;
	uint32_t lds_bytes = 0;
	size_t out_pitch = 0;
};
inline DecimPlan plan_decimate(uint64_t buf_len, int factor, uint32_t channels, size_t n_streams, size_t sample_bytes) {
	DecimPlan p;
	if ((factor != 2 && factor != 4 && factor != 8) || (channels != 1 && channels != 2) || n_streams > DECIM_MAX_STREAMS) return p;
	const uint64_t tiles = (buf_len + DECIM_TILE - 1) / DECIM_TILE;
	if (tiles > 0x7fffffffull || buf_len * (uint64_t)factor > 0xffffffffull) return p;
	p.ok = true;
	p.tiles = (uint32_t)tiles;
	p.streams = (uint32_t)n_streams;
	p.taps = 2 * DECIM_HALF * (uint32_t)factor + 1;
	p.hist_floats = (p.taps - 1) * channels;
	p.lds_bytes = DECIM_SPAN_Q * (uint32_t)factor * channels * (uint32_t)sizeof(float);
	p.out_pitch = ((size_t)buf_len * channels * sample_bytes + 255) & ~(size_t)255;
	return p;
}
static_assert(2 * DECIM_HALF * 8 * 2 <= DECIM_CARRY_THREADS * 4, "decimate_carry_kernel: a stream's longest history, four floats per thread");

}
#endif
```

Before: 246.4 million.

## Fuse analyze and decode kernels into a single per-voice prologue kernel

The separate analyze and decode kernels are merged into one prologue kernel. Lane 0 analyzes the voice into shared memory, then all 64 lanes decode the steps, reading ops and the plan from the LDS copies instead of global memory, and the ops are written back once at the end. This removes one kernel launch and a round trip of per-voice info and op state through global memory. The render sequence is also reorganized as a planned stage list. Decode now runs inside the prologue even when the fast path is off; it returns early when the voice total is zero.

Result: no change. 246.8 million (median of 6 runs) (+0.2%).

```diff
diff --git a/saugns_amd/build.py b/saugns_amd/build.py
--- a/saugns_amd/build.py
+++ b/saugns_amd/build.py
@@ -8,7 +8,7 @@
 SOURCES = ["capi.cpp", "engine.cpp", "plan.cpp", "tables.cpp", "program_io.cpp", "sndout.cpp", "bank_builder.cpp",
            "hip_backend.hip"]
 HEADERS = ["engine.h", "hip_backend.h", "capi_internal.h", "sau_dev_math.h", "sau_dev_ops.h", "launch_plan.h",
-           "k_common.h", "k_wave_scan.h", "k_block_loop.h", "k_fast_types.h", "k_analyze.h", "k_decode.h", "k_fast_voice.h", "k_fast_group.h", "k_fast_group_lm.h",
+           "k_common.h", "k_wave_scan.h", "k_block_loop.h", "k_fast_types.h", "k_analyze.h", "k_decode.h", "k_prologue.h", "k_fast_voice.h", "k_fast_group.h", "k_fast_group_lm.h",
            "k_chain.h", "k_finish.h", "k_levels.h", "k_decimate.h",
            "sau_dev_types.h", "../../include/sau_abi.h", "../../include/saugns_amd.h"]
 FLAGS = ["--offload-arch=gfx950", "-O3", "-ffp-contract=off", "-fPIC", "-std=c++17",
diff --git a/saugns_amd/csrc/hip_backend.hip b/saugns_amd/csrc/hip_backend.hip
--- a/saugns_amd/csrc/hip_backend.hip
+++ b/saugns_amd/csrc/hip_backend.hip
@@ -25,6 +25,7 @@
 #include "k_fast_types.h"
 #include "k_analyze.h"
 #include "k_decode.h"
+#include "k_prologue.h"
 #include "k_fast_voice.h"
 #include "k_chain.h"
 #include "k_finish.h"
@@ -472,19 +473,26 @@
 		j.fk = plan_fast(seg, tun_, lim_, j.in);
 		if (!prepare_fast(j, err) || !prepare_chains(j, err)) return false;
 		fill_tables(j);
-		if (!launch_analyze(j, err)) return false;
-		if (j.fk.use_fast) {
-			if (!launch_decode(j, err)) return false;
-			if (j.fk.main_build == 2 && !launch_split(j, err)) return false;
-			if (j.fp.scan ? !launch_sums_and_chains(j, err) : !launch_closed_form(j, err)) return false;
-			if (!launch_cub(j, err)) return false;
-			if (!j.launched) return false;
-			if (!launch_repair(j, err)) return false;
-			if (j.tf) (void)hipEventRecord(j.tf->b, stream_);
-		}
-		if (!launch_finalize(j, err)) return false;
-		if (!launch_block_loop(j, err)) return false;
-		return launch_mixer(j, err);
+		Stage stages[MAX_STAGES];
+		const uint32_t n_stages = plan_stages(j.fk, stages);
+		for (uint32_t i = 0; i < n_stages; ++i) {
+			switch (stages[i]) {
+			case STAGE_PROLOGUE: if (!launch_prologue(j, err)) return false; break;
+			case STAGE_SPLIT: if (!launch_split(j, err)) return false; break;
+			case STAGE_SUMS_CHAINS: if (!launch_sums_and_chains(j, err)) return false; break;
+			case STAGE_CLOSED_FORM: if (!launch_closed_form(j, err)) return false; break;
+			case STAGE_CUB: if (!launch_cub(j, err)) return false; break;
+			case STAGE_REPAIR:
+				if (!j.launched) return false;
+				if (!launch_repair(j, err)) return false;
+				if (j.tf) (void)hipEventRecord(j.tf->b, stream_);
+				break;
+			case STAGE_FINALIZE: if (!launch_finalize(j, err)) return false; break;
+			case STAGE_BLOCK_LOOP: if (!launch_block_loop(j, err)) return false; break;
+			case STAGE_MIXER: if (!launch_mixer(j, err)) return false; break;
+			}
+		}
+		return true;
 	}
 
 	bool ensure_rows(Job &j, std::string &err) {
@@ -640,20 +648,16 @@
 		j.fp.n_tabs = j.fk.tabs.n;
 	}
 
-	bool launch_analyze(Job &j, std::string &err) {
+	bool launch_prologue(Job &j, std::string &err) {
 		const SegmentDesc &seg = j.seg;
-		(void)err;
 		TimedPair *ta = timing_on_ ? new_pair(3) : nullptr;
 		if (ta) (void)hipEventRecord(ta->a, stream_);
 		uint32_t lo = seg.max_ops, ls = seg.max_steps;
 		size_t albytes = (size_t)lo * sizeof(DevOp) + (size_t)ls * sizeof(Step) + (size_t)lo * sizeof(uint32_t);
 		if (albytes > 48 * 1024 || !tun_.analyze_lds) { lo = 0; ls = 0; albytes = 0; }
-		hipLaunchKernelGGL(analyze_kernel, dim3(seg.n_voices), dim3(64), albytes, stream_, j.fp, lo, ls);
+		hipLaunchKernelGGL(prologue_kernel, dim3(seg.n_voices), dim3(64), albytes, stream_, j.fp, lo, ls);
 		if (ta) (void)hipEventRecord(ta->b, stream_);
-		return true;
-	}
-	bool launch_decode(Job &j, std::string &err) {
-		hipLaunchKernelGGL(decode_kernel, dim3(j.seg.n_voices), dim3(64), 0, stream_, j.fp);
+		if (!j.fk.use_fast) return true;
 		if (!wait_for_predecessor(err)) return false;
 		j.tf = timing_on_ ? new_pair(2) : nullptr;
 		if (j.tf) (void)hipEventRecord(j.tf->a, stream_);
diff --git a/saugns_amd/csrc/k_analyze.h b/saugns_amd/csrc/k_analyze.h
--- a/saugns_amd/csrc/k_analyze.h
+++ b/saugns_amd/csrc/k_analyze.h
@@ -52,38 +52,11 @@
 	return false;
 }
 
-__global__ void __launch_bounds__(64) analyze_kernel(FastParams P, uint32_t lds_ops, uint32_t lds_steps) {
-	extern __shared__ __align__(16) unsigned char a_lds[];
-	const uint32_t v = blockIdx.x;
-	const int lane = threadIdx.x;
-	if (v == 0 && lane == 0 && P.inmix)
-		for (uint32_t x = 0; x < 8; ++x) P.inmix[INMIX_QUEUE + INMIX_LINE * x] = 0;
-	if (v == 0 && lane == 0) { P.work_count[0] = 0; P.work_count[1] = 0; }
-	if (v >= P.n_voices) return;
-	const VoiceDesc vd = P.voices[v];
-	const uint32_t *gids = P.op_ids + vd.ops_ofs;
-	const bool use_lds = lds_ops != 0 && vd.nops <= lds_ops && vd.plan_len <= lds_steps;
-	DevOp *lops = (DevOp *)a_lds;
-	Step *lplan = (Step *)(a_lds + (size_t)lds_ops * sizeof(DevOp));
-	uint32_t *lids = (uint32_t *)(a_lds + (size_t)lds_ops * sizeof(DevOp) + (size_t)lds_steps * sizeof(Step));
-	__shared__ uint8_t a_extra[256], a_dep[256], a_level[256];
-	for (uint32_t i = (uint32_t)lane; i < 64; i += 64) { ((uint32_t *)a_extra)[i] = 0; ((uint32_t *)a_dep)[i] = 0; ((uint32_t *)a_level)[i] = 0; }
-	if (use_lds) {
-		static_assert(sizeof(DevOp) % 16 == 0 && sizeof(Step) == 16, "copied 16 bytes at a time");
-		constexpr uint32_t Q = sizeof(DevOp) / 16;
-		for (uint32_t i = (uint32_t)lane; i < vd.nops * Q; i += 64)
-			((uint4 *)lops)[i] = ((const uint4 *)&P.ops[gids[i / Q]])[i % Q];
-		for (uint32_t i = (uint32_t)lane; i < vd.plan_len; i += 64) ((uint4 *)lplan)[i] = ((const uint4 *)(P.steps + vd.plan_ofs))[i];
-		for (uint32_t i = (uint32_t)lane; i < vd.nops; i += 64) lids[i] = i;
-	}
-	__syncthreads();
-	if (lane == 0) {
-	const uint32_t *ids = use_lds ? lids : gids;
-	DevOp *const OPS = use_lds ? lops : P.ops;
+__device__ __forceinline__ FastInfo analyze_voice(const FastParams &P, const uint32_t v, const VoiceDesc &vd, const uint32_t *ids,
+		DevOp *const OPS, const Step *plan, uint8_t *a_extra, uint8_t *a_dep, uint8_t *a_level) {
 	bool bad = (vd.flags & VD_NO_FAST) != 0 || !P.enable;
 	bool seq = false, has_red = false, has_rcub = false, has_rchain = false;
 	uint32_t min_time = 0xFFFFFFFFu;
-	const Step *plan = use_lds ? lplan : P.steps + vd.plan_ofs;
 	for (uint32_t i = 0; i < vd.nops; ++i) OPS[ids[i]].rt_frozen = 0;
 	if (P.chain_desc)
 		for (uint32_t k = 0; k < vd.n_chain; ++k)
@@ -346,7 +319,6 @@
 	if ((seq || has_chain) && !P.seq_enable) bad = true;
 	if (!bad && vd.nops <= P.max_ops && vd.plan_len <= P.max_steps && maxd >= 1 && maxd + x_carrier <= P.np / 2)
 		fi.total = min(min_time, vd.run_len);
-	P.info[v] = fi;
 	if (fi.total && seq_kind == 2 && n_scan_out == 0 && P.lean_on) atomicOr(&P.pass_flags[FAST_LEAN_FLAG], 1u);
 	else if (fi.total && (seq_kind == 1 || seq_kind == 2)) atomicOr(&P.pass_flags[FAST_MAX_LEVELS + 2], 1u);
 	P.fast_done[v] = 0;
@@ -357,11 +329,5 @@
 		if (seq_kind == 0) P.vlists[atomicAdd(&P.pass_flags[FAST_CF_COUNT], 1u)] = v;
 		else if (seq_kind == 3) P.vlists[P.n_voices + atomicAdd(&P.pass_flags[FAST_LK_COUNT], 1u)] = v;
 	}
-	}
-	if (use_lds) {
-		__syncthreads();
-		constexpr uint32_t Q = sizeof(DevOp) / 16;
-		for (uint32_t i = (uint32_t)lane; i < vd.nops * Q; i += 64)
-			((uint4 *)&P.ops[gids[i / Q]])[i % Q] = ((const uint4 *)lops)[i];
-	}
-}
+	return fi;
+}
diff --git a/saugns_amd/csrc/k_decode.h b/saugns_amd/csrc/k_decode.h
--- a/saugns_amd/csrc/k_decode.h
+++ b/saugns_amd/csrc/k_decode.h
@@ -112,15 +112,12 @@
 	}
 }
 
-__global__ void __launch_bounds__(64) decode_kernel(FastParams P) {
-	const uint32_t v = blockIdx.x;
-	const int l = threadIdx.x;
-	if (P.info[v].total == 0) return;
-	const bool lean = P.lean_on && P.info[v].seq == 2 && P.info[v].n_scan == 0;
-	const uint32_t NP = 64 * (P.info[v].cub ? FAST_CUB_ROWS : lean ? P.rows_lean : (P.info[v].seq == 1 || P.info[v].seq == 2) ? P.rows_multi :
-		(P.split_cf && P.info[v].seq == 0) ? P.rows_cf : P.rows);
-	const VoiceDesc vd = P.voices[v];
-	const uint32_t *ids = P.op_ids + vd.ops_ofs;
+__device__ __forceinline__ void decode_voice(const FastParams &P, const uint32_t v, const int l, const VoiceDesc &vd, const uint32_t *ids,
+		const uint32_t *gids, DevOp *const OPS, const Step *plan, FastInfo &fi) {
+	if (fi.total == 0) return;
+	const bool lean = P.lean_on && fi.seq == 2 && fi.n_scan == 0;
+	const uint32_t NP = 64 * (fi.cub ? FAST_CUB_ROWS : lean ? P.rows_lean : (fi.seq == 1 || fi.seq == 2) ? P.rows_multi :
+		(P.split_cf && fi.seq == 0) ? P.rows_cf : P.rows);
 	bool keep = false;
 	FastStep f;
 	FastLine fl, pl;
@@ -128,16 +125,15 @@
 	memset(&f, 0, sizeof f); memset(&fl, 0, sizeof fl); memset(&fa, 0, sizeof fa); memset(&pl, 0, sizeof pl);
 	bool is_chain = false, chain_line = false, chain_inline = false;
 	uint32_t dep = 0;
-	const uint32_t seq = P.info[v].seq;
+	const uint32_t seq = fi.seq;
 	if ((uint32_t)l < vd.plan_len) {
-		const Step *plan = P.steps + vd.plan_ofs;
 		for (uint32_t q = 0; q <= (uint32_t)l; ++q) {
 			const Step sq = plan[q];
 			if (sq.flags & SF_BEGIN) ++dep;
 			if (q < (uint32_t)l && (sq.flags & SF_END)) --dep;
 		}
 		const Step st = plan[l];
-		const DevOp &o = P.ops[ids[st.op]];
+		const DevOp &o = OPS[ids[st.op]];
 		keep = !(st.kind == ST_LINE && st.which == L_FREQ && o.rt_fconst_valid);
 		is_chain = step_is_chain(st, o);
 		const uint32_t st_which = st.kind == ST_SMLINE ? (uint32_t)L_PMA : (uint32_t)st.which;
@@ -148,7 +144,7 @@
 				uint32_t d2 = 0, frozen_at = 0;
 				for (uint32_t q = 0; q <= (uint32_t)l; ++q) {
 					const Step sq = plan[q];
-					const DevOp &oq = P.ops[ids[sq.op]];
+					const DevOp &oq = OPS[ids[sq.op]];
 					if (sq.flags & SF_BEGIN) {
 						++d2;
 						if (!frozen_at && !(oq.flags & OPF_TIME_INF) && oq.time == 0) frozen_at = d2;
@@ -160,7 +156,7 @@
 			zero_fill = root_end && !(st.flags & SF_LAYER) && !(st.which & OX_VOICE);
 			keep = zero_fill;
 		}
-		const uint32_t eff_dep = dep + P.info[v].xlead - min(P.ops[ids[st.op]].st_prev_phase, P.info[v].xlead);
+		const uint32_t eff_dep = dep + fi.xlead - min(OPS[ids[st.op]].st_prev_phase, fi.xlead);
 		f.kind = (uint32_t)(st.kind == ST_SMLINE ? (uint8_t)ST_LINE : st.kind) | ((uint32_t)st.flags << 8) | (st_which << 16) | (eff_dep << 24);
 		const FastIds cs = P.fast_ids[(seq ? P.ids_full_ofs : 0u) + vd.plan_ofs + l];
 		f.out_off = cs.out != NO_SLOT ? (uint32_t)cs.out * NP : ~0u;
@@ -179,7 +175,7 @@
 		f.diff_scale = o.type == OT_WAVE ? P.wc[wv].diff_scale : 0.f;
 		f.diff_offset = o.type == OT_WAVE ? P.wc[wv].diff_offset : 0.f;
 		f.tab = o.type == OT_WAVE ? P.tab_of_wave[wv] : -1;
-		f.gop = ids[st.op];
+		f.gop = gids[st.op];
 		f.prev_Is = o.prev_Is;
 		if (o.type == OT_RASEG) {
 			const bool rate2x = (o.flags & OPF_RATE2X) != 0;
@@ -191,7 +187,7 @@
 			f.diff_scale = bits_f(o.ras_level);
 			f.diff_offset = bits_f(o.ras_alpha);
 			f.type |= rate2x ? 1u << 17 : 0u;
-			if (P.info[v].cub && (vd.flags & VD_TAILS) && o.wave == LN_cub && !o.rt_frozen) {
+			if (fi.cub && (vd.flags & VD_TAILS) && o.wave == LN_cub && !o.rt_frozen) {
 				uint32_t rem = (vd.flags & VD_MORE) ? TAIL_FAR : min(vd.run_len, TAIL_FAR);
 				uint32_t closed = 0;
 				for (uint32_t q = (uint32_t)l + 1; q-- > 0;) {
@@ -200,7 +196,7 @@
 					if (sq.flags & SF_BEGIN) {
 						if (closed) --closed;
 						else {
-							const DevOp &oa = P.ops[ids[sq.op]];
+							const DevOp &oa = OPS[ids[sq.op]];
 							if (!(oa.flags & OPF_TIME_INF) && oa.time < rem) rem = oa.time;
 						}
 					}
@@ -220,19 +216,19 @@
 			f.pan = bits_f(row);
 			ChainDesc cd;
 			memset(&cd, 0, sizeof cd);
-			cd.n = P.info[v].total; cd.gop = ids[st.op]; cd.row = row;
+			cd.n = fi.total; cd.gop = gids[st.op]; cd.row = row;
 			uint32_t cmode = step_is_chain_acc(st, o) ? CM_INC : CM_BASE;
 			if (st.sm == NO_SLOT) {
 				LineState pls = o.line[L_PMA];
-				const LineBlock lb = line_begin(pls, P.info[v].total, false, 0.f, lattice_none(), 0);
+				const LineBlock lb = line_begin(pls, fi.total, false, 0.f, lattice_none(), 0);
 				pl.sw = lb.sw; pl.goal_len = lb.goal_len; pl.hold = lb.hold; pl.pad = 0;
 				chain_line = true;
 			}
 			uint32_t lstep = ~0u;
-			if (step_is_chain_inline(P.chain_inline != 0 || P.info[v].early != 0, plan, (uint32_t)l, ids, P.ops, &lstep)) {
+			if (step_is_chain_inline(P.chain_inline != 0 || fi.early != 0, plan, (uint32_t)l, ids, OPS, &lstep)) {
 				chain_inline = true;
 				cmode = CM_INLINE;
-				if (P.info[v].early) { cd.lflags |= CL_EARLY; f.type |= FT_CHAIN_EARLY; }
+				if (fi.early) { cd.lflags |= CL_EARLY; f.type |= FT_CHAIN_EARLY; }
 				if (o.type == OT_RASEG) cd.lflags |= CL_RASEG;
 				cd.coeff = o.coeff;
 				cd.pl = pl;
@@ -244,9 +240,9 @@
 					const Step ls = lstep != ~0u ? plan[lstep] : st;
 					const bool have_mul = ls.fmul != NO_SLOT;
 					float pf = 1.f;
-					if (have_mul && ls.prov != NO_SLOT) pf = P.ops[ids[ls.prov]].rt_fconst;
+					if (have_mul && ls.prov != NO_SLOT) pf = OPS[ids[ls.prov]].rt_fconst;
 					LineState fls = o.line[L_FREQ];
-					const LineBlock lb = line_begin(fls, P.info[v].total, have_mul, pf, lattice_none(), 0);
+					const LineBlock lb = line_begin(fls, fi.total, have_mul, pf, lattice_none(), 0);
 					cd.fl.sw = lb.sw; cd.fl.goal_len = lb.goal_len; cd.fl.hold = lb.hold; cd.fl.pad = 0;
 					if (lb.mul_goal) cd.lflags |= CL_MUL_GOAL;
 					if (lb.mul_hold) cd.lflags |= CL_MUL_HOLD;
@@ -270,7 +266,7 @@
 						P.wc[wv].diff_scale, P.wc[wv].diff_offset);
 				pprev = pa;
 			}
-			DevOp &ow = P.ops[ids[st.op]];
+			DevOp &ow = OPS[ids[st.op]];
 			ow.st_phase = o.phase; ow.st_prev_phase = pprev; ow.st_prev_Is = Is0; ow.st_prev_s = held;
 			f.type = OT_AMP;
 			f.fc = held;
@@ -285,7 +281,7 @@
 			const bool have_mul = st.fmul != NO_SLOT;
 			bool pconst = false; float pf = 1.f;
 			if (have_mul && st.prov != NO_SLOT) {
-				const DevOp &po = P.ops[ids[st.prov]];
+				const DevOp &po = OPS[ids[st.prov]];
 				pconst = po.rt_fconst_valid != 0; pf = po.rt_fconst;
 			}
 			fa.freq_off = ~0u; fa.fmul_off = ~0u; fa.coeff = o.coeff; fa.flags = 0; fa.mulc = 1.f;
@@ -295,7 +291,7 @@
 			LineState ls = o.line[line_step ? st_which : L_AMP];
 			if (line_step || amp_inline) {
 				if (ls.flags & LP_GOAL) {
-					const LineBlock lb = line_begin(ls, P.info[v].total, line_step && have_mul, pconst ? pf : 1.f, lattice_none(), 0);
+					const LineBlock lb = line_begin(ls, fi.total, line_step && have_mul, pconst ? pf : 1.f, lattice_none(), 0);
 					fl.sw = lb.sw; fl.goal_len = lb.goal_len; fl.hold = lb.hold; fl.pad = 0;
 					f.ramp = 1;
 					if (lb.mul_goal) fa.flags |= FA_MUL_GOAL;
@@ -321,7 +317,7 @@
 				uint32_t xi = 0;
 				for (uint32_t q = vd.plan_len; q-- > 0;) {
 					const Step sq = plan[q];
-					const DevOp &oq = P.ops[ids[sq.op]];
+					const DevOp &oq = OPS[ids[sq.op]];
 					if (oq.rt_frozen) continue;
 					if (sq.kind == ST_LINE && sq.which == L_FREQ && oq.rt_fconst_valid) continue;
 					const FastIds cq = P.fast_ids[P.ids_full_ofs + vd.plan_ofs + q];
@@ -333,10 +329,10 @@
 					const bool writes = sq.kind == ST_LINE || sq.kind == ST_LERP || sq.kind == ST_SMLINE ||
 						(sq.kind == ST_OSC && !(sq.which & OX_VOICE));
 					const bool rmw = sq.kind == ST_LERP || (sq.kind == ST_OSC && (sq.flags & SF_LAYER));
-					const bool v_early = P.info[v].early != 0;
+					const bool v_early = fi.early != 0;
 					const bool q_chain = step_is_chain(sq, oq);
 					uint32_t q_ls = ~0u;
-					const bool q_inline = q_chain && step_is_chain_inline(P.chain_inline != 0 || v_early, plan, q, ids, P.ops, &q_ls);
+					const bool q_inline = q_chain && step_is_chain_inline(P.chain_inline != 0 || v_early, plan, q, ids, OPS, &q_ls);
 					const bool q_early = q_inline && v_early;
 					{
 						bool needed = false;
@@ -405,7 +401,7 @@
 				uint32_t xi = 0;
 				for (uint32_t q = 0; q < (uint32_t)l; ++q) {
 					const Step sq = plan[q];
-					const DevOp &oq = P.ops[ids[sq.op]];
+					const DevOp &oq = OPS[ids[sq.op]];
 					if (oq.rt_frozen) continue;
 					if (sq.kind == ST_OSC && (((oq.type == OT_WAVE || oq.type == OT_RASEG) && !oq.rt_fconst_valid) ||
 					                          (oq.type == OT_NOISE && oq.wave == NZ_re))) ++xi;
@@ -419,7 +415,7 @@
 					fa.freq_off = cs.freq != NO_SLOT ? (uint32_t)cs.freq * NP : ~0u;
 				} else {
 					LineState fls = o.line[L_FREQ];
-					const LineBlock lb = line_begin(fls, P.info[v].total, have_mul, pconst ? pf : 1.f, lattice_none(), 0);
+					const LineBlock lb = line_begin(fls, fi.total, have_mul, pconst ? pf : 1.f, lattice_none(), 0);
 					fa.fl.sw = lb.sw; fa.fl.goal_len = lb.goal_len; fa.fl.hold = lb.hold;
 					fa.flags |= FA_FVAR_LINE;
 					if (lb.mul_goal) fa.flags |= FA_MUL_GOAL;
@@ -434,7 +430,7 @@
 					uint32_t k = 0;
 					for (uint32_t q = 0; q < (uint32_t)l; ++q) {
 						const Step sq = plan[q];
-						const uint32_t tq = P.ops[ids[sq.op]].type;
+						const uint32_t tq = OPS[ids[sq.op]].type;
 						if (sq.kind == ST_OSC && (tq == OT_WAVE || tq == OT_RASEG)) ++k;
 					}
 					if (k < vd.n_inc) fa.pad[2] = 2u | ((vd.inc_base + k) << 8);
@@ -445,34 +441,34 @@
 	{
 		bool lost = false;
 		if ((uint32_t)l < vd.plan_len && seq) {
-			const Step st = P.steps[vd.plan_ofs + l];
+			const Step st = plan[l];
 			const FastIds cs = P.fast_ids[P.ids_full_ofs + vd.plan_ofs + l];
-			const DevOp &o = P.ops[ids[st.op]];
+			const DevOp &o = OPS[ids[st.op]];
 			if (keep && st.kind == ST_LINE && st.which == L_FREQ && cs.out == NO_SLOT) lost = true;
 			if (keep && st.kind == ST_LINE && (st.which == L_FREQ2 || st.which == L_AMP2) && cs.out == NO_SLOT)
 				keep = false;
 			if (keep && st.kind == ST_LERP && st.freq != NO_SLOT && cs.aux == NO_SLOT) {
 				bool found = false;
 				for (uint32_t q = (uint32_t)l; q-- > 0;) {
-					const Step sq = P.steps[vd.plan_ofs + q];
+					const Step sq = plan[q];
 					if (sq.out != st.freq) continue;
 					if (sq.kind == ST_LINE && (sq.which == L_FREQ2 || sq.which == L_AMP2)) {
-						const DevOp &oq = P.ops[ids[sq.op]];
+						const DevOp &oq = OPS[ids[sq.op]];
 						const LineState &ls = oq.line[sq.which];
 						float c = ls.v0;
 						bool pc = true;
 						if (sq.fmul != NO_SLOT && (ls.flags & LP_STATE_RATIO)) {
-							pc = sq.prov != NO_SLOT && P.ops[ids[sq.prov]].rt_fconst_valid != 0;
-							if (pc) c *= P.ops[ids[sq.prov]].rt_fconst;
+							pc = sq.prov != NO_SLOT && OPS[ids[sq.prov]].rt_fconst_valid != 0;
+							if (pc) c *= OPS[ids[sq.prov]].rt_fconst;
 							else {
 								for (uint32_t r = q; r-- > 0;) {
-									const Step sr = P.steps[vd.plan_ofs + r];
+									const Step sr = plan[r];
 									if (sr.out != sq.fmul) continue;
 									if (sr.kind == ST_LINE && sr.which == L_FREQ) {
-										const DevOp &po = P.ops[ids[sr.op]];
+										const DevOp &po = OPS[ids[sr.op]];
 										const LineState &pls = po.line[L_FREQ];
 										pc = !(pls.flags & LP_GOAL) && (sr.fmul == NO_SLOT || !(pls.flags & LP_STATE_RATIO) ||
-										                                (sr.prov != NO_SLOT && P.ops[ids[sr.prov]].rt_fconst_valid != 0));
+										                                (sr.prov != NO_SLOT && OPS[ids[sr.prov]].rt_fconst_valid != 0));
 										if (pc) c *= po.rt_fconst;
 									}
 									break;
@@ -489,12 +485,12 @@
 			if (keep && st.kind == ST_OSC && (o.type == OT_WAVE || o.type == OT_RASEG) && !o.rt_fconst_valid && st.freq != NO_SLOT && cs.freq == NO_SLOT) lost = true;
 			if (keep && (f.ramp & 2) && fa.fmul_off == ~0u && (fa.flags & (FA_MUL_GOAL | FA_MUL_HOLD)) && fa.mulc == 1.f && st.fmul != NO_SLOT && cs.fmul == NO_SLOT) {
 				bool pc = false;
-				if (st.prov != NO_SLOT) pc = P.ops[ids[st.prov]].rt_fconst_valid != 0;
+				if (st.prov != NO_SLOT) pc = OPS[ids[st.prov]].rt_fconst_valid != 0;
 				if (!pc) lost = true;
 			}
 		}
 		if (__any(lost)) {
-			if (l == 0) { P.info[v].total = 0; P.info[v].bail = 1; }
+			fi.total = 0; fi.bail = 1;
 			keep = false;
 		}
 	}
@@ -513,8 +509,8 @@
 			if (f.ramp & 2) P.faux[at] = fa;
 			if (chain_line && P.fplines) P.fplines[at] = pl;
 		}
-		if (l == 0) { if (li == 0) P.info[v].n_fsteps = (uint32_t)__popcll(m); else P.info[v].n_pass[li - 1] = (uint32_t)__popcll(m); }
+		if (l == 0) { if (li == 0) fi.n_fsteps = (uint32_t)__popcll(m); else fi.n_pass[li - 1] = (uint32_t)__popcll(m); }
 	}
 	const unsigned long long mc = __ballot(is_chain && keep && !chain_inline);
-	if (l == 0) P.info[v].n_chain = (uint32_t)__popcll(mc);
+	fi.n_chain = (uint32_t)__popcll(mc);
 }
diff --git a/saugns_amd/csrc/k_prologue.h b/saugns_amd/csrc/k_prologue.h
--- /dev/null
+++ b/saugns_amd/csrc/k_prologue.h
@@ -0,0 +1,41 @@
+
+__global__ void __launch_bounds__(64) prologue_kernel(FastParams P, uint32_t lds_ops, uint32_t lds_steps) {
+	extern __shared__ __align__(16) unsigned char a_lds[];
+	const uint32_t v = blockIdx.x;
+	const int lane = threadIdx.x;
+	if (v == 0 && lane == 0 && P.inmix)
+		for (uint32_t x = 0; x < 8; ++x) P.inmix[INMIX_QUEUE + INMIX_LINE * x] = 0;
+	if (v == 0 && lane == 0) { P.work_count[0] = 0; P.work_count[1] = 0; }
+	if (v >= P.n_voices) return;
+	const VoiceDesc vd = P.voices[v];
+	const uint32_t *gids = P.op_ids + vd.ops_ofs;
+	const bool use_lds = lds_ops != 0 && vd.nops <= lds_ops && vd.plan_len <= lds_steps;
+	DevOp *lops = (DevOp *)a_lds;
+	Step *lplan = (Step *)(a_lds + (size_t)lds_ops * sizeof(DevOp));
+	uint32_t *lids = (uint32_t *)(a_lds + (size_t)lds_ops * sizeof(DevOp) + (size_t)lds_steps * sizeof(Step));
+	__shared__ uint8_t a_extra[256], a_dep[256], a_level[256];
+	__shared__ FastInfo s_fi;
+	for (uint32_t i = (uint32_t)lane; i < 64; i += 64) { ((uint32_t *)a_extra)[i] = 0; ((uint32_t *)a_dep)[i] = 0; ((uint32_t *)a_level)[i] = 0; }
+	constexpr uint32_t Q = sizeof(DevOp) / 16;
+	if (use_lds) {
+		static_assert(sizeof(DevOp) % 16 == 0 && sizeof(Step) == 16, "copied 16 bytes at a time");
+		for (uint32_t i = (uint32_t)lane; i < vd.nops * Q; i += 64)
+			((uint4 *)lops)[i] = ((const uint4 *)&P.ops[gids[i / Q]])[i % Q];
+		for (uint32_t i = (uint32_t)lane; i < vd.plan_len; i += 64) ((uint4 *)lplan)[i] = ((const uint4 *)(P.steps + vd.plan_ofs))[i];
+		for (uint32_t i = (uint32_t)lane; i < vd.nops; i += 64) lids[i] = i;
+	}
+	__syncthreads();
+	const uint32_t *ids = use_lds ? lids : gids;
+	DevOp *const OPS = use_lds ? lops : P.ops;
+	const Step *plan = use_lds ? lplan : P.steps + vd.plan_ofs;
+	if (lane == 0) s_fi = analyze_voice(P, v, vd, ids, OPS, plan, a_extra, a_dep, a_level);
+	__syncthreads();
+	FastInfo fi = s_fi;
+	decode_voice(P, v, lane, vd, ids, gids, OPS, plan, fi);
+	if (use_lds) {
+		__syncthreads();
+		for (uint32_t i = (uint32_t)lane; i < vd.nops * Q; i += 64)
+			((uint4 *)&P.ops[gids[i / Q]])[i % Q] = ((const uint4 *)lops)[i];
+	}
+	if (lane == 0) P.info[v] = fi;
+}
diff --git a/saugns_amd/csrc/launch_plan.h b/saugns_amd/csrc/launch_plan.h
--- a/saugns_amd/csrc/launch_plan.h
+++ b/saugns_amd/csrc/launch_plan.h
@@ -524,6 +524,33 @@
 	return p;
 }
 
+enum Stage : uint32_t {
+	STAGE_PROLOGUE = 1,
+	STAGE_SPLIT,
+	STAGE_SUMS_CHAINS,
+	STAGE_CLOSED_FORM,
+	STAGE_CUB,
+	STAGE_REPAIR,
+	STAGE_FINALIZE,
+	STAGE_BLOCK_LOOP,
+	STAGE_MIXER,
+};
+constexpr uint32_t MAX_STAGES = 9;
+inline uint32_t plan_stages(const FastPlan &k, Stage out[MAX_STAGES]) {
+	uint32_t n = 0;
+	out[n++] = STAGE_PROLOGUE;
+	if (k.use_fast) {
+		if (k.main_build == 2) out[n++] = STAGE_SPLIT;
+		out[n++] = k.scan ? STAGE_SUMS_CHAINS : STAGE_CLOSED_FORM;
+		out[n++] = STAGE_CUB;
+		out[n++] = STAGE_REPAIR;
+	}
+	out[n++] = STAGE_FINALIZE;
+	out[n++] = STAGE_BLOCK_LOOP;
+	out[n++] = STAGE_MIXER;
+	return n;
+}
+
 inline Mixer plan_mixer(const SegmentDesc &seg, const Tuning &tun, const PlanInputs &in, size_t pcm_pitch, bool inmix_live,
 		uint32_t early_blocks) {
 	if (!in.max_write) return MIX_NONE;
```
